# l-johnson-code/glTF-Renderer

Measured on AMD Instinct MI355X. Metric: Mrays/sec + ms/frame @1920x1080, 8-bounce, 1/2/4/8 MI355X, higher is better.
Workload: dtype f32

## Files before the change

gltf_renderer_amd/csrc/mipt_api.hip:

```cpp
#include <hip/hip_runtime.h>

#include <cmath>
#include <cstdio>
#include <cstdlib>
#include <cstring>
#include <string>
#include <vector>

#include "pt_types.h"

#include "pt_host.h"

using namespace pt;

struct StagingRing {
    static constexpr int kSlots = 8;
    void* host[kSlots] = {};
    size_t cap[kSlots] = {};
    hipEvent_t done[kSlots] = {};
    bool pending[kSlots] = {};
    int next = 0;
};

enum AccelState { ACCEL_CLEAN = 0, ACCEL_REFIT = 1, ACCEL_REBUILD = 2 };


struct pt_ctx {
    int device = 0;
    hipStream_t stream = nullptr;
    std::string error;
    StagingRing staging;

    std::vector<BufferRec> buffers;
    std::vector<TextureRec> textures;
    std::vector<SamplerRec> samplers;
    BufferRec* d_buffers = nullptr; size_t d_buffers_cap = 0; bool buffers_dirty = true;
    uint32_t* d_white = nullptr;
    struct TrioRec { const uint32_t *a, *n, *m, *e; uint4* ptr; };
    std::vector<TrioRec> trios;

    RMat* d_rmats = nullptr; int n_materials = 0; size_t rmats_cap = 0;
    std::vector<RMat> rmats_host;
    pt_light* d_lights = nullptr; int n_lights = 0; size_t lights_cap = 0;

    std::vector<InstanceRec> instances;
    InstanceRec* d_instances = nullptr; size_t instances_cap = 0;
    uint32_t n_tris = 0;
    Bvh4Node* d_nodes = nullptr; TriPacket* d_tris = nullptr; ShadePacket* d_shade = nullptr; size_t accel_cap = 0;
    uint32_t wide_nodes = 0, stack_need = 0;
    int32_t root = 0;
    AccelScratch scratch;
    int accel_state = ACCEL_REBUILD;
    bool accel_built = false;
    bool instances_dirty = true;
    std::vector<uint8_t> touched;
    uint8_t* d_touched = nullptr; size_t touched_cap = 0;
    uint32_t accel_refits = 0, accel_builds = 0;
    std::vector<int> free_buffers, free_textures, free_envs;

    std::vector<EnvDevice*> envs;
    float* d_sheen = nullptr;
    float* d_srgb = nullptr;
    float2* d_tangent_lut = nullptr;
    Counters* d_counters = nullptr;
    void* d_bones = nullptr; size_t bones_cap = 0, bones_used = 0;
    hipEvent_t bones_fence = nullptr; bool bones_fence_pending = false;
    void* d_workspace = nullptr; size_t workspace_cap = 0;
    void* d_tonemap = nullptr; size_t tonemap_cap = 0;
    pt::ExchangeState* exchange = nullptr;
    int32_t* d_deep = nullptr; size_t deep_cap = 0;
    uint32_t* d_occ = nullptr; size_t occ_pixels = 0; uint32_t occ_w = 0, occ_h = 0; bool occ_stale = true;
    bool occ_enabled = false;
    bool stage_timing = false;
    StageTimers timers;
    int kernel_mode = PT_MODE_WAVEFRONT;
    int stage_blocks = 0;
    hipEvent_t ev_trace[2] = {nullptr, nullptr}, ev_accel[2] = {nullptr, nullptr}, ev_skin[2] = {nullptr, nullptr};
    bool have_trace = false, have_accel = false, have_skin = false;
    int bounce_limit = PT_REFERENCE_MAX_BOUNCES;
    int samples_per_trace = 1;
    bool cull_null_shadow = false;
    bool counters_enabled = false;

    float previous_world_to_clip[16] = {0};
    int accumulated_frames = 0;

    int fail(int code, const std::string& msg) { error = msg; return code; }
};

#define HIPOK(call)                                                                                          \
    do {                                                                                                     \
        hipError_t _e = (call);                                                                              \
        if (_e != hipSuccess) return ctx->fail(PT_ERR_DEVICE, std::string(#call) + ": " + hipGetErrorString(_e)); \
    } while (0)
#define ENTER(ctx)                                                                                           \
    do {                                                                                                     \
        hipError_t _e = hipSetDevice((ctx)->device);                                                         \
        if (_e != hipSuccess) return (ctx)->fail(PT_ERR_DEVICE, std::string("hipSetDevice: ") + hipGetErrorString(_e)); \
    } while (0)

namespace {

hipError_t staged_upload(pt_ctx* ctx, void* dst, const void* src, size_t bytes) {
    if (bytes == 0) return hipSuccess;
    StagingRing& r = ctx->staging;
    const int k = r.next;
    r.next = (r.next + 1) % StagingRing::kSlots;
    hipError_t e;
    if (r.pending[k]) { if ((e = hipEventSynchronize(r.done[k]))) return e; r.pending[k] = false; }
    if (bytes > r.cap[k]) {
        if (r.host[k]) hipHostFree(r.host[k]);
        r.host[k] = nullptr; r.cap[k] = 0;
        const size_t nc = bytes + bytes / 2 + 4096;
        if ((e = hipHostMalloc(&r.host[k], nc, hipHostMallocDefault))) return e;
        r.cap[k] = nc;
    }
    if (!r.done[k] && (e = hipEventCreateWithFlags(&r.done[k], hipEventDisableTiming))) return e;
    memcpy(r.host[k], src, bytes);
    if ((e = hipMemcpyAsync(dst, r.host[k], bytes, hipMemcpyHostToDevice, ctx->stream))) return e;
    if ((e = hipEventRecord(r.done[k], ctx->stream))) return e;
    r.pending[k] = true;
    return hipSuccess;
}

template <typename T>
hipError_t upload_table(pt_ctx* ctx, T*& d, size_t& cap, const std::vector<T>& h) {
    size_t n = h.size() ? h.size() : 1;
    if (n > cap) {
        hipError_t e = hipStreamSynchronize(ctx->stream);
        if (e) return e;
        hipFree(d);
        d = nullptr; cap = 0;
        size_t nc = n + n / 2 + 8;
        e = hipMalloc((void**)&d, nc * sizeof(T));
        if (e) return e;
        cap = nc;
    }
    if (h.empty()) return hipSuccess;
    return staged_upload(ctx, d, h.data(), h.size() * sizeof(T));
}

void mat4_mul(const float* a, const float* b, float* out) {
    for (int c = 0; c < 4; c++)
        for (int r = 0; r < 4; r++) {
            float s = 0;
            for (int k = 0; k < 4; k++) s += a[k * 4 + r] * b[c * 4 + k];
            out[c * 4 + r] = s;
        }
}
bool mat4_inverse(const float* mf, float* out) {
    double m[16], inv[16];
    for (int i = 0; i < 16; i++) m[i] = mf[i];
    double s0 = m[0] * m[5] - m[4] * m[1], s1 = m[0] * m[9] - m[8] * m[1], s2 = m[0] * m[13] - m[12] * m[1];
    double s3 = m[4] * m[9] - m[8] * m[5], s4 = m[4] * m[13] - m[12] * m[5], s5 = m[8] * m[13] - m[12] * m[9];
    double c5 = m[10] * m[15] - m[14] * m[11], c4 = m[6] * m[15] - m[14] * m[7], c3 = m[6] * m[11] - m[10] * m[7];
    double c2 = m[2] * m[15] - m[14] * m[3], c1 = m[2] * m[11] - m[10] * m[3], c0 = m[2] * m[7] - m[6] * m[3];
    double det = s0 * c5 - s1 * c4 + s2 * c3 + s3 * c2 - s4 * c1 + s5 * c0;
    if (det == 0) return false;
    double id = 1.0 / det;
    inv[0] = (m[5] * c5 - m[9] * c4 + m[13] * c3) * id;
    inv[4] = (-m[4] * c5 + m[8] * c4 - m[12] * c3) * id;
    inv[8] = (m[7] * s5 - m[11] * s4 + m[15] * s3) * id;
    inv[12] = (-m[6] * s5 + m[10] * s4 - m[14] * s3) * id;
    inv[1] = (-m[1] * c5 + m[9] * c2 - m[13] * c1) * id;
    inv[5] = (m[0] * c5 - m[8] * c2 + m[12] * c1) * id;
    inv[9] = (-m[3] * s5 + m[11] * s2 - m[15] * s1) * id;
    inv[13] = (m[2] * s5 - m[10] * s2 + m[14] * s1) * id;
    inv[2] = (m[1] * c4 - m[5] * c2 + m[13] * c0) * id;
    inv[6] = (-m[0] * c4 + m[4] * c2 - m[12] * c0) * id;
    inv[10] = (m[3] * s4 - m[7] * s2 + m[15] * s0) * id;
    inv[14] = (-m[2] * s4 + m[6] * s2 - m[14] * s0) * id;
    inv[3] = (-m[1] * c3 + m[5] * c1 - m[9] * c0) * id;
    inv[7] = (m[0] * c3 - m[4] * c1 + m[8] * c0) * id;
    inv[11] = (-m[3] * s3 + m[7] * s1 - m[11] * s0) * id;
    inv[15] = (m[2] * s3 - m[6] * s1 + m[10] * s0) * id;
    for (int i = 0; i < 16; i++) out[i] = (float)inv[i];
    return true;
}

size_t format_stride(int f) {
    switch (f) {
        case PT_FORMAT_R16_UINT: return 2;
        case PT_FORMAT_R32_UINT: return 4;
        case PT_FORMAT_R32G32B32_FLOAT: return 12;
        case PT_FORMAT_R10G10B10A2_UNORM: return 4;
        case PT_FORMAT_R32G32_FLOAT: return 8;
        case PT_FORMAT_R16G16B16A16_UNORM: return 8;
        case PT_FORMAT_JOINT_WEIGHT: return 16;
        default: return 0;
    }
}

int stage_blocks_for(size_t slots) { return slots >= 1200000 ? 1536 : (slots >= 400000 ? 768 : 512); }

void mark_buffer_users(pt_ctx* ctx, int handle) {
    if (handle < 0) return;
    if (ctx->touched.size() != ctx->instances.size()) ctx->touched.assign(ctx->instances.size(), 0);
    const void* ptr = ctx->buffers[handle].ptr;
    bool any = false;
    for (size_t i = 0; i < ctx->instances.size(); i++) {
        const InstanceRec& r = ctx->instances[i];
        if (r.p_index == ptr || r.p_position == ptr || r.p_tangent_space == ptr || r.p_texcoord[0] == ptr || r.p_texcoord[1] == ptr || r.p_color == ptr) {
            ctx->touched[i] = 1;
            any = true;
        }
    }
    if (any && ctx->accel_state == ACCEL_CLEAN) ctx->accel_state = ACCEL_REFIT;
}

}

namespace pt {
class Pathtracer {
public:
    static int BuildAccel(pt_ctx* ctx) {
        if (ctx->buffers_dirty) { HIPOK(upload_table(ctx, ctx->d_buffers, ctx->d_buffers_cap, ctx->buffers)); ctx->buffers_dirty = false; }
        if (ctx->instances_dirty) { HIPOK(upload_table(ctx, ctx->d_instances, ctx->instances_cap, ctx->instances)); ctx->instances_dirty = false; }
        if (ctx->accel_state == ACCEL_CLEAN && ctx->accel_built) return PT_OK;
        const bool refit = ctx->accel_built && ctx->accel_state == ACCEL_REFIT;
        if (!refit) {
            size_t need = ctx->n_tris ? ctx->n_tris : 1;
            if (need > ctx->accel_cap) {
                HIPOK(hipStreamSynchronize(ctx->stream));
                hipFree(ctx->d_nodes); hipFree(ctx->d_tris); hipFree(ctx->d_shade);
                ctx->d_nodes = nullptr; ctx->d_tris = nullptr; ctx->d_shade = nullptr; ctx->accel_cap = 0;
                size_t cap = need + need / 8 + 64;
                HIPOK(hipMalloc((void**)&ctx->d_nodes, cap * sizeof(Bvh4Node)));
                HIPOK(hipMalloc((void**)&ctx->d_tris, cap * sizeof(TriPacket)));
                HIPOK(hipMalloc((void**)&ctx->d_shade, cap * sizeof(ShadePacket)));
                ctx->accel_cap = cap;
            }
        }
        HIPOK(hipEventRecord(ctx->ev_accel[0], ctx->stream));
        if (refit) {
            const size_t n = ctx->instances.size();
            if (n > ctx->touched_cap) {
                HIPOK(hipStreamSynchronize(ctx->stream));
                hipFree(ctx->d_touched); ctx->d_touched = nullptr; ctx->touched_cap = 0;
                HIPOK(hipMalloc((void**)&ctx->d_touched, n + 64));
                ctx->touched_cap = n + 64;
            }
            HIPOK(staged_upload(ctx, ctx->d_touched, ctx->touched.data(), n));
            HIPOK(accel_refit(ctx->scratch, ctx->d_instances, ctx->d_touched, ctx->n_tris, ctx->wide_nodes, ctx->d_nodes, ctx->d_tris, ctx->d_shade, ctx->stream));
            ctx->accel_refits++;
        } else {
            ctx->scratch.why.clear();
            const hipError_t be = accel_build(ctx->scratch, ctx->d_buffers, ctx->d_instances, (int)ctx->instances.size(), ctx->n_tris, ctx->d_nodes, ctx->d_tris,
                                              ctx->d_shade, &ctx->root, &ctx->wide_nodes, &ctx->stack_need, ctx->stream);
            if (be != hipSuccess) {
                ctx->accel_built = false; ctx->accel_state = ACCEL_REBUILD;
                return ctx->fail(PT_ERR_DEVICE, std::string("acceleration-structure build: ") + (ctx->scratch.why.empty() ? hipGetErrorString(be) : ctx->scratch.why.c_str()));
            }
            ctx->accel_builds++;
            ctx->occ_stale = true;
        }
        HIPOK(hipEventRecord(ctx->ev_accel[1], ctx->stream));
        ctx->have_accel = true;
        ctx->accel_state = ACCEL_CLEAN;
        ctx->accel_built = true;
        std::fill(ctx->touched.begin(), ctx->touched.end(), (uint8_t)0);
        if (!refit && ctx->stack_need > kDeepStackMax && ctx->scratch.builder != 0) {
            const int chosen = ctx->scratch.builder;
            ctx->scratch.builder = 0;
            ctx->scratch.fallbacks++;
            ctx->scratch.fallback_why = "clustered tree needs a traversal stack of " + std::to_string(ctx->stack_need) + " entries";
            const hipError_t be = accel_build(ctx->scratch, ctx->d_buffers, ctx->d_instances, (int)ctx->instances.size(), ctx->n_tris, ctx->d_nodes, ctx->d_tris,
                                              ctx->d_shade, &ctx->root, &ctx->wide_nodes, &ctx->stack_need, ctx->stream);
            ctx->scratch.builder = chosen;
            if (be != hipSuccess) {
                ctx->accel_built = false; ctx->accel_state = ACCEL_REBUILD;
                return ctx->fail(PT_ERR_DEVICE, std::string("acceleration-structure build (radix fallback): ") + (ctx->scratch.why.empty() ? hipGetErrorString(be) : ctx->scratch.why.c_str()));
            }
            HIPOK(hipEventRecord(ctx->ev_accel[1], ctx->stream));
        }
        if (!refit && ctx->stack_need > kDeepStackMax) {
            ctx->accel_built = false; ctx->accel_state = ACCEL_REBUILD;
            return ctx->fail(PT_ERR_CAPACITY, "acceleration structure needs a traversal stack of " + std::to_string(ctx->stack_need) + " entries (limit " +
                                              std::to_string(kDeepStackMax) + ")");
        }
        return PT_OK;
    }

    static int PathtraceScene(pt_ctx* ctx, const pt_settings* settings, const pt_execute_params* ep) {
        float world_to_clip[16], clip_to_world[16], view_to_world[16];
        mat4_mul(ep->view_to_clip, ep->world_to_view, world_to_clip);
        if (!mat4_inverse(ep->world_to_view, view_to_world) || !mat4_inverse(world_to_clip, clip_to_world))
            return ctx->fail(PT_ERR_INVALID_ARGUMENT, "singular camera matrix");
        bool reset = memcmp(world_to_clip, ctx->previous_world_to_clip, 64) != 0 || settings->reset;
        if (reset) ctx->accumulated_frames = 0;
        if (ctx->accumulated_frames < settings->max_accumulated_frames) {
            if (ep->light_count > ctx->n_lights) return ctx->fail(PT_ERR_INVALID_ARGUMENT, "light_count exceeds uploaded lights");
            if (ep->environment_map >= 0 && (ep->environment_map >= (int)ctx->envs.size() || !ctx->envs[ep->environment_map]))
                return ctx->fail(PT_ERR_BAD_HANDLE, "bad environment map handle");
            if (!ep->output) return ctx->fail(PT_ERR_INVALID_ARGUMENT, "output is null");
            if (ctx->accel_state != ACCEL_CLEAN || !ctx->accel_built || ctx->instances_dirty) { int r = BuildAccel(ctx); if (r) return r; }

            SceneRec sc;
            memset(&sc, 0, sizeof(sc));
            sc.rmats = ctx->d_rmats; sc.lights = ctx->d_lights; sc.instances = ctx->d_instances;
            sc.n_materials = (uint32_t)ctx->n_materials; sc.n_instances = (uint32_t)ctx->instances.size();
            sc.nodes = ctx->d_nodes; sc.tris = ctx->d_tris; sc.shade = ctx->d_shade; sc.root = ctx->root; sc.num_tris = ctx->n_tris;
            sc.sheen_e = ctx->d_sheen; sc.srgb_lut = ctx->d_srgb; sc.tangent_lut = ctx->d_tangent_lut;
            sc.has_env = 0;
            if (ep->environment_map >= 0) {
                const EnvDevice& ed = *ctx->envs[ep->environment_map];
                sc.env.cube = ed.cube; sc.env.cube_n = ed.mip_n[0]; sc.env.importance = ed.importance;
                for (int i = 0; i < 12; i++) sc.env.level_offset[i] = ed.level_offset[i];
                sc.env.imp_res = ed.imp_res; sc.env.imp_levels = ed.levels; sc.env.imp_total = ed.total;
                sc.env.blocked = ed.blocked;
                for (int i = 0; i < 5; i++) sc.env.blocked_offset[i] = ed.blocked_offset[i];
                sc.has_env = 1;
            }

            FrameConstants fc;
            memset(&fc, 0, sizeof(fc));
            memcpy(fc.clip_to_world, clip_to_world, 64);
            fc.camera_pos[0] = view_to_world[12]; fc.camera_pos[1] = view_to_world[13]; fc.camera_pos[2] = view_to_world[14];
            fc.num_of_lights = ep->light_count;
            fc.res_x = ep->width; fc.res_y = ep->height;
            fc.seed = settings->use_frame_as_seed ? (uint32_t)ep->frame : settings->seed;
            fc.accumulated_frames = ctx->accumulated_frames;
            memcpy(fc.environment_color, settings->environment_color, 12);
            fc.environment_intensity = settings->environment_intensity;
            fc.debug_output = settings->debug_output;
            fc.flags = settings->flags;
            fc.max_ray_length = 1000;
            auto clampi = [](int v, int lo, int hi) { return v < lo ? lo : (v > hi ? hi : v); };
            fc.min_bounces = clampi(settings->min_bounces, 0, ctx->bounce_limit);
            fc.max_bounces = clampi(settings->max_bounces, 0, ctx->bounce_limit);
            fc.luminance_clamp = settings->luminance_clamp;
            fc.min_rr = settings->min_russian_roulette_continue_prob;
            fc.max_rr = settings->max_russian_roulette_continue_prob;
            fc.tiles_x = (ep->width + PT_TILE - 1) / PT_TILE;
            fc.tiles_y = (ep->height + PT_TILE - 1) / PT_TILE;
            fc.tile_rank_count = ep->tile_rank_count ? ep->tile_rank_count : 1;
            fc.tile_rank = ep->tile_rank;
            if (fc.tile_rank >= fc.tile_rank_count) return ctx->fail(PT_ERR_INVALID_ARGUMENT, "tile_rank >= tile_rank_count");
            uint32_t ntiles = fc.tiles_x * fc.tiles_y;
            fc.my_tiles = ntiles > fc.tile_rank ? (ntiles - fc.tile_rank + fc.tile_rank_count - 1) / fc.tile_rank_count : 0;

            int batch = 1;
            if ((settings->flags & PT_FLAG_ACCUMULATE) && settings->debug_output == PT_DEBUG_OUTPUT_NONE) {
                batch = ctx->samples_per_trace;
                const long long room = (long long)settings->max_accumulated_frames - ctx->accumulated_frames;
                if ((long long)batch > room) batch = (int)room;
            }
            fc.cull_null_shadow = ctx->cull_null_shadow ? 1u : 0u;
            {
                size_t rare = 0;
                for (const RMat& m : ctx->rmats_host) rare += (m.sheen_color_factor[0] != 0.0f || m.sheen_color_factor[1] != 0.0f || m.sheen_color_factor[2] != 0.0f) ? 1 : 0;
                fc.defer_rare = (rare != 0 && rare * 10 <= ctx->rmats_host.size()) ? 1u : 0u;
                static const int forced = [] { const char* e = getenv("MIPT_DEFER_RARE"); return e ? (atoi(e) != 0 ? 1 : 0) : -1; }();
                if (forced >= 0) fc.defer_rare = (uint32_t)forced;
            }
            fc.spp = 1; fc.pixel_slots = fc.my_tiles * 256u;
            fc.div_pixel_slots = FastDiv::make(fc.pixel_slots); fc.div_tiles_x = FastDiv::make(fc.tiles_x);
            fc.seed_step = settings->use_frame_as_seed ? 1u : 0u;

            if ((int)ctx->stack_need > traversal_stack_capacity()) {
                const uint32_t entries = (ctx->stack_need - (uint32_t)traversal_stack_capacity() + 7u) & ~7u;
                size_t lanes;
                if (ctx->kernel_mode == PT_MODE_MEGAKERNEL) lanes = (size_t)fc.my_tiles * 256;
                else lanes = (size_t)traversal_grid_lanes(ctx->stage_blocks > 0 ? ctx->stage_blocks : stage_blocks_for((size_t)fc.pixel_slots * (size_t)batch));
                const size_t need = (size_t)entries * lanes * 4;
                if (need > ctx->deep_cap) {
                    HIPOK(hipStreamSynchronize(ctx->stream));
                    hipFree(ctx->d_deep); ctx->d_deep = nullptr; ctx->deep_cap = 0;
                    if (hipMalloc((void**)&ctx->d_deep, need) != hipSuccess) { (void)hipGetLastError(); return ctx->fail(PT_ERR_OUT_OF_MEMORY, "deep traversal stack: " + std::to_string(need) + " bytes"); }
                    ctx->deep_cap = need;
                }
                sc.deep_stack = ctx->d_deep; sc.deep_entries = entries; sc.deep_lanes = (uint32_t)lanes;
            }
            HIPOK(hipEventRecord(ctx->ev_trace[0], ctx->stream));
            if (ctx->kernel_mode == PT_MODE_MEGAKERNEL) {
                for (int k = 0; k < batch; k++) {
                    FrameConstants fk = fc;
                    fk.seed = fc.seed + (uint32_t)k * fc.seed_step;
                    fk.accumulated_frames = fc.accumulated_frames + k;
                    launch_megakernel(sc, fk, (float4*)ep->output, ctx->d_counters, ctx->counters_enabled, ctx->stream);
                }
            } else {
                fc.spp = (uint32_t)batch;
                if ((unsigned long long)fc.pixel_slots * fc.spp > 0x7fffffffull) return ctx->fail(PT_ERR_CAPACITY, "sample batch too large for this resolution");
                const int stage_blocks = ctx->stage_blocks > 0 ? ctx->stage_blocks : stage_blocks_for((size_t)fc.pixel_slots * fc.spp);
                size_t need = wavefront_workspace_bytes(fc, stage_blocks);
                if (need > ctx->workspace_cap) {
                    HIPOK(hipStreamSynchronize(ctx->stream));
                    hipFree(ctx->d_workspace); ctx->d_workspace = nullptr; ctx->workspace_cap = 0;
                    HIPOK(hipMalloc(&ctx->d_workspace, need));
                    ctx->workspace_cap = need;
                }
                uint32_t* occ = nullptr;
                if (ctx->occ_enabled && settings->debug_output == PT_DEBUG_OUTPUT_NONE) {
                    const size_t px = (size_t)ep->width * ep->height;
                    if (px != ctx->occ_pixels || ep->width != ctx->occ_w) {
                        HIPOK(hipStreamSynchronize(ctx->stream));
                        hipFree(ctx->d_occ); ctx->d_occ = nullptr; ctx->occ_pixels = 0;
                        if (hipMalloc((void**)&ctx->d_occ, px * 8 * 4) == hipSuccess) { ctx->occ_pixels = px; ctx->occ_w = ep->width; ctx->occ_h = ep->height; ctx->occ_stale = true; }
                        else (void)hipGetLastError();
                    }
                    if (ctx->d_occ && ctx->occ_stale) { HIPOK(hipMemsetAsync(ctx->d_occ, 0xff, ctx->occ_pixels * 8 * 4, ctx->stream)); ctx->occ_stale = false; }
                    occ = ctx->d_occ;
                }
                HIPOK(launch_wavefront(sc, fc, (float4*)ep->output, ctx->d_counters, ctx->counters_enabled, ctx->d_workspace, stage_blocks,
                                       ctx->stage_timing ? &ctx->timers : nullptr, ctx->stream, occ));
            }
            HIPOK(hipGetLastError());
            HIPOK(hipEventRecord(ctx->ev_trace[1], ctx->stream));
            ctx->have_trace = true;
            if (settings->flags & PT_FLAG_ACCUMULATE) ctx->accumulated_frames += batch;
            else ctx->accumulated_frames = 0;
        }
        memcpy(ctx->previous_world_to_clip, world_to_clip, 64);
        return PT_OK;
    }
};

class GpuSkin {
public:
    static int Run(pt_ctx* ctx, const pt_skin_params* p, const pt_bone* bones, int bone_count) {
        auto buf = [&](int h, int fmt, size_t count, const void** out) -> bool {
            if (h < 0 || h >= (int)ctx->buffers.size()) return false;
            const BufferRec& b = ctx->buffers[h];
            if ((int)b.format != fmt || b.bytes < count * format_stride(fmt)) return false;
            *out = b.ptr;
            return true;
        };
        SkinArgs a;
        memset(&a, 0, sizeof(a));
        a.num_of_vertices = p->num_of_vertices;
        a.input_mesh_flags = p->input_mesh_flags;
        a.output_mesh_flags = p->output_mesh_flags;
        a.num_of_morph_targets = p->num_of_morph_targets < PT_MAX_SIMULTANEOUS_MORPH_TARGETS ? p->num_of_morph_targets : PT_MAX_SIMULTANEOUS_MORPH_TARGETS;
        if (a.num_of_morph_targets < 0) a.num_of_morph_targets = 0;
        if (!bones || bone_count <= 0) a.input_mesh_flags &= (uint32_t)!PT_MESH_FLAG_JOINT_WEIGHT;
        const void* ptr = nullptr;
        if (!buf(p->input_position, PT_FORMAT_R32G32B32_FLOAT, p->num_of_vertices, &ptr)) return ctx->fail(PT_ERR_BAD_HANDLE, "skin: input_position");
        a.in_position = (const float*)ptr;
        if (a.input_mesh_flags & PT_MESH_FLAG_TANGENT_SPACE) {
            if (!buf(p->input_tangent_space, PT_FORMAT_R10G10B10A2_UNORM, p->num_of_vertices, &ptr)) return ctx->fail(PT_ERR_BAD_HANDLE, "skin: input_tangent_space");
            a.in_tangent_space = (const uint32_t*)ptr;
        }
        if (a.input_mesh_flags & PT_MESH_FLAG_JOINT_WEIGHT) {
            if (!buf(p->input_joint_weight, PT_FORMAT_JOINT_WEIGHT, p->num_of_vertices, &ptr)) return ctx->fail(PT_ERR_BAD_HANDLE, "skin: input_joint_weight");
            a.in_joint_weight = (const uint4*)ptr;
        }
        if (a.output_mesh_flags & PT_DYNAMIC_MESH_FLAG_POSITION) {
            if (!buf(p->output_position, PT_FORMAT_R32G32B32_FLOAT, p->num_of_vertices, &ptr)) return ctx->fail(PT_ERR_BAD_HANDLE, "skin: output_position");
            a.out_position = (float*)ptr;
        }
        if (a.output_mesh_flags & PT_DYNAMIC_MESH_FLAG_TANGENT_SPACE) {
            if (!buf(p->output_tangent_space, PT_FORMAT_R10G10B10A2_UNORM, p->num_of_vertices, &ptr)) return ctx->fail(PT_ERR_BAD_HANDLE, "skin: output_tangent_space");
            a.out_tangent_space = (uint32_t*)ptr;
        }
        for (int i = 0; i < a.num_of_morph_targets; i++) {
            a.morph_weight[i] = p->morph_weights[i];
            if (p->morph_position[i] != -1) {
                if (!buf(p->morph_position[i], PT_FORMAT_R32G32B32_FLOAT, p->num_of_vertices, &ptr)) return ctx->fail(PT_ERR_BAD_HANDLE, "skin: morph_position");
                a.morph_position[i] = (const float*)ptr;
            }
            if (p->morph_tangent_space[i] != -1) {
                if (!buf(p->morph_tangent_space[i], PT_FORMAT_R10G10B10A2_UNORM, p->num_of_vertices, &ptr)) return ctx->fail(PT_ERR_BAD_HANDLE, "skin: morph_tangent_space");
                a.morph_tangent_space[i] = (const uint32_t*)ptr;
            }
        }
        if (a.input_mesh_flags & PT_MESH_FLAG_JOINT_WEIGHT) {
            size_t bytes = (size_t)bone_count * sizeof(pt_bone);
            if (ctx->bones_used + bytes > ctx->bones_cap) {
                if (bytes > ctx->bones_cap) {
                    HIPOK(hipStreamSynchronize(ctx->stream));
                    hipFree(ctx->d_bones); ctx->d_bones = nullptr; ctx->bones_cap = 0;
                    const size_t nc = bytes * 8 + 4096;
                    HIPOK(hipMalloc(&ctx->d_bones, nc));
                    ctx->bones_cap = nc;
                } else if (ctx->bones_fence_pending) HIPOK(hipEventSynchronize(ctx->bones_fence));
                ctx->bones_used = 0;
            }
            void* dst = (char*)ctx->d_bones + ctx->bones_used;
            ctx->bones_used += (bytes + 255) & ~(size_t)255;
            HIPOK(staged_upload(ctx, dst, bones, bytes));
            a.bones = (const pt_bone*)dst;
            a.bone_count = bone_count;
        }
        HIPOK(hipEventRecord(ctx->ev_skin[0], ctx->stream));
        launch_skin(a, p->use_mfma != 0, ctx->stream);
        HIPOK(hipGetLastError());
        HIPOK(hipEventRecord(ctx->ev_skin[1], ctx->stream));
        if (a.bones) { HIPOK(hipEventRecord(ctx->bones_fence, ctx->stream)); ctx->bones_fence_pending = true; }
        ctx->have_skin = true;
        if (a.out_position) mark_buffer_users(ctx, p->output_position);
        if (a.out_tangent_space) mark_buffer_users(ctx, p->output_tangent_space);
        return PT_OK;
    }
};
}

static int exchange_frame_checked(pt_ctx* ctx, const void* local, void* frame, uint32_t w, uint32_t h, int mode, int dst, std::string& err) {
    return exchange_frame(ctx->exchange, local, frame ? frame : const_cast<void*>(local), w, h, mode, dst, ctx->stream, err);
}

extern "C" {

int pt_abi_version(void) { return MIPT_ABI_VERSION; }

int pt_create(int device, void* hip_stream, const float* sheen_e_16x16, pt_ctx** out) {
    if (!out || !sheen_e_16x16) return PT_ERR_INVALID_ARGUMENT;
    *out = nullptr;
    int count = 0;
    if (hipGetDeviceCount(&count) != hipSuccess || device < 0 || device >= count) return PT_ERR_DEVICE;
    if (hipSetDevice(device) != hipSuccess) return PT_ERR_DEVICE;
    pt_ctx* ctx = new pt_ctx();
    ctx->device = device;
    ctx->stream = (hipStream_t)hip_stream;
    float srgb[256];
    for (int i = 0; i < 256; i++) {
        double c = i / 255.0;
        srgb[i] = (float)(c <= 0.04045 ? c / 12.92 : pow((c + 0.055) / 1.055, 2.4));
    }
    bool ok = hipMalloc((void**)&ctx->d_sheen, 256 * 4) == hipSuccess && hipMalloc((void**)&ctx->d_srgb, 256 * 4) == hipSuccess &&
              hipMalloc((void**)&ctx->d_counters, sizeof(Counters)) == hipSuccess && hipMalloc((void**)&ctx->d_white, 16) == hipSuccess &&
              hipMemset(ctx->d_white, 0xff, 16) == hipSuccess &&
              hipMemcpy(ctx->d_sheen, sheen_e_16x16, 256 * 4, hipMemcpyHostToDevice) == hipSuccess &&
              hipMemcpy(ctx->d_srgb, srgb, 256 * 4, hipMemcpyHostToDevice) == hipSuccess &&
              hipMemset(ctx->d_counters, 0, sizeof(Counters)) == hipSuccess &&
              hipMalloc((void**)&ctx->d_tangent_lut, 1024 * sizeof(float2)) == hipSuccess &&
              build_tangent_lut(ctx->d_tangent_lut, ctx->stream) == hipSuccess;
    for (int i = 0; i < 2 && ok; i++)
        ok = hipEventCreate(&ctx->ev_trace[i]) == hipSuccess && hipEventCreate(&ctx->ev_accel[i]) == hipSuccess && hipEventCreate(&ctx->ev_skin[i]) == hipSuccess;
    ok = ok && hipEventCreateWithFlags(&ctx->bones_fence, hipEventDisableTiming) == hipSuccess;
    if (!ok) { pt_destroy(ctx); return PT_ERR_DEVICE; }
    ctx->samplers.push_back({PT_ADDRESS_WRAP, PT_ADDRESS_WRAP, PT_FILTER_LINEAR, PT_FILTER_LINEAR});
    if (const char* b = getenv("MIPT_ACCEL_BUILDER")) {
        if (!strcmp(b, "ploc")) ctx->scratch.builder = PT_BUILDER_PLOC;
        else if (!strcmp(b, "lbvh")) ctx->scratch.builder = PT_BUILDER_LBVH;
        else if (!strcmp(b, "reinsert")) ctx->scratch.builder = PT_BUILDER_PLOC_REINSERT;
    }
    if (const char* b = getenv("MIPT_OCC_CACHE")) ctx->occ_enabled = atoi(b) != 0;
    if (const char* b = getenv("MIPT_REINSERT_PASSES")) {
        const int v = atoi(b);
        if (v >= 0 && v <= 64) ctx->scratch.reinsert_passes = v;
    }
    if (const char* b = getenv("MIPT_REINSERT_MIN_GAIN")) {
        const float v = (float)atof(b);
        if (v >= 0.0f && v < 1.0f) ctx->scratch.reinsert_min_gain = v;
    }
    *out = ctx;
    return PT_OK;
}

void pt_destroy(pt_ctx* ctx) {
    if (!ctx) return;
    hipSetDevice(ctx->device);
    hipStreamSynchronize(ctx->stream);
    for (auto& b : ctx->buffers) hipFree((void*)b.ptr);
    for (auto& t : ctx->textures) hipFree((void*)t.texels);
    for (auto& t : ctx->trios) hipFree((void*)t.ptr);
    for (auto* e : ctx->envs) if (e) { env_free(*e); delete e; }
    hipFree(ctx->d_buffers); hipFree(ctx->d_white); hipFree(ctx->d_rmats); hipFree(ctx->d_lights);
// ... 73 lines not shown
    return PT_OK;
}

int pt_texture_create(pt_ctx* ctx, const uint8_t* rgba8, int width, int height, int srgb, int* handle_out) {
    if (!ctx || !rgba8 || !handle_out || width <= 0 || height <= 0) return PT_ERR_INVALID_ARGUMENT;
    ENTER(ctx);
    void* d = nullptr;
    size_t bytes = (size_t)width * height * 4;
    HIPOK(hipMalloc(&d, bytes + 4));
    hipError_t e = hipMemcpy(d, rgba8, bytes, hipMemcpyHostToDevice);
    if (e) { hipFree(d); return ctx->fail(PT_ERR_DEVICE, std::string("pt_texture_create: ") + hipGetErrorString(e)); }
    const TextureRec rec = {(const uint32_t*)d, width, height, srgb ? 1u : 0u, 0u};
    if (!ctx->free_textures.empty()) { *handle_out = ctx->free_textures.back(); ctx->free_textures.pop_back(); ctx->textures[*handle_out] = rec; }
    else { ctx->textures.push_back(rec); *handle_out = (int)ctx->textures.size() - 1; }
    return PT_OK;
}

int pt_texture_destroy(pt_ctx* ctx, int handle) {
    if (!ctx) return PT_ERR_INVALID_ARGUMENT;
    if (handle < 0 || handle >= (int)ctx->textures.size() || !ctx->textures[handle].texels) return ctx->fail(PT_ERR_BAD_HANDLE, "pt_texture_destroy");
    for (const RMat& m : ctx->rmats_host)
        for (int k = 0; k < SLOT_COUNT; k++)
            if (m.tex[k].texels == ctx->textures[handle].texels)
                return ctx->fail(PT_ERR_NOT_READY, "pt_texture_destroy: the texture is used by the current material table (replace it with pt_scene_set_materials first)");
    ENTER(ctx);
    HIPOK(hipStreamSynchronize(ctx->stream));
    hipFree((void*)ctx->textures[handle].texels);
    ctx->textures[handle] = TextureRec{nullptr, 0, 0, 0u, 0u};
    ctx->free_textures.push_back(handle);
    return PT_OK;
}

int pt_sampler_create(pt_ctx* ctx, const pt_sampler_desc* d, int* handle_out) {
    if (!ctx || !d || !handle_out) return PT_ERR_INVALID_ARGUMENT;
    if (d->address_u < 0 || d->address_u > 2 || d->address_v < 0 || d->address_v > 2) return ctx->fail(PT_ERR_INVALID_ARGUMENT, "pt_sampler_create: address mode");
    ctx->samplers.push_back({d->address_u, d->address_v, d->min_filter, d->mag_filter});
    *handle_out = (int)ctx->samplers.size() - 1;
    return PT_OK;
}

__global__ void k_trio_interleave(uint4* __restrict__ dst, const uint32_t* __restrict__ a, const uint32_t* __restrict__ n, const uint32_t* __restrict__ m,
                                  const uint32_t* __restrict__ e, size_t count) {
    const size_t i = (size_t)blockIdx.x * blockDim.x + threadIdx.x;
    if (i < count) dst[i] = make_uint4(a[i], n ? n[i] : 0xffffffffu, m ? m[i] : 0xffffffffu, e ? e[i] : 0xffffffffu);
}

int pt_scene_set_materials(pt_ctx* ctx, const pt_material* m, int count) {
    if (!ctx || (count > 0 && !m) || count < 0) return PT_ERR_INVALID_ARGUMENT;
    for (const InstanceRec& r : ctx->instances)
        if (r.gpu.material_id >= count)
            return ctx->fail(PT_ERR_BAD_HANDLE, "pt_scene_set_materials: the current instance table uses material " + std::to_string(r.gpu.material_id) +
                                                ", the new table has " + std::to_string(count) + " (replace the instances first)");
    ENTER(ctx);
    for (int i = 0; i < count; i++) {
        const pt_texture_sample* slots[15] = {&m[i].normal, &m[i].albedo, &m[i].metallic_roughness, &m[i].occlusion, &m[i].emissive, &m[i].specular,
                                              &m[i].specular_color, &m[i].clearcoat, &m[i].clearcoat_roughness, &m[i].clearcoat_normal, &m[i].anisotropy,
                                              &m[i].sheen_color, &m[i].sheen_roughness, &m[i].transmission, &m[i].thickness};
        for (auto* s : slots) {
            if (s->descriptor < -1 || s->descriptor >= (int)ctx->textures.size() || (s->descriptor >= 0 && !ctx->textures[s->descriptor].texels))
                return ctx->fail(PT_ERR_BAD_HANDLE, "material texture descriptor out of range or destroyed");
            if (s->sampler < 0 || s->sampler >= (int)ctx->samplers.size()) return ctx->fail(PT_ERR_BAD_HANDLE, "material sampler out of range");
        }
    }
    std::vector<RMat> rm((size_t)count);
    for (int i = 0; i < count; i++) {
        const pt_material& s = m[i];
        RMat& r = rm[i];
        memset(&r, 0, sizeof(r));
        r.flags = s.flags; r.alpha_mode = s.alpha_mode; r.metalness_factor = s.metalness_factor; r.roughness_factor = s.roughness_factor;
        memcpy(r.base_color_factor, s.base_color_factor, 16);
        memcpy(r.emissive_factor, s.emissive_factor, 12); r.alpha_cutoff = s.alpha_cutoff;
        r.ior = s.ior; r.normal_scale = s.normal_scale; r.specular_factor = s.specular_factor; r.clearcoat_normal_scale = s.clearcoat_normal_scale;
        memcpy(r.specular_color_factor, s.specular_color_factor, 12); r.clearcoat_factor = s.clearcoat_factor;
        r.clearcoat_roughness_factor = s.clearcoat_roughness_factor; r.anisotropy_strength = s.anisotropy_strength;
        r.anisotropy_cos = (float)cos((double)s.anisotropy_rotation); r.anisotropy_sin = (float)sin((double)s.anisotropy_rotation);
        memcpy(r.sheen_color_factor, s.sheen_color_factor, 12); r.sheen_roughness_factor = s.sheen_roughness_factor;
        r.transmission_factor = s.transmission_factor;
        const pt_texture_sample* slots[SLOT_COUNT] = {&s.normal, &s.albedo, &s.metallic_roughness, &s.occlusion, &s.emissive, &s.specular,
                                                      &s.specular_color, &s.clearcoat, &s.clearcoat_roughness, &s.clearcoat_normal, &s.anisotropy,
                                                      &s.sheen_color, &s.sheen_roughness, &s.transmission, &s.thickness};
        for (int k = 0; k < SLOT_COUNT; k++) {
            const pt_texture_sample& a = *slots[k];
            RTex& t = r.tex[k];
            if (a.descriptor == -1) {
                t.texels = ctx->d_white; t.width = 1; t.height = 1; t.flags = RT_POINT;
                t.m00 = 0; t.m01 = 0; t.ox = 0; t.m10 = 0; t.m11 = 0; t.oy = 0;
                continue;
            }
            const TextureRec& tx = ctx->textures[a.descriptor];
            const SamplerRec& sm = ctx->samplers[a.sampler];
            float sn = 0.0f, cs = 1.0f;
            if (a.rotation != 0.0f) { sn = (float)sin((double)a.rotation); cs = (float)cos((double)a.rotation); }
            t.texels = tx.texels; t.width = tx.width; t.height = tx.height;
            t.flags = (tx.srgb ? RT_SRGB : 0u) | ((uint32_t)sm.address_u << 1) | ((uint32_t)sm.address_v << 3) |
                      (sm.mag_filter == PT_FILTER_POINT ? RT_POINT : 0u) | ((a.tex_coord & 1) ? RT_TEXCOORD1 : 0u);
            t.m00 = cs * a.scale[0]; t.m01 = sn * a.scale[1]; t.ox = a.offset[0];
            t.m10 = -sn * a.scale[0]; t.m11 = cs * a.scale[1]; t.oy = a.offset[1];
            r.bound_mask |= 1u << k;
        }
    }
    const char* env_trio = getenv("MIPT_TEXTURE_INTERLEAVE");
    const bool use_trio = !(env_trio && env_trio[0] == '0');
    std::vector<char> trio_live(ctx->trios.size(), 0);
    for (int i = 0; i < count && use_trio; i++) {
        RMat& r = rm[i];
        const RTex& A = r.tex[SLOT_ALBEDO];
        const RTex& N = r.tex[SLOT_NORMAL];
        const RTex& M = r.tex[SLOT_METALLIC_ROUGHNESS];
        const RTex& E = r.tex[SLOT_EMISSIVE];
        const bool ba = (r.bound_mask >> SLOT_ALBEDO) & 1u, bn = (r.bound_mask >> SLOT_NORMAL) & 1u, bm = (r.bound_mask >> SLOT_METALLIC_ROUGHNESS) & 1u;
        auto same_footprint = [&](const RTex& t) {
            return t.width == A.width && t.height == A.height && ((t.flags ^ A.flags) & ~(uint32_t)RT_SRGB) == 0 && memcmp(&t.m00, &A.m00, 6 * sizeof(float)) == 0;
        };
        const bool be = ((r.bound_mask >> SLOT_EMISSIVE) & 1u) && same_footprint(E);
        if (!ba || !(bn || bm) || (bn && !same_footprint(N)) || (bm && !same_footprint(M))) continue;
        const uint32_t* kn = bn ? N.texels : nullptr;
        const uint32_t* km = bm ? M.texels : nullptr;
        const uint32_t* ke = be ? E.texels : nullptr;
        size_t at = ctx->trios.size();
        for (size_t k = 0; k < ctx->trios.size(); k++)
            if (ctx->trios[k].a == A.texels && ctx->trios[k].n == kn && ctx->trios[k].m == km && ctx->trios[k].e == ke) { at = k; break; }
        if (at == ctx->trios.size()) {
            const size_t texels = (size_t)A.width * A.height;
            uint4* d = nullptr;
            if (hipMalloc((void**)&d, texels * 16 + 32) != hipSuccess) { (void)hipGetLastError(); continue; }
            hipLaunchKernelGGL(k_trio_interleave, dim3((unsigned)((texels + 255) / 256)), dim3(256), 0, ctx->stream, d, A.texels, kn, km, ke, texels);
            HIPOK(hipMemsetAsync((char*)d + texels * 16, 0xff, 32, ctx->stream));
            ctx->trios.push_back({A.texels, kn, km, ke, d});
            trio_live.push_back(0);
        }
        trio_live[at] = 1;
        r.trio = ctx->trios[at].ptr;
        r.bound_mask |= RM_TRIO | ((bn && (N.flags & RT_SRGB)) ? RM_TRIO_SRGB_N : 0u) | ((bm && (M.flags & RT_SRGB)) ? RM_TRIO_SRGB_M : 0u) |
                        (be ? (RM_TRIO_EMISSIVE | ((E.flags & RT_SRGB) ? RM_TRIO_SRGB_E : 0u)) : 0u);
    }
    HIPOK(upload_table(ctx, ctx->d_rmats, ctx->rmats_cap, rm));
    ctx->rmats_host.swap(rm);
    ctx->n_materials = count;
    bool any_dead = false;
    for (char l : trio_live) any_dead |= !l;
    if (any_dead) {
        HIPOK(hipStreamSynchronize(ctx->stream));
        std::vector<pt_ctx::TrioRec> keep;
        for (size_t k = 0; k < ctx->trios.size(); k++) { if (trio_live[k]) keep.push_back(ctx->trios[k]); else hipFree((void*)ctx->trios[k].ptr); }
        ctx->trios.swap(keep);
    }
    return PT_OK;
}

extern "C" int pt_debug_interleaved_materials(const pt_ctx* ctx) {
    int n = 0;
    if (ctx) for (const RMat& r : ctx->rmats_host) n += (r.bound_mask & RM_TRIO) ? 1 : 0;
    return n;
}

extern "C" int pt_debug_interleaved_emissive(const pt_ctx* ctx) {
    int n = 0;
    if (ctx) for (const RMat& r : ctx->rmats_host) n += (r.bound_mask & RM_TRIO_EMISSIVE) ? 1 : 0;
    return n;
}

extern "C" int pt_debug_intersect(pt_ctx* ctx, const float* rays, uint32_t n, uint32_t ray_flags, int mode, float* out) {
    if (!ctx || (n && (!rays || !out)) || mode < 0 || mode > 1) return PT_ERR_INVALID_ARGUMENT;
    ENTER(ctx);
    if (ctx->accel_state != ACCEL_CLEAN || !ctx->accel_built || ctx->instances_dirty) { int r = Pathtracer::BuildAccel(ctx); if (r) return r; }
    if (n == 0) return PT_OK;
    SceneRec sc;
    memset(&sc, 0, sizeof(sc));
    sc.rmats = ctx->d_rmats; sc.lights = ctx->d_lights; sc.instances = ctx->d_instances;
    sc.n_materials = (uint32_t)ctx->n_materials; sc.n_instances = (uint32_t)ctx->instances.size();
    sc.nodes = ctx->d_nodes; sc.tris = ctx->d_tris; sc.shade = ctx->d_shade; sc.root = ctx->root; sc.num_tris = ctx->n_tris;
    sc.sheen_e = ctx->d_sheen; sc.srgb_lut = ctx->d_srgb; sc.tangent_lut = ctx->d_tangent_lut;
    const uint32_t lanes = (n + 255u) & ~255u;
    float *d_rays = nullptr, *d_out = nullptr; int32_t* d_deep = nullptr;
    auto done = [&](int code, const std::string& why) { hipFree(d_rays); hipFree(d_out); hipFree(d_deep); return code == PT_OK ? PT_OK : ctx->fail(code, why); };
    if (hipMalloc((void**)&d_rays, (size_t)n * 32) != hipSuccess || hipMalloc((void**)&d_out, (size_t)n * 32) != hipSuccess) { (void)hipGetLastError(); return done(PT_ERR_OUT_OF_MEMORY, "pt_debug_intersect: ray buffers"); }
    if ((int)ctx->stack_need > traversal_stack_capacity()) {
        const uint32_t entries = (ctx->stack_need - (uint32_t)traversal_stack_capacity() + 7u) & ~7u;
        if (hipMalloc((void**)&d_deep, (size_t)entries * lanes * 4) != hipSuccess) { (void)hipGetLastError(); return done(PT_ERR_OUT_OF_MEMORY, "pt_debug_intersect: deep stack"); }
        sc.deep_stack = d_deep; sc.deep_entries = entries; sc.deep_lanes = lanes;
    }
    hipError_t e = hipMemcpyAsync(d_rays, rays, (size_t)n * 32, hipMemcpyHostToDevice, ctx->stream);
    if (e == hipSuccess) { launch_debug_intersect(sc, d_rays, n, ray_flags, mode, d_out, ctx->stream); e = hipGetLastError(); }
    if (e == hipSuccess && getenv("MIPT_DEBUG_INTERSECT_TIMING")) {
        hipEvent_t ev[2]; hipEventCreate(&ev[0]); hipEventCreate(&ev[1]);
        hipEventRecord(ev[0], ctx->stream);
        for (int k = 0; k < 5; k++) launch_debug_intersect(sc, d_rays, n, ray_flags, mode, d_out, ctx->stream);
        hipEventRecord(ev[1], ctx->stream); hipEventSynchronize(ev[1]);
        float ms = 0; hipEventElapsedTime(&ms, ev[0], ev[1]);
        fprintf(stderr, "pt_debug_intersect: %u rays, %.3f ms per launch, %.1f Mrays/s\n", n, ms / 5, n / (ms / 5) * 1e-3);
        hipEventDestroy(ev[0]); hipEventDestroy(ev[1]);
    }
    if (e == hipSuccess) e = hipMemcpyAsync(out, d_out, (size_t)n * 32, hipMemcpyDeviceToHost, ctx->stream);
    if (e == hipSuccess) e = hipStreamSynchronize(ctx->stream);
    return done(e == hipSuccess ? PT_OK : PT_ERR_DEVICE, std::string("pt_debug_intersect: ") + hipGetErrorString(e));
}

extern "C" int pt_debug_sample_texture(pt_ctx* ctx, int unit, const uint32_t* mat_slot, const float* tc, uint32_t n, float* out_rgba, int32_t* out_taps) {
    if (!ctx || unit < 0 || unit > 1 || (n && (!mat_slot || !tc || !out_rgba))) return PT_ERR_INVALID_ARGUMENT;
    for (uint32_t i = 0; i < n; i++) {
        const uint32_t mat = mat_slot[2 * i], slot = mat_slot[2 * i + 1];
        if (mat >= (uint32_t)ctx->n_materials || !(slot < (uint32_t)SLOT_COUNT || (slot >= 16u && slot <= 19u)))
            return ctx->fail(PT_ERR_INVALID_ARGUMENT, "pt_debug_sample_texture: query " + std::to_string(i) + " names material " + std::to_string(mat) +
                                                      " slot " + std::to_string(slot) + " (" + std::to_string(ctx->n_materials) + " materials)");
    }
    ENTER(ctx);
    if (n == 0) return PT_OK;
    SceneRec sc;
    memset(&sc, 0, sizeof(sc));
    sc.rmats = ctx->d_rmats; sc.n_materials = (uint32_t)ctx->n_materials;
    sc.sheen_e = ctx->d_sheen; sc.srgb_lut = ctx->d_srgb; sc.tangent_lut = ctx->d_tangent_lut;
    uint32_t* d_ms = nullptr; float *d_tc = nullptr, *d_out = nullptr; int32_t* d_taps = nullptr;
    auto done = [&](int code, const std::string& why) { hipFree(d_ms); hipFree(d_tc); hipFree(d_out); hipFree(d_taps); return code == PT_OK ? PT_OK : ctx->fail(code, why); };
    if (hipMalloc((void**)&d_ms, (size_t)n * 8) != hipSuccess || hipMalloc((void**)&d_tc, (size_t)n * 16) != hipSuccess ||
        hipMalloc((void**)&d_out, (size_t)n * 16) != hipSuccess || hipMalloc((void**)&d_taps, (size_t)n * 20) != hipSuccess) {
        (void)hipGetLastError(); return done(PT_ERR_OUT_OF_MEMORY, "pt_debug_sample_texture: query buffers");
    }
    hipError_t e = hipMemcpyAsync(d_ms, mat_slot, (size_t)n * 8, hipMemcpyHostToDevice, ctx->stream);
    if (e == hipSuccess) e = hipMemcpyAsync(d_tc, tc, (size_t)n * 16, hipMemcpyHostToDevice, ctx->stream);
    if (e == hipSuccess) {
        if (unit == 0) launch_debug_sample_texture_wf(sc, d_ms, d_tc, n, d_out, d_taps, ctx->stream);
        else launch_debug_sample_texture_mk(sc, d_ms, d_tc, n, d_out, d_taps, ctx->stream);
        e = hipGetLastError();
    }
    if (e == hipSuccess) e = hipMemcpyAsync(out_rgba, d_out, (size_t)n * 16, hipMemcpyDeviceToHost, ctx->stream);
    if (e == hipSuccess && out_taps) e = hipMemcpyAsync(out_taps, d_taps, (size_t)n * 20, hipMemcpyDeviceToHost, ctx->stream);
    if (e == hipSuccess) e = hipStreamSynchronize(ctx->stream);
    return done(e == hipSuccess ? PT_OK : PT_ERR_DEVICE, std::string("pt_debug_sample_texture: ") + hipGetErrorString(e));
}

extern "C" int pt_debug_env_query(pt_ctx* ctx, int env, int unit, int op, const float* in, uint32_t n, float* out) {
    if (!ctx || unit < 0 || unit > 1 || op < 0 || op > 3 || (n && (!in || !out))) return PT_ERR_INVALID_ARGUMENT;
    if (env < 0 || env >= (int)ctx->envs.size() || !ctx->envs[env]) return ctx->fail(PT_ERR_BAD_HANDLE, "pt_debug_env_query: environment " + std::to_string(env));
    ENTER(ctx);
    if (n == 0) return PT_OK;
    const EnvDevice& ed = *ctx->envs[env];
    SceneRec sc;
    memset(&sc, 0, sizeof(sc));
    sc.env.cube = ed.cube; sc.env.cube_n = ed.mip_n[0]; sc.env.importance = ed.importance;
    for (int i = 0; i < 12; i++) sc.env.level_offset[i] = ed.level_offset[i];
    sc.env.imp_res = ed.imp_res; sc.env.imp_levels = ed.levels; sc.env.imp_total = ed.total;
    sc.env.blocked = ed.blocked;
    for (int i = 0; i < 5; i++) sc.env.blocked_offset[i] = ed.blocked_offset[i];
    sc.has_env = 1;
    const size_t in_bytes = (size_t)n * 8 * 4, out_bytes = (size_t)n * 16 * 4;
    float *d_in = nullptr, *d_out = nullptr;
    auto done = [&](int code, const std::string& why) { hipFree(d_in); hipFree(d_out); return code == PT_OK ? PT_OK : ctx->fail(code, why); };
    if (hipMalloc((void**)&d_in, in_bytes) != hipSuccess || hipMalloc((void**)&d_out, out_bytes) != hipSuccess) {
        (void)hipGetLastError(); return done(PT_ERR_OUT_OF_MEMORY, "pt_debug_env_query: query buffers");
    }
    hipError_t e = hipMemcpyAsync(d_in, in, in_bytes, hipMemcpyHostToDevice, ctx->stream);
    if (e == hipSuccess) e = hipMemcpyAsync(d_out, out, out_bytes, hipMemcpyHostToDevice, ctx->stream);
    if (e == hipSuccess) {
        if (unit == 0) launch_debug_env_query_wf(sc, op, d_in, n, d_out, ctx->stream);
        else launch_debug_env_query_mk(sc, op, d_in, n, d_out, ctx->stream);
        e = hipGetLastError();
    }
    if (e == hipSuccess) e = hipMemcpyAsync(out, d_out, out_bytes, hipMemcpyDeviceToHost, ctx->stream);
    if (e == hipSuccess) e = hipStreamSynchronize(ctx->stream);
    return done(e == hipSuccess ? PT_OK : PT_ERR_DEVICE, std::string("pt_debug_env_query: ") + hipGetErrorString(e));
}

extern "C" int pt_debug_env_create_raw(pt_ctx* ctx, int cube_n, const uint16_t* cube_rgba16f, const float* pyramid, int* env_out) {
    if (!ctx || cube_n < 1 || cube_n > 16384 || !cube_rgba16f || !pyramid || !env_out) return PT_ERR_INVALID_ARGUMENT;
    ENTER(ctx);
    EnvDevice* env = new EnvDevice();
    hipError_t e = env_build_raw(*env, cube_n, cube_rgba16f, pyramid, ctx->stream);
    if (e) { env_free(*env); delete env; return ctx->fail(PT_ERR_DEVICE, std::string("pt_debug_env_create_raw: ") + hipGetErrorString(e)); }
    if (!ctx->free_envs.empty()) { *env_out = ctx->free_envs.back(); ctx->free_envs.pop_back(); ctx->envs[*env_out] = env; }
    else { ctx->envs.push_back(env); *env_out = (int)ctx->envs.size() - 1; }
    return PT_OK;
}

extern "C" int pt_debug_env_read_blocked(pt_ctx* ctx, int env, float* out) {
    if (!ctx || !out) return PT_ERR_INVALID_ARGUMENT;
    if (env < 0 || env >= (int)ctx->envs.size() || !ctx->envs[env]) return ctx->fail(PT_ERR_BAD_HANDLE, "pt_debug_env_read_blocked: environment " + std::to_string(env));
    ENTER(ctx);
    HIPOK(hipStreamSynchronize(ctx->stream));
    const EnvDevice& ed = *ctx->envs[env];
    HIPOK(hipMemcpy(out, ed.blocked, (size_t)(ed.blocked_offset[4] + 1024u * 1024u) * 4, hipMemcpyDeviceToHost));
    return PT_OK;
}

int pt_scene_set_lights(pt_ctx* ctx, const pt_light* l, int count) {
    if (!ctx || (count > 0 && !l) || count < 0) return PT_ERR_INVALID_ARGUMENT;
    ENTER(ctx);
    std::vector<pt_light> h(l, l + count);
    HIPOK(upload_table(ctx, ctx->d_lights, ctx->lights_cap, h));
    ctx->n_lights = count;
    return PT_OK;
}

int pt_scene_set_instances(pt_ctx* ctx, const pt_instance_desc* in, int count) {
    if (!ctx || (count > 0 && !in) || count < 0) return PT_ERR_INVALID_ARGUMENT;
    if (count > PT_MAX_TLAS_INSTANCES) return ctx->fail(PT_ERR_CAPACITY, "more than PT_MAX_TLAS_INSTANCES instances");
    std::vector<InstanceRec> recs;
    uint64_t tris = 0;
    auto check = [&](int h, int fmt_a, int fmt_b, size_t count_needed) -> bool {
        if (h == -1) return true;
        if (!live_buffer(ctx, h)) return false;
        const BufferRec& b = ctx->buffers[h];
        if ((int)b.format != fmt_a && (int)b.format != fmt_b) return false;
        return b.bytes >= count_needed * format_stride(b.format);
    };
    for (int i = 0; i < count; i++) {
        const pt_instance_desc& d = in[i];
// ... 310 lines not shown
```

gltf_renderer_amd/csrc/pt_host.h:

```cpp
#pragma once
#include <hip/hip_runtime.h>

#include <string>
#include <vector>

#include "pt_types.h"

namespace pt {

struct AccelScratch {
    TriPacket* tris_unsorted = nullptr;
    uint64_t *keys_a = nullptr, *keys_b = nullptr;
    uint32_t *vals_a = nullptr, *vals_b = nullptr;
    int32_t* leaf_parent = nullptr;
    int32_t* node_parent = nullptr;
    void* seg = nullptr;
    size_t seg_leaves = 0;
    float* block_bounds = nullptr;
    uint32_t* bounds = nullptr;
    void* sort_temp = nullptr;
    size_t sort_temp_bytes = 0;
    BvhNode* nodes2 = nullptr;
    uint32_t* kept = nullptr;
    uint32_t* widx = nullptr;
    uint32_t* collapse_counters = nullptr;
    WideRanges* wide_ranges = nullptr;
    int builder = 2;
    float reinsert_min_gain = 1e-3f;
    int reinsert_passes = 8;
    void* reins_box = nullptr; int32_t *reins_parent = nullptr, *reins_top = nullptr; float* reins_gain = nullptr; uint32_t* reins_out = nullptr;
    unsigned long long* reins_lock = nullptr; uint8_t* reins_state = nullptr;
    void* ploc_c[2] = {nullptr, nullptr};
    uint32_t *ploc_nn = nullptr, *ploc_valid = nullptr, *ploc_pos = nullptr, *ploc_count = nullptr, *ploc_perm = nullptr, *ploc_counters = nullptr;
    int32_t *ploc_left = nullptr, *ploc_right = nullptr;
    void* ploc_scan_temp = nullptr; size_t ploc_scan_bytes = 0;
    size_t capacity = 0;
    std::string why;
    uint32_t fallbacks = 0;
    std::string fallback_why;
};
void accel_scratch_free(AccelScratch& s);
hipError_t accel_build(AccelScratch& s, const BufferRec* d_buffers, const InstanceRec* d_instances, int n_inst, uint32_t n_tris, Bvh4Node* d_nodes,
                       TriPacket* d_tris, ShadePacket* d_shade, int32_t* root_out, uint32_t* wide_nodes_out, uint32_t* stack_need_out, hipStream_t stream);
hipError_t accel_refit(AccelScratch& s, const InstanceRec* d_instances, const uint8_t* d_touched, uint32_t n_tris, uint32_t wide_nodes,
                       Bvh4Node* d_nodes, TriPacket* d_tris, ShadePacket* d_shade, hipStream_t stream);

hipError_t build_tangent_lut(float2* d_lut, hipStream_t stream);

struct EnvDevice {
    uint16_t* cube = nullptr;
    size_t mip_offset[16] = {0};
    int mip_n[16] = {0};
    int mips = 0;
    float* importance = nullptr;
    uint32_t level_offset[12] = {0};
    int levels = 0;
    int imp_res = 1024;
    float* blocked = nullptr;
    uint32_t blocked_offset[5] = {0};
    float total = 0.f;
};
hipError_t env_build(EnvDevice& e, const float* d_equirect, int w, int h, hipStream_t stream);
hipError_t env_build_raw(EnvDevice& e, int n, const uint16_t* cube_rgba16f, const float* pyramid, hipStream_t stream);
void env_free(EnvDevice& e);

struct SkinArgs {
    uint32_t num_of_vertices, input_mesh_flags, output_mesh_flags;
    int32_t num_of_morph_targets;
    float morph_weight[4];
    const float* morph_position[4];
    const uint32_t* morph_tangent_space[4];
    const float* in_position;
    const uint32_t* in_tangent_space;
    const uint4* in_joint_weight;
    const pt_bone* bones;
    int32_t bone_count;
    float* out_position;
    uint32_t* out_tangent_space;
};
void launch_skin(const SkinArgs& a, bool use_mfma, hipStream_t stream);
void launch_tonemap(const float4* in, uint32_t w, uint32_t h, const pt_tonemap_config& cfg, float* out_rgb, uint32_t* out_rgba8, hipStream_t stream);

size_t traversal_grid_lanes(int stage_blocks);
constexpr uint32_t kDeepStackMax = 1024;
int traversal_stack_capacity();
enum { STAGE_GENERATE = 0, STAGE_TRACE = 1, STAGE_SHADE = 2, STAGE_SHADOW = 3, STAGE_RESOLVE = 4, STAGE_COUNT = 5 };
struct StageTimers {
    std::vector<hipEvent_t> ev;
    std::vector<uint8_t> kind;
    size_t used = 0;
};
void launch_debug_sample_texture_wf(const SceneRec& sc, const uint32_t* d_mat_slot, const float* d_tc, uint32_t n, float* d_out, int32_t* d_taps, hipStream_t stream);
void launch_debug_sample_texture_mk(const SceneRec& sc, const uint32_t* d_mat_slot, const float* d_tc, uint32_t n, float* d_out, int32_t* d_taps, hipStream_t stream);
void launch_debug_env_query_wf(const SceneRec& sc, int op, const float* d_in, uint32_t n, float* d_out, hipStream_t stream);
void launch_debug_env_query_mk(const SceneRec& sc, int op, const float* d_in, uint32_t n, float* d_out, hipStream_t stream);
void launch_debug_intersect(const SceneRec& sc, const float* d_rays, uint32_t n, uint32_t rf, int mode, float* d_out, hipStream_t stream);
void launch_megakernel(const SceneRec& sc, const FrameConstants& fc, float4* output, Counters* counters, bool count, hipStream_t stream);
size_t wavefront_workspace_bytes(const FrameConstants& fc, int stage_blocks);
hipError_t launch_wavefront(const SceneRec& sc, const FrameConstants& fc, float4* output, Counters* counters, bool count, void* workspace,
                            int stage_blocks, StageTimers* timers, hipStream_t stream, uint32_t* occ_cache);

size_t radix_sort_temp_bytes(size_t n);
hipError_t radix_sort_pairs_u64_u32(void* temp, uint64_t* keys_in, uint64_t* keys_out, uint32_t* vals_in, uint32_t* vals_out, size_t n, hipStream_t stream);
size_t exclusive_scan_temp_bytes(size_t n);
hipError_t exclusive_scan_u32(void* temp, const uint32_t* in, uint32_t* out, size_t n, hipStream_t stream);

struct ExchangeState;
uint32_t tiles_of_rank(uint32_t w, uint32_t h, uint32_t rank, uint32_t world);
hipError_t tiles_pack(const void* image, uint32_t w, uint32_t h, uint32_t rank, uint32_t world, void* packed, hipStream_t stream);
hipError_t tiles_unpack(const void* packed, uint32_t w, uint32_t h, uint32_t rank, uint32_t world, void* image, hipStream_t stream);
int exchange_unique_id(void* out128, std::string& err);
int exchange_probe(std::string& err);
int exchange_create(ExchangeState** out, int rank, int world, const void* id128, std::string& err);
int exchange_create_loopback(ExchangeState** out, int rank, int world, uint64_t group, int device, std::string& err);
const char* exchange_transport_name(const ExchangeState* x);
int exchange_frame(ExchangeState* x, const void* local, void* frame, uint32_t w, uint32_t h, int mode, int dst, hipStream_t stream, std::string& err);
void exchange_free(ExchangeState* x);

}
```

gltf_renderer_amd/csrc/pt_shading.h:

```cpp
#pragma once
#include "pt_math.h"
#include "pt_types.h"

namespace pt {

constexpr float kMinRoughness = 0.001f;

PT_DEV vec4 next_random(uint32_t px, uint32_t py, uint32_t seed, int& count) {
    uint32_t x = px * 1664525u + 1013904223u, y = py * 1664525u + 1013904223u;
    uint32_t z = seed * 1664525u + 1013904223u, w = (uint32_t)count * 1664525u + 1013904223u;
    count++;
    x += y * w; y += z * x; z += x * y; w += y * z;
    x ^= x >> 16; y ^= y >> 16; z ^= z >> 16; w ^= w >> 16;
    x += y * w; y += z * x; z += x * y; w += y * z;
    const float s = 2.3283064365386963e-10f;
    return {(float)x * s, (float)y * s, (float)z * s, (float)w * s};
}

PT_DEV vec3 decode_octahedral(float ex, float ey) {
    float z = 1.f - fabsf(ex) - fabsf(ey);
    float x = ex, y = ey;
    if (!(z >= 0.f)) {
        x = (ex >= 0 ? 1.f : -1.f) * (1.f - fabsf(ey));
        y = (ey >= 0 ? 1.f : -1.f) * (1.f - fabsf(ex));
// ... 281 lines not shown
    if (threadIdx.x < n) {
        float4 q[6];
        shade_inst_pack(sc.instances[threadIdx.x], q);
#pragma unroll
        for (int k = 0; k < 6; k++) pt_lds_inst[threadIdx.x * 6u + k] = q[k];
    }
    __syncthreads();
}
PT_DEV ShadeInst load_shade_inst(const SceneRec& sc, uint32_t id) {
    float4 q[6];
    if (sc.small_tables || id < kInstCacheMax) {
#pragma unroll
        for (int k = 0; k < 6; k++) q[k] = pt_lds_inst[id * 6u + k];
    } else shade_inst_pack(sc.instances[id], q);
    return shade_inst_unpack(q);
}
#else
PT_DEV void stage_instances(const SceneRec&) {}
PT_DEV ShadeInst load_shade_inst(const SceneRec& sc, uint32_t id) { float4 q[6]; shade_inst_pack(sc.instances[id], q); return shade_inst_unpack(q); }
#endif
PT_DEV HitGeom get_vertex_attributes(const SceneRec& sc, const ShadeInst& in, const PacketVerts& pv, vec3 w) {
    HitGeom a;
    const vec3 p0 = pv.p[0], p1 = pv.p[1], p2 = pv.p[2];
    const bool has_ts = (in.streams & SI_TANGENT_SPACE) != 0;
    const uint32_t ts0 = pv.ts[0], ts1 = pv.ts[1], ts2 = pv.ts[2];
    a.color = fetch_vertex_color((in.streams & SI_COLOR) != 0, pv, w);
    a.tc[0] = fetch_texcoord((in.streams & SI_TEXCOORD0) != 0, pv.uv0, w);
    a.tc[1] = fetch_texcoord((in.streams & SI_TEXCOORD1) != 0, pv.uv1, w);
    vec3 pos = w.x * p0 + w.y * p1 + w.z * p2;
    vec3 ng = cross(p1 - p0, p2 - p0);
    vec3 n, t;
    float tw;
    if (has_ts) {
        vec3 n0, n1, n2, t0, t1, t2;
        float w0, w1, w2;
        decode_tangent_space(ts0, tangent_sincos(sc, (ts0 >> 20) & 0x3ffu), n0, t0, w0);
        decode_tangent_space(ts1, tangent_sincos(sc, (ts1 >> 20) & 0x3ffu), n1, t1, w1);
        decode_tangent_space(ts2, tangent_sincos(sc, (ts2 >> 20) & 0x3ffu), n2, t2, w2);
        n = w.x * n0 + w.y * n1 + w.z * n2;
        t = w.x * t0 + w.y * t1 + w.z * t2;
        tw = w0;
    } else {
        n = ng;
        vec3 helper = v3(1, 0, 0);
        if (fabsf(ng.x) > fabsf(ng.y)) helper = v3(0, 1, 0);
        t = normalize(cross(helper, ng));
        tw = 1;
    }
    a.position = mul_point(in.T, pos);
    a.ng = normalize(mul_dir(in.N, ng));
    a.n = normalize(mul_dir(in.N, n));
    a.t = normalize(mul_dir(in.T, t));
    a.tw = tw;
    a.bt = tw * normalize(cross(a.n, a.t));
    return a;
}

struct Surface {
    vec3 albedo; float alpha, metalness, ax, ay;
    vec3 n, at, ab; float ior;
    vec3 spec_color; float spec_factor, clearcoat, cc_rough;
    vec3 cc_n, sheen_color; float sheen_a, transmissive;
    vec3 emissive_texel;
    float sheen_lh, sheen_sv;
};
struct MatHeader {
    uint32_t flags; int32_t alpha_mode; float metalness_factor, roughness_factor;
    vec4 base_color_factor;
    vec3 emissive_factor; float alpha_cutoff;
    float ior, normal_scale, specular_factor, clearcoat_normal_scale;
    vec3 specular_color_factor; float clearcoat_factor;
    float clearcoat_roughness_factor, anisotropy_strength, anisotropy_cos, anisotropy_sin;
    vec3 sheen_color_factor; float sheen_roughness_factor;
    float transmission_factor; uint32_t bound_mask;
    const uint4* trio;
};
PT_DEV MatHeader load_mat_header(const RMat* m) {
    const float4* q = (const float4*)m;
    const float4 a = q[0], b = q[1], c = q[2], d = q[3], e = q[4], f = q[5], g = q[6], h = q[7];
    MatHeader r;
    r.flags = __float_as_uint(a.x); r.alpha_mode = __float_as_int(a.y); r.metalness_factor = a.z; r.roughness_factor = a.w;
    r.base_color_factor = {b.x, b.y, b.z, b.w};
    r.emissive_factor = v3(c.x, c.y, c.z); r.alpha_cutoff = c.w;
    r.ior = d.x; r.normal_scale = d.y; r.specular_factor = d.z; r.clearcoat_normal_scale = d.w;
    r.specular_color_factor = v3(e.x, e.y, e.z); r.clearcoat_factor = e.w;
    r.clearcoat_roughness_factor = f.x; r.anisotropy_strength = f.y; r.anisotropy_cos = f.z; r.anisotropy_sin = f.w;
    r.sheen_color_factor = v3(g.x, g.y, g.z); r.sheen_roughness_factor = g.w;
    r.transmission_factor = h.x; r.bound_mask = __float_as_uint(h.y);
    r.trio = (const uint4*)(((uint64_t)__float_as_uint(h.w) << 32) | (uint64_t)__float_as_uint(h.z));
    return r;
}
PT_DEV bool slot_bound(uint32_t mask, int slot) { return (mask >> slot) & 1u; }
#ifdef PT_LUT_LDS
constexpr uint32_t kMatCacheMax = 96;
constexpr uint32_t kMatCacheRecs = 17;
static __shared__ float4 pt_lds_mat[kMatCacheMax * kMatCacheRecs];
PT_DEV bool materials_cached(const SceneRec& sc) { return sc.small_tables || sc.n_materials <= kMatCacheMax; }
PT_DEV void stage_materials(const SceneRec& sc) {
    if (materials_cached(sc)) {
        const uint32_t total = sc.n_materials * kMatCacheRecs;
        for (uint32_t i = threadIdx.x; i < total; i += blockDim.x) {
            const uint32_t m = i / kMatCacheRecs, k = i - m * kMatCacheRecs;
            pt_lds_mat[i] = ((const float4*)(sc.rmats + m))[k];
        }
    }
    __syncthreads();
}
PT_DEV MatHeader material_header(const SceneRec& sc, uint32_t mid) {
    if (materials_cached(sc)) return load_mat_header((const RMat*)(pt_lds_mat + mid * kMatCacheRecs));
    return load_mat_header(sc.rmats + mid);
}
PT_DEV RTex material_slot012(const SceneRec& sc, uint32_t mid, int slot) {
    if (materials_cached(sc)) return load_rtex((const RTex*)(pt_lds_mat + mid * kMatCacheRecs + 8 + 3 * slot));
    return load_rtex(&sc.rmats[mid].tex[slot]);
}
#else
PT_DEV MatHeader material_header(const SceneRec& sc, uint32_t mid) { return load_mat_header(sc.rmats + mid); }
PT_DEV RTex material_slot012(const SceneRec& sc, uint32_t mid, int slot) { return load_rtex(&sc.rmats[mid].tex[slot]); }
#endif
PT_DEV void base_color_alpha(const SceneRec& sc, const RMat* m, const vec2 tc[2], vec4 vc, unsigned& taps, float& base_alpha, float& alpha, float& cutoff) {
    const float4* q = (const float4*)m;
    const float4 a = q[0], b = q[1], c = q[2], h = q[7];
    vec4 col = vec4{b.x, b.y, b.z, b.w} * vc;
    if (slot_bound(__float_as_uint(h.y), SLOT_ALBEDO)) col = col * sample_slot(sc, m, SLOT_ALBEDO, tc, taps);
    const int alpha_mode = __float_as_int(a.y);
    cutoff = c.w;
    base_alpha = col.w;
    alpha = alpha_mode == PT_ALPHA_MODE_BLEND ? col.w : (alpha_mode == PT_ALPHA_MODE_MASK ? (col.w < cutoff ? 0.f : 1.f) : 1.f);
}
PT_DEV vec3 normal_from_sample(vec4 s, float scale, vec3 gn, vec3 t, vec3 b) {
    vec3 nm = v3(s.x * 2.f - 1.f, s.y * 2.f - 1.f, s.z * 2.f - 1.f);
    nm.x *= scale; nm.y *= scale;
    return normalize(to_world(t, b, gn, nm));
}
PT_DEV vec3 emissive_of(const SceneRec& sc, const RMat* m, const MatHeader& h, const vec2 tc[2], unsigned& taps, vec3 fetched) {
    vec3 e = h.emissive_factor;
#if PT_TEX_PAIRS && PT_TEX_TRIO
    if (h.bound_mask & RM_TRIO_EMISSIVE) { taps++; return e * fetched; }
#endif
    if (slot_bound(h.bound_mask, SLOT_EMISSIVE)) e = e * xyz(sample_slot(sc, m, SLOT_EMISSIVE, tc, taps));
    return e;
}
PT_DEV vec3 normal_adaptation(vec3 ng, vec3 ns, vec3 v) {
    vec3 r = reflect(-v, ns);
    float rdng = dot(r, ng);
    if (rdng < 0) return normalize(v + normalize(r - rdng * ng));
    return ns;
}
struct PbrTexels {
    TexTaps k_alb, k_nrm, k_mr;
    uint32_t a00, a10, a01, a11, n00, n10, n01, n11, m00, m10, m01, m11;
    vec4 emissive;
};
PT_DEV PbrTexels fetch_pbr_texels(const SceneRec& sc, uint32_t mid, const MatHeader& h, const vec2 tc[2]) {
    PbrTexels f;
    f.emissive = vec4{0, 0, 0, 0};
#if PT_TEX_PAIRS && PT_TEX_TRIO
    const bool trio = (h.bound_mask & RM_TRIO) != 0;
    const RTex t_alb = material_slot012(sc, mid, SLOT_ALBEDO);
    const TexTaps k_alb = texture_taps(t_alb, tc);
    TexTaps k_nrm = k_alb, k_mr = k_alb;
    k_nrm.srgb = (h.bound_mask & RM_TRIO_SRGB_N) ? (uint32_t)RT_SRGB : 0u; k_mr.srgb = (h.bound_mask & RM_TRIO_SRGB_M) ? (uint32_t)RT_SRGB : 0u;
    uint32_t a00 = 0, a10 = 0, a01 = 0, a11 = 0, n00 = 0, n10 = 0, n01 = 0, n11 = 0, m00 = 0, m10 = 0, m01 = 0, m11 = 0;
    if (__any(trio)) {
        if (trio) {
            const uint4* row0 = h.trio + (k_alb.p0 - t_alb.texels) + k_alb.ia;
            const uint4* row1 = h.trio + (k_alb.p1 - t_alb.texels) + k_alb.ia;
            const uint4 A0 = gload_u4(row0), B0 = gload_u4(row0 + 1), A1 = gload_u4(row1), B1 = gload_u4(row1 + 1);
            uint4 t00 = k_alb.i0 == k_alb.ia ? A0 : B0, t01 = k_alb.i0 == k_alb.ia ? A1 : B1;
            uint4 t10 = k_alb.i1 == k_alb.ia ? A0 : B0, t11 = k_alb.i1 == k_alb.ia ? A1 : B1;
            if (__any(k_alb.edge)) {
                if (k_alb.edge) { t10 = gload_u4(h.trio + (k_alb.p0 - t_alb.texels) + k_alb.i1); t11 = gload_u4(h.trio + (k_alb.p1 - t_alb.texels) + k_alb.i1); }
            }
            a00 = t00.x; a10 = t10.x; a01 = t01.x; a11 = t11.x;
            n00 = t00.y; n10 = t10.y; n01 = t01.y; n11 = t11.y;
            m00 = t00.z; m10 = t10.z; m01 = t01.z; m11 = t11.z;
            if (h.bound_mask & RM_TRIO_EMISSIVE) {
                TexTaps k_em = k_alb;
                k_em.srgb = (h.bound_mask & RM_TRIO_SRGB_E) ? (uint32_t)RT_SRGB : 0u;
                f.emissive = resolve_taps(k_em, t00.w, t10.w, t01.w, t11.w, sc.srgb_lut);
            }
        }
    }
    if (__any(!trio)) {
        if (!trio) {
            const RTex t_nrm = material_slot012(sc, mid, SLOT_NORMAL), t_mr = material_slot012(sc, mid, SLOT_METALLIC_ROUGHNESS);
            k_nrm = texture_taps(t_nrm, tc); k_mr = texture_taps(t_mr, tc);
            const uint2 ar0 = tap_row(k_alb, 0), ar1 = tap_row(k_alb, 1), nr0 = tap_row(k_nrm, 0), nr1 = tap_row(k_nrm, 1), mr0 = tap_row(k_mr, 0), mr1 = tap_row(k_mr, 1);
            const TexQuad qa = tap_quad(k_alb, ar0, ar1), qn = tap_quad(k_nrm, nr0, nr1), qm = tap_quad(k_mr, mr0, mr1);
            a00 = qa.t00; a10 = qa.t10; a01 = qa.t01; a11 = qa.t11;
            n00 = qn.t00; n10 = qn.t10; n01 = qn.t01; n11 = qn.t11;
            m00 = qm.t00; m10 = qm.t10; m01 = qm.t01; m11 = qm.t11;
        }
    }
#else
    const RTex t_alb = material_slot012(sc, mid, SLOT_ALBEDO), t_nrm = material_slot012(sc, mid, SLOT_NORMAL), t_mr = material_slot012(sc, mid, SLOT_METALLIC_ROUGHNESS);
    const TexTaps k_alb = texture_taps(t_alb, tc), k_nrm = texture_taps(t_nrm, tc), k_mr = texture_taps(t_mr, tc);
#if PT_TEX_PAIRS
    const uint2 ar0 = tap_row(k_alb, 0), ar1 = tap_row(k_alb, 1), nr0 = tap_row(k_nrm, 0), nr1 = tap_row(k_nrm, 1), mr0 = tap_row(k_mr, 0), mr1 = tap_row(k_mr, 1);
    const TexQuad qa = tap_quad(k_alb, ar0, ar1), qn = tap_quad(k_nrm, nr0, nr1), qm = tap_quad(k_mr, mr0, mr1);
    const uint32_t a00 = qa.t00, a10 = qa.t10, a01 = qa.t01, a11 = qa.t11;
    const uint32_t n00 = qn.t00, n10 = qn.t10, n01 = qn.t01, n11 = qn.t11;
    const uint32_t m00 = qm.t00, m10 = qm.t10, m01 = qm.t01, m11 = qm.t11;
#else
    const uint32_t a00 = gload(k_alb.p00), a10 = gload(k_alb.p10), a01 = gload(k_alb.p01), a11 = gload(k_alb.p11);
    const uint32_t n00 = gload(k_nrm.p00), n10 = gload(k_nrm.p10), n01 = gload(k_nrm.p01), n11 = gload(k_nrm.p11);
    const uint32_t m00 = gload(k_mr.p00), m10 = gload(k_mr.p10), m01 = gload(k_mr.p01), m11 = gload(k_mr.p11);
#endif
#endif
    f.k_alb = k_alb; f.k_nrm = k_nrm; f.k_mr = k_mr;
    f.a00 = a00; f.a10 = a10; f.a01 = a01; f.a11 = a11;
    f.n00 = n00; f.n10 = n10; f.n01 = n01; f.n11 = n11;
    f.m00 = m00; f.m10 = m10; f.m01 = m01; f.m11 = m11;
    return f;
}
PT_DEV Surface get_surface(const SceneRec& sc, uint32_t flags, const RMat* m, const MatHeader& h, const HitGeom& a, vec3 view, unsigned& taps) {
    Surface s;
    const PbrTexels f = fetch_pbr_texels(sc, (uint32_t)(m - sc.rmats), h, a.tc);
    s.emissive_texel = xyz(f.emissive);
    const TexTaps &k_alb = f.k_alb, &k_nrm = f.k_nrm, &k_mr = f.k_mr;
    const uint32_t a00 = f.a00, a10 = f.a10, a01 = f.a01, a11 = f.a11, n00 = f.n00, n10 = f.n10, n01 = f.n01, n11 = f.n11, m00 = f.m00, m10 = f.m10, m01 = f.m01, m11 = f.m11;
    const bool b_alb = slot_bound(h.bound_mask, SLOT_ALBEDO), b_nrm = slot_bound(h.bound_mask, SLOT_NORMAL), b_mr = slot_bound(h.bound_mask, SLOT_METALLIC_ROUGHNESS);
    taps += (b_alb ? 1u : 0u) + (b_nrm ? 1u : 0u) + (b_mr ? 1u : 0u);
    vec4 bc = h.base_color_factor * a.color;
    if (b_alb) bc = bc * resolve_taps(k_alb, a00, a10, a01, a11, sc.srgb_lut);
    s.albedo = xyz(bc);
    s.alpha = h.alpha_mode == PT_ALPHA_MODE_BLEND ? bc.w : (h.alpha_mode == PT_ALPHA_MODE_MASK ? (bc.w < h.alpha_cutoff ? 0.f : 1.f) : 1.f);
    s.n = b_nrm ? normal_from_sample(resolve_taps(k_nrm, n00, n10, n01, n11, sc.srgb_lut), h.normal_scale, a.n, a.t, a.bt) : a.n;
    if (flags & PT_FLAG_SHADING_NORMAL_ADAPTATION) s.n = normal_adaptation(a.ng, s.n, view);
    float metal = h.metalness_factor, rough = h.roughness_factor;
    if (b_mr) { vec4 t = resolve_taps(k_mr, m00, m10, m01, m11, sc.srgb_lut); metal *= t.z; rough *= t.y; }
    s.metalness = metal;
    s.ay = hmax(rough * rough, kMinRoughness);
    if (slot_bound(h.bound_mask, SLOT_OCCLUSION)) taps++;
    if (slot_bound(h.bound_mask, SLOT_EMISSIVE)) taps++;
    s.ior = h.ior;
    s.spec_factor = h.specular_factor;
    s.spec_color = h.specular_color_factor;
    s.clearcoat = h.clearcoat_factor;
    s.cc_rough = h.clearcoat_roughness_factor;
    s.cc_n = a.n;
    float strength = h.anisotropy_strength;
    vec3 av = v3(1, 0, 1);
    s.sheen_color = h.sheen_color_factor;
    float sheen_rough = h.sheen_roughness_factor;
    s.transmissive = h.transmission_factor;
#ifndef PT_PROBE_BASE_ONLY
    if ((h.bound_mask & ((1u << SLOT_COUNT) - 1u)) >> SLOT_SPECULAR) {
        if (slot_bound(h.bound_mask, SLOT_SPECULAR)) s.spec_factor *= sample_slot(sc, m, SLOT_SPECULAR, a.tc, taps).w;
        if (slot_bound(h.bound_mask, SLOT_SPECULAR_COLOR)) s.spec_color = s.spec_color * xyz(sample_slot(sc, m, SLOT_SPECULAR_COLOR, a.tc, taps));
        if (slot_bound(h.bound_mask, SLOT_CLEARCOAT)) s.clearcoat *= sample_slot(sc, m, SLOT_CLEARCOAT, a.tc, taps).x;
        if (slot_bound(h.bound_mask, SLOT_CLEARCOAT_ROUGHNESS)) s.cc_rough *= sample_slot(sc, m, SLOT_CLEARCOAT_ROUGHNESS, a.tc, taps).y;
        if (slot_bound(h.bound_mask, SLOT_CLEARCOAT_NORMAL))
            s.cc_n = normal_from_sample(sample_slot(sc, m, SLOT_CLEARCOAT_NORMAL, a.tc, taps), h.clearcoat_normal_scale, a.n, a.t, a.bt);
        if (slot_bound(h.bound_mask, SLOT_ANISOTROPY)) {
            vec4 t = sample_slot(sc, m, SLOT_ANISOTROPY, a.tc, taps);
            av = v3(t.x * 2 - 1, t.y * 2 - 1, t.z);
        }
        if (slot_bound(h.bound_mask, SLOT_SHEEN_COLOR)) s.sheen_color = s.sheen_color * xyz(sample_slot(sc, m, SLOT_SHEEN_COLOR, a.tc, taps));
        if (slot_bound(h.bound_mask, SLOT_SHEEN_ROUGHNESS)) sheen_rough *= sample_slot(sc, m, SLOT_SHEEN_ROUGHNESS, a.tc, taps).w;
        if (slot_bound(h.bound_mask, SLOT_TRANSMISSION)) s.transmissive *= sample_slot(sc, m, SLOT_TRANSMISSION, a.tc, taps).x;
        if (slot_bound(h.bound_mask, SLOT_THICKNESS)) taps++;
    }
#endif
    if (flags & PT_FLAG_SHADING_NORMAL_ADAPTATION) s.cc_n = normal_adaptation(a.ng, s.cc_n, view);
    const float cr = h.anisotropy_cos, sr = h.anisotropy_sin;
    vec2 adir = normalize(vec2{cr * av.x + -sr * av.y, sr * av.x + cr * av.y});
    strength *= av.z;
    vec3 sb = normalize(cross(s.n, a.t));
    vec3 st = normalize(cross(sb, s.n));
    sb = sb * a.tw;
    s.at = normalize(to_world(st, sb, s.n, v3(adir.x, adir.y, 0)));
    s.ab = normalize(cross(s.at, s.n));
    s.ax = hmax(lerpf(s.ay, 1, strength * strength), kMinRoughness);
    s.sheen_a = hmax(sheen_rough * sheen_rough, kMinRoughness);
    s.ax = hmax(s.ax, kMinRoughness); s.ay = hmax(s.ay, kMinRoughness);
    s.cc_rough = hmax(s.cc_rough, kMinRoughness);
    if (flags & PT_FLAG_MATERIAL_USE_GEOMETRIC_NORMALS) { s.n = a.ng; s.cc_n = a.ng; }
    return s;
}

PT_DEV vec4 debug_sample_query(const SceneRec& sc, uint32_t mid, int slot, const vec2 tc[2], int32_t taps5[5]) {
    const RMat* m = sc.rmats + mid;
    unsigned taps = 0;
    const uint32_t* base;
    TexTaps k;
    vec4 r;
    if (slot < SLOT_COUNT) {
        const RTex t = load_rtex(&m->tex[slot]);
        k = texture_taps(t, tc); base = t.texels;
        r = sample_slot(sc, m, slot, tc, taps);
    } else {
        const MatHeader h = material_header(sc, mid);
        const PbrTexels f = fetch_pbr_texels(sc, mid, h, tc);
        const int s = slot == 16 ? SLOT_ALBEDO : slot == 17 ? SLOT_NORMAL : slot == 18 ? SLOT_METALLIC_ROUGHNESS : SLOT_EMISSIVE;
#if PT_TEX_PAIRS && PT_TEX_TRIO
        const bool trio = (h.bound_mask & RM_TRIO) != 0;
#else
        const bool trio = false;
#endif
        const RTex t = load_rtex(&m->tex[trio ? SLOT_ALBEDO : s]);
        base = t.texels;
        if (slot == 16) { k = f.k_alb; r = resolve_taps(k, f.a00, f.a10, f.a01, f.a11, sc.srgb_lut); }
        else if (slot == 17) { k = f.k_nrm; r = resolve_taps(k, f.n00, f.n10, f.n01, f.n11, sc.srgb_lut); }
        else if (slot == 18) { k = f.k_mr; r = resolve_taps(k, f.m00, f.m10, f.m01, f.m11, sc.srgb_lut); }
        else if (trio && (h.bound_mask & RM_TRIO_EMISSIVE)) { k = f.k_alb; r = f.emissive; }
        else { const RTex te = load_rtex(&m->tex[SLOT_EMISSIVE]); k = texture_taps(te, tc); base = te.texels; r = sample_slot(sc, m, SLOT_EMISSIVE, tc, taps); }
    }
#if PT_TEX_PAIRS
    taps5[0] = k.i0; taps5[1] = k.i1;
    taps5[2] = (int32_t)((k.p0 - base) / k.width); taps5[3] = (int32_t)((k.p1 - base) / k.width);
    taps5[4] = k.ia;
#else
    (void)k; (void)base; taps5[0] = taps5[1] = taps5[2] = taps5[3] = taps5[4] = -1;
#endif
    return r;
}

PT_DEV float schlick(float f0, float c) { return f0 + (1 - f0) * hpow5(1 - fabsf(c)); }
PT_DEV vec3 schlick3(vec3 f0, float c) { return f0 + (1 - f0) * hpow5(1 - fabsf(c)); }
PT_DEV float ggx_d(float a, float ndh) {
    float a2 = a * a;
    float den = ndh * ndh * (a2 - 1) + 1;
    den *= kPi * den;
    return fdiv(a2 * heavyside(ndh), den);
}
PT_DEV float ggx_corr_v(float a, float ndl, float ndv, float hdl, float hdv) {
    float a2 = a * a;
    float num = 0.5f * heavyside(hdl) * heavyside(hdv);
    float den = fabsf(ndv) * sqrtf(a2 + (1 - a2) * ndl * ndl);
    den += fabsf(ndl) * sqrtf(a2 + (1 - a2) * ndv * ndv);
    return fdiv(num, den);
}
PT_DEV float specular_brdf(float a, float ndl, float ndv, float ndh, float hdl, float hdv) { return ggx_corr_v(a, ndl, ndv, hdl, hdv) * ggx_d(a, ndh); }
PT_DEV float ggx_aniso_d(float ax, float ay, vec3 h) {
    float a2 = ax * ay;
    vec3 f = v3(ay * h.x, ax * h.y, a2 * h.z);
    float w2 = fdiv(a2, dot(f, f));
    return fdiv(heavyside(h.z) * a2 * w2 * w2, kPi);
}
PT_DEV float aniso_specular_brdf(float ax, float ay, vec3 v, vec3 h, vec3 l) {
    float hdv = dot(h, v), hdl = dot(h, l);
    float num = 0.5f * heavyside(hdv) * heavyside(hdl);
    float vv = fabsf(l.z) * length(v3(ax * v.x, ay * v.y, v.z));
    float ll = fabsf(v.z) * length(v3(ax * l.x, ay * l.y, l.z));
    return fdiv(num, vv + ll) * ggx_aniso_d(ax, ay, h);
}
PT_DEV float fresnel_coat_w(float weight, float ndv) {
    float f0 = (1 - 1.5f) / (1 + 1.5f);
    f0 *= f0;
    return weight * schlick(f0, ndv);
}
PT_DEV float sheen_l(float alpha, float x) {
    float t = (1 - alpha) * (1 - alpha);
    float a = lerpf(21.5473f, 25.3245f, t), b = lerpf(3.82987f, 3.32435f, t), c = lerpf(0.19823f, 0.16801f, t);
    float d = lerpf(-1.97760f, -1.27393f, t), e = lerpf(-4.32054f, -4.85967f, t);
    return fdiv(a, 1 + b * hpow(x, c)) + d * x + e;
}
PT_DEV float sheen_shadowing(float alpha, float c, float l_half) {
    if (c < 0.5f) return pt_exp(sheen_l(alpha, c));
    return pt_exp(2 * l_half - sheen_l(alpha, 1 - c));
}
PT_DEV float sheen_alpha(const Surface& s) { return clampf(s.sheen_a, 0.000001f, 1); }
PT_DEV void prepare_sheen(Surface& s, vec3 v) {
    const float sa = sheen_alpha(s);
    s.sheen_lh = sheen_l(sa, 0.5f);
    s.sheen_sv = sheen_shadowing(sa, to_local(s.at, s.ab, s.n, v).z, s.sheen_lh);
}
PT_DEV float sheen_brdf(const Surface& s, float alpha, float ndl, float ndv, float ndh) {
    float inv_r = fdiv(1.0f, alpha);
    float sin2h = 1 - ndh * ndh;
    float d = fdiv((2 + inv_r) * hpow(sin2h, inv_r * 0.5f), 2 * kPi);
    float vis = clampf(fdiv(1.0f, (1 + s.sheen_sv + sheen_shadowing(alpha, ndl, s.sheen_lh)) * 4 * ndv * ndl), 0, 1);
    return d * vis;
}
PT_DEV float sheen_e(const float* lut, float alpha, float cos_theta) {
    float x = cos_theta * 16.f - 0.5f, y = alpha * 16.f - 0.5f;
    if (!(x == x)) x = 0;
    if (!(y == y)) y = 0;
    x = clampf(x, -1.f, 16.f); y = clampf(y, -1.f, 16.f);
    float fx0 = floorf(x), fy0 = floorf(y);
    int i0 = (int)fx0, j0 = (int)fy0;
    float fx = x - fx0, fy = y - fy0;
    int ia = max(i0, 0), ib = min(i0 + 1, 15), ja = max(j0, 0), jb = min(j0 + 1, 15);
    ia = min(ia, 15); ja = min(ja, 15); ib = max(ib, 0); jb = max(jb, 0);
    float w00 = (1 - fx) * (1 - fy), w10 = fx * (1 - fy), w01 = (1 - fx) * fy, w11 = fx * fy;
    return sheen_entry(lut, ja * 16 + ia) * w00 + sheen_entry(lut, ja * 16 + ib) * w10 + sheen_entry(lut, jb * 16 + ia) * w01 + sheen_entry(lut, jb * 16 + ib) * w11;
}
PT_DEV float modulate_roughness(float a, float ior) { return clampf(lerpf(0, a, saturate(2 * (ior - 1))), kMinRoughness, 1.0f); }

PT_DEV vec3 gltf_bsdf(const float* lut, const Surface& s, vec3 v, vec3 l, int mode) {
    vec3 n = s.n;
    vec3 h = normalize(v + l);
    vec3 vl = to_local(s.at, s.ab, n, v), hl = to_local(s.at, s.ab, n, h), ll = to_local(s.at, s.ab, n, l);
    float hdl = dot(h, l), hdv = dot(h, v);
    float h_dot_abs_l = dot(normalize(v3(ll.x, ll.y, fabsf(ll.z)) + vl), vl);
    bool refl = mode != 2, trans = mode != 1;
    float cndv = dot(n, v), cndh = dot(n, h), cndl = dot(n, l);
#ifndef PT_PROBE_BASE_ONLY
    const float cc = refl ? saturate(cndl) * specular_brdf(s.cc_rough, cndl, cndv, cndh, hdl, hdv) : 0.f;
#else
    const float cc = 0.f;
#endif
    const float coat_w = fresnel_coat_w(s.clearcoat, cndv);
    float spec = refl ? saturate(ll.z) * aniso_specular_brdf(s.ax, s.ay, vl, hl, ll) : 0.f;
    vec3 diffuse = refl ? saturate(ll.z) * (s.albedo / kPi) : v3(0);
    vec3 transmission = v3(0);
#ifndef PT_PROBE_BASE_ONLY
    if (trans) {
        float a = modulate_roughness(s.ay, s.ior);
        vec3 lr = l - 2 * dot(n, l) * n;
        vec3 hr = normalize(v + lr);
        transmission = saturate(-ll.z) * (s.albedo * specular_brdf(a, dot(n, lr), dot(n, v), dot(n, hr), dot(hr, lr), dot(hr, v)));
    }
#endif
    diffuse = lerp3(diffuse, transmission, s.transmissive);
    float f0s = fdiv(1 - s.ior, 1 + s.ior);
    vec3 f0 = v3(f0s);
    f0 *= f0 * s.spec_color;
    f0 = hmin(f0, v3(1));
    vec3 fr = schlick3(f0, h_dot_abs_l);
    vec3 dielectric = (1 - s.spec_factor * max3(fr)) * diffuse + s.spec_factor * fr * v3(spec);
    vec3 metal = refl ? v3(spec) * schlick3(s.albedo, hdv) : v3(0);
    vec3 material = lerp3(dielectric, metal, s.metalness);
    float sa = sheen_alpha(s);
    float ms = max3(s.sheen_color);
#ifndef PT_SHEEN_SKIP
#define PT_SHEEN_SKIP 1
#endif
    const bool no_sheen = s.sheen_color.x == 0.0f && s.sheen_color.y == 0.0f && s.sheen_color.z == 0.0f;
    if (PT_SHEEN_SKIP && !__any(!no_sheen)) {
        const float sin2h = 1 - hl.z * hl.z;
        const float layer = (refl && !(sin2h >= 0.0f)) ? __builtin_nanf("") : 0.0f;
        material = v3(layer) + material * 1.0f;
    } else {
#ifndef PT_PROBE_BASE_ONLY
        vec3 sheen = refl ? v3(saturate(ll.z) * sheen_brdf(s, sa, ll.z, vl.z, hl.z)) : v3(0);
#else
        vec3 sheen = v3(0);
#endif
        float scaling = 1.0f;
        if (ms != 0.0f) scaling = hmin(1.0f - ms * sheen_e(lut, sa, vl.z), 1.0f - ms * sheen_e(lut, sa, ll.z));
        material = s.sheen_color * sheen + material * scaling;
    }
    return lerp3(material, v3(cc), coat_w);
}

PT_DEV vec2 uv_to_square(vec2 uv) { return {uv.x * 2 + -1, uv.y * -2 + 1}; }
PT_DEV vec2 square_to_uv(vec2 s) { return {(s.x - -1) * 0.5f, (s.y - 1) * -0.5f}; }
PT_DEV float square_to_disk_angle(vec2 s, float& r) {
    r = hmax(fabsf(s.x), fabsf(s.y));
    return r == 0 ? 0 : fdiv(kPi * (r + (fabsf(s.y) - fabsf(s.x))), 4 * r);
}
PT_DEV vec2 square_to_disk_finish(vec2 s, float r, float cs, float sn) { return {signf(s.x) * r * cs, signf(s.y) * r * sn}; }
PT_DEV vec2 square_to_disk(vec2 s) {
    float r;
    const float phi = square_to_disk_angle(s, r);
    float sn_, cs_;
    pt_sincos(phi, sn_, cs_);
    return square_to_disk_finish(s, r, cs_, sn_);
}
PT_DEV vec3 square_to_sphere(vec2 s) {
    float d = 1 - (fabsf(s.x) + fabsf(s.y));
    float r = 1 - fabsf(d);
    float phi = (r == 0) ? 0 : (kPi / 4) * (fdiv(fabsf(s.y) - fabsf(s.x), r) + 1);
    float f = r * sqrtf(2 - r * r);
    float sn_, cs_;
    pt_sincos(phi, sn_, cs_);
    return {f * signf(s.x) * cs_, f * signf(s.y) * sn_, signf(d) * (1 - r * r)};
}
PT_DEV vec2 sphere_to_square(vec3 p) {
    float r = sqrtf(1 - fabsf(p.z));
    float phi = pt_atan2(fabsf(p.y), fabsf(p.x));
    float d = signf(p.z) * (1 - r);
    float diff = r * ((4 / kPi) * phi - 1);
    return {signf(p.x) * 0.5f * (1 - d - diff), signf(p.y) * 0.5f * (1 - d + diff)};
}
PT_DEV vec3 cubemap_to_direction(int face, float u, float v) {
    vec3 ud, vd, fd;
    switch (face) {
        case 0: fd = v3(1, 0, 0); ud = v3(0, 0, -1); vd = v3(0, -1, 0); break;
        case 1: fd = v3(-1, 0, 0); ud = v3(0, 0, 1); vd = v3(0, -1, 0); break;
        case 2: fd = v3(0, 1, 0); ud = v3(1, 0, 0); vd = v3(0, 0, 1); break;
        case 3: fd = v3(0, -1, 0); ud = v3(1, 0, 0); vd = v3(0, 0, -1); break;
        case 4: fd = v3(0, 0, 1); ud = v3(1, 0, 0); vd = v3(0, -1, 0); break;
        default: fd = v3(0, 0, -1); ud = v3(-1, 0, 0); vd = v3(0, -1, 0); break;
    }
    u = u * 2 - 1; v = v * 2 - 1;
    return normalize(fd + u * ud + v * vd);
}
PT_DEV vec3 sample_cosine_hemisphere_finish(vec3 n, float u1, float cs, float sn) {
    float y = 2 * u1 - 1;
    float s = sqrtf(1.0f - y * y);
    return normalize(n + v3(s * cs, s * sn, y));
}
PT_DEV vec3 sample_cosine_hemisphere(vec3 n, float u0, float u1) {
    float theta = kTau * u0;
    float sn_, cs_;
    pt_sincos(theta, sn_, cs_);
    return sample_cosine_hemisphere_finish(n, u1, cs_, sn_);
}
PT_DEV float cosine_hemisphere_pdf(vec3 n, vec3 v) { return saturate(fdiv(dot(v, n), kPi)); }
PT_DEV vec3 sample_ggx_normal_finish(float a, float u1, float cs, float sn) {
    float ct = sqrtf(fdiv(1 - u1, 1 + (a * a - 1) * u1));
    float st = sqrtf(1 - ct * ct);
    return {st * cs, st * sn, ct};
}
PT_DEV vec3 sample_ggx_normal(float a, float u0, float u1) {
    float phi = kTau * u0;
    float sn_, cs_;
    pt_sincos(phi, sn_, cs_);
    return sample_ggx_normal_finish(a, u1, cs_, sn_);
}
PT_DEV float ggx_normal_pdf(float a, vec3 n, vec3 h) { float ndh = dot(n, h); return ggx_d(a, ndh) * ndh; }

struct Lobes { float alpha, clearcoat, sheen, specular, diffuse, transmission; };
PT_DEV Lobes lobe_probabilities(const Surface& s, vec3 v) {
    Lobes p;
    float remaining = 1;
    p.alpha = 1.0f - s.alpha;
    remaining -= p.alpha;
    p.clearcoat = lerpf(0.f, 1.f, fresnel_coat_w(s.clearcoat, dot(s.cc_n, v)));
    p.clearcoat *= remaining;
    remaining -= p.clearcoat;
    p.sheen = any_gt0(s.sheen_color) ? 0.5f : 0.0f;
    p.sheen *= remaining;
    remaining -= p.sheen;
    p.specular = 0.5f;
    p.specular *= remaining;
    remaining -= p.specular;
    p.transmission = s.transmissive;
    p.transmission *= remaining;
    remaining -= p.transmission;
    p.diffuse = remaining;
    return p;
}
PT_DEV float transmission_pdf(const Surface& s, vec3 v, vec3 l) {
    float a = modulate_roughness(s.ay, s.ior);
    l = l - 2 * dot(s.n, l) * s.n;
    vec3 h = normalize(v + l);
    float pdf = ggx_normal_pdf(a, s.n, h);
    pdf = fdiv(pdf, 4 * dot(v, h));
    return pdf;
}
PT_DEV float bsdf_pdf(const Surface& s, vec3 v, vec3 l, bool is_transmission, const Lobes& p) {
    if (is_transmission) return p.transmission * transmission_pdf(s, v, l);
    vec3 h = normalize(v + l);
    float vdh4 = 4 * dot(v, h);
    float cc = ggx_normal_pdf(s.cc_rough, s.cc_n, h);
    cc = fdiv(cc, vdh4);
    float pdf = p.clearcoat * cc;
    float cosp = cosine_hemisphere_pdf(s.n, l);
    pdf += p.sheen * cosp;
    vec3 lh = to_local(s.at, s.ab, s.n, h);
    float sp = ggx_aniso_d(s.ax, s.ay, lh) * lh.z;
    sp = fdiv(sp, vdh4);
    pdf += p.specular * sp;
    pdf += p.diffuse * cosp;
    return pdf;
}
PT_DEV vec3 evaluate_bsdf(uint32_t flags, const float* lut, const Surface& s, const Lobes& p, vec3 ng, vec3 v, vec3 l, float& pdf) {
    if (flags & PT_FLAG_MATERIAL_DIFFUSE_WHITE) {
        float ndl = saturate(dot(s.n, l));
        pdf = fdiv(ndl, kPi);
        return v3(fdiv(ndl, kPi));
    }
    if (flags & PT_FLAG_MATERIAL_MIS) {
        bool is_transmission = (dot(ng, l) * dot(ng, v)) < 0;
        pdf = bsdf_pdf(s, v, l, is_transmission, p);
        return s.alpha * gltf_bsdf(lut, s, v, l, is_transmission ? 2 : 1);
    }
    float ndl = saturate(dot(s.n, l));
    pdf = fdiv(ndl, kPi);
    pdf *= s.alpha;
    return s.alpha * gltf_bsdf(lut, s, v, l, 0);
}
PT_DEV vec3 sample_bsdf(uint32_t flags, const float* lut, const Surface& s, const Lobes& p, vec3 u, vec3 v, vec3& l, float& pdf,
                        bool& is_transmission, bool& use_mis) {
    if (flags & PT_FLAG_MATERIAL_DIFFUSE_WHITE) {
        use_mis = true; is_transmission = false;
        l = sample_cosine_hemisphere(s.n, u.y, u.z);
        pdf = cosine_hemisphere_pdf(s.n, l);
        return v3(fdiv(dot(s.n, l), kPi));
    }
    if (flags & PT_FLAG_MATERIAL_MIS) {
        is_transmission = false; use_mis = true;
        float x = u.x;
        int layer;
        if (x <= p.alpha) layer = 4;
        else { x -= p.alpha;
            if (x <= p.clearcoat) layer = 3;
            else { x -= p.clearcoat;
                if (x <= p.sheen) layer = 2;
                else { x -= p.sheen;
                    if (x <= p.specular) layer = 1;
                    else { x -= p.specular; layer = (x <= p.transmission) ? 5 : 0; } } } }
        if (layer == 4) {
            l = -v; use_mis = false; pdf = p.alpha; is_transmission = true;
            return v3(1 - s.alpha);
        }
        const vec2 sq = uv_to_square({u.y, u.z});
        float disk_r = 0;
        const float disk_phi = square_to_disk_angle(sq, disk_r);
        const float angle = layer == 1 ? disk_phi : kTau * u.y;
        float cs, sn;
        pt_sincos(angle, sn, cs);
        if (layer == 0 || layer == 2) l = sample_cosine_hemisphere_finish(s.n, u.z, cs, sn);
        else if (layer == 1) {
            vec2 d = square_to_disk_finish(sq, disk_r, cs, sn);
            vec3 hl = v3(d.x, d.y, sqrtf(1 - d.x * d.x - d.y * d.y));
            hl.x *= s.ax; hl.y *= s.ay;
            hl = normalize(hl);
            l = reflect(-v, to_world(s.at, s.ab, s.n, hl));
        } else if (layer == 3) {
            vec3 t, b;
            basis_simple(s.cc_n, t, b);
            l = reflect(-v, to_world(t, b, s.cc_n, sample_ggx_normal_finish(s.cc_rough, u.z, cs, sn)));
        } else {
            float a = modulate_roughness(s.ay, s.ior);
            vec3 h = to_world(s.at, s.ab, s.n, sample_ggx_normal_finish(a, u.z, cs, sn));
            l = reflect(-v, h);
            l = l - 2 * dot(s.n, l) * s.n;
            is_transmission = true;
        }
        pdf = bsdf_pdf(s, v, l, is_transmission, p);
        return s.alpha * gltf_bsdf(lut, s, v, l, is_transmission ? 2 : 1);
    }
    if (u.x > s.alpha) {
        l = -v; use_mis = false; pdf = (1 - s.alpha); is_transmission = true;
        return v3(1 - s.alpha);
    }
    use_mis = true; is_transmission = false;
    l = sample_cosine_hemisphere(s.n, u.y, u.z);
    pdf = cosine_hemisphere_pdf(s.n, l);
    pdf *= s.alpha;
    return s.alpha * gltf_bsdf(lut, s, v, l, 0);
}

#ifdef PT_LUT_LDS
constexpr int kLightCacheMax = 32;
static __shared__ float4 pt_lds_light[kLightCacheMax * 4];
PT_DEV void spot_cone_terms(float inner_angle, float outer_angle, float& scale, float& offset) {
    scale = fdiv(1.0f, hmax(0.001f, pt_cos(inner_angle) - pt_cos(outer_angle)));
    offset = -pt_cos(outer_angle) * scale;
}
PT_DEV void stage_lights(const SceneRec& sc, int num_of_lights) {
    const uint32_t n = (uint32_t)(num_of_lights < kLightCacheMax ? num_of_lights : kLightCacheMax), n4 = n * 4u;
    if (threadIdx.x < n4) pt_lds_light[threadIdx.x] = gload_f4((const float4*)sc.lights + threadIdx.x);
    __syncthreads();
    if (threadIdx.x < n) {
        float4& last = pt_lds_light[threadIdx.x * 4u + 3u];
        float scale, offset;
        spot_cone_terms(last.x, last.y, scale, offset);
        last.z = scale; last.w = offset;
    }
    __syncthreads();
}
PT_DEV pt_light load_light(const SceneRec& sc, uint32_t li, bool& cone_terms_staged) {
    float4 q[4];
    cone_terms_staged = sc.small_tables || li < (uint32_t)kLightCacheMax;
    if (cone_terms_staged) { const float4* p = pt_lds_light + li * 4u; q[0] = p[0]; q[1] = p[1]; q[2] = p[2]; q[3] = p[3]; }
    else { const float4* p = (const float4*)sc.lights + (size_t)li * 4u; q[0] = gload_f4(p); q[1] = gload_f4(p + 1); q[2] = gload_f4(p + 2); q[3] = gload_f4(p + 3); }
    pt_light l;
    static_assert(sizeof(pt_light) == 64, "pt_light");
    memcpy(&l, q, 64);
    return l;
}
#else
PT_DEV void spot_cone_terms(float inner_angle, float outer_angle, float& scale, float& offset) {
    scale = fdiv(1.0f, hmax(0.001f, pt_cos(inner_angle) - pt_cos(outer_angle)));
    offset = -pt_cos(outer_angle) * scale;
}
PT_DEV void stage_lights(const SceneRec&, int) {}
PT_DEV pt_light load_light(const SceneRec& sc, uint32_t li, bool& cone_terms_staged) { cone_terms_staged = false; return sc.lights[li]; }
#endif
PT_DEV void light_ray(const pt_light& light, vec3 p, vec3& dir, vec3& color, bool cone_terms_staged = false) {
    bool local = light.type == PT_LIGHT_POINT || light.type == PT_LIGHT_SPOT;
    if (local) dir = v3p(light.position) - p;
    else dir = -v3p(light.direction);
    color = v3p(light.color) * light.intensity;
    if (local) {
        float distance = length(dir);
        float falloff = 1.0f;
        if (light.cutoff > 0.0f) falloff = hmax(hmin(1.0f - hpow4(fdiv(distance, light.cutoff)), 1.0f), 0.0f);
        falloff = fdiv(falloff, distance * distance);
        color *= falloff;
    }
    dir = normalize(dir);
    if (light.type == PT_LIGHT_SPOT) {
        float scale, offset;
        if (cone_terms_staged) { float staged[2]; memcpy(staged, light.pad, 8); scale = staged[0]; offset = staged[1]; }
        else spot_cone_terms(light.inner_angle, light.outer_angle, scale, offset);
        float cd = -dot(normalize(v3p(light.direction)), dir);
        float att = saturate(cd * scale + offset);
        att *= att;
        color *= att;
    }
}

PT_DEV void dir_to_face(vec3 d, int& face, float& u, float& v) {
    float ax = fabsf(d.x), ay = fabsf(d.y), az = fabsf(d.z), sc, tc, ma;
    if (ax >= ay && ax >= az) { ma = ax; if (d.x >= 0) { face = 0; sc = -d.z; tc = -d.y; } else { face = 1; sc = d.z; tc = -d.y; } }
    else if (ay >= az) { ma = ay; if (d.y >= 0) { face = 2; sc = d.x; tc = d.z; } else { face = 3; sc = d.x; tc = -d.z; } }
    else { ma = az; if (d.z >= 0) { face = 4; sc = d.x; tc = -d.y; } else { face = 5; sc = -d.x; tc = -d.y; } }
    const float rma_ = frcp_refined(ma);
    u = 0.5f * (fdiv_with(sc, ma, rma_) + 1.0f);
    v = 0.5f * (fdiv_with(tc, ma, rma_) + 1.0f);
}
PT_DEV vec3 cube_texel(const uint16_t* cube, int n, int face, int i, int j) {
    const uint2 q = *(const uint2*)(cube + (((size_t)face * n + j) * n + i) * 4);
    return {half_bits_to_float((uint16_t)(q.x & 0xffff)), half_bits_to_float((uint16_t)(q.x >> 16)), half_bits_to_float((uint16_t)(q.y & 0xffff))};
}
PT_DEV size_t cube_tap_index(int n, int face, int i, int j) {
    if (!(i >= 0 && i < n && j >= 0 && j < n)) {
        vec3 d = cubemap_to_direction(face, fdiv((float)i + 0.5f, (float)n), fdiv((float)j + 0.5f, (float)n));
        float u, v;
        dir_to_face(d, face, u, v);
        i = (int)floorf(u * (float)n); j = (int)floorf(v * (float)n);
        i = min(max(i, 0), n - 1); j = min(max(j, 0), n - 1);
    }
    return ((size_t)face * n + j) * n + i;
}
PT_DEV vec3 cube_unpack(uint2 q) {
    return {half_bits_to_float((uint16_t)(q.x & 0xffff)), half_bits_to_float((uint16_t)(q.x >> 16)), half_bits_to_float((uint16_t)(q.y & 0xffff))};
}
PT_DEV bool cube_footprint(int n, vec3 d, size_t a[4], float w[4]) {
    int face; float u, v;
    dir_to_face(d, face, u, v);
    if (!(u == u) || !(v == v)) return false;
    float x = u * (float)n - 0.5f, y = v * (float)n - 0.5f;
    float fx0 = floorf(x), fy0 = floorf(y);
    float fx = x - fx0, fy = y - fy0;
    int i0 = (int)fx0, j0 = (int)fy0;
    w[0] = (1 - fx) * (1 - fy); w[1] = fx * (1 - fy); w[2] = (1 - fx) * fy; w[3] = fx * fy;
    a[0] = cube_tap_index(n, face, i0, j0); a[1] = cube_tap_index(n, face, i0 + 1, j0);
    a[2] = cube_tap_index(n, face, i0, j0 + 1); a[3] = cube_tap_index(n, face, i0 + 1, j0 + 1);
    return true;
}
PT_DEV vec3 sample_cube(const uint16_t* cube, int n, vec3 d) {
    size_t a[4]; float w[4];
    if (!cube_footprint(n, d, a, w)) return v3(0);
    const size_t a00 = a[0], a10 = a[1], a01 = a[2], a11 = a[3];
    const float w00 = w[0], w10 = w[1], w01 = w[2], w11 = w[3];
    const uint2* texels = (const uint2*)cube;
    const uint2 q00 = gload_u2(texels + a00), q10 = gload_u2(texels + a10), q01 = gload_u2(texels + a01), q11 = gload_u2(texels + a11);
    return cube_unpack(q00) * w00 + cube_unpack(q10) * w10 + cube_unpack(q01) * w01 + cube_unpack(q11) * w11;
}
PT_DEV float imp_load(const EnvRec& e, int level, uint32_t x, uint32_t y) {
    uint32_t n = (uint32_t)e.imp_res >> level;
    if (x >= n || y >= n) return 0.f;
    return e.importance[e.level_offset[level] + (size_t)y * n + x];
}
PT_DEV void importance_step(float ul, float ur, float ll, float lr, float& ux, float& uy, uint32_t& sx, uint32_t& sy) {
    const float left = ul + ll, right = ur + lr, total = left + right;
    const float prob_left = fdiv(left, total);
    const bool go_left = ux < prob_left;
    ux = fdiv(go_left ? ux : ux - prob_left, go_left ? prob_left : 1 - prob_left);
    const float prob_upper = fdiv(go_left ? ul : ur, go_left ? left : right);
    const bool up = uy < prob_upper;
    uy = fdiv(up ? uy : uy - prob_upper, up ? prob_upper : 1 - prob_upper);
    sx = go_left ? 0u : 1u;
    sy = up ? 0u : 1u;
}
#ifdef PT_LUT_LDS
constexpr int kImpLdsLevels = 3;
constexpr uint32_t kImpLdsFloat4 = (16u + 256u + 4096u) / 4u;
static __shared__ float4 pt_lds_imp[kImpLdsFloat4];
PT_DEV void stage_importance_top(const SceneRec& sc) {
    if (sc.has_env) for (uint32_t i = threadIdx.x; i < kImpLdsFloat4; i += 256u) pt_lds_imp[i] = gload_f4((const float4*)sc.env.blocked + i);
    __syncthreads();
}
PT_DEV const float4* importance_lds_top() { return pt_lds_imp; }
PT_DEV void stage_importance_top_into(const SceneRec& sc, float4* dst) {
    if (sc.has_env) for (uint32_t i = threadIdx.x; i < kImpLdsFloat4; i += 256u) dst[i] = gload_f4((const float4*)sc.env.blocked + i);
    __syncthreads();
}
#else
constexpr int kImpLdsLevels = 0;
PT_DEV void stage_importance_top(const SceneRec&) {}
PT_DEV const float4* importance_lds_top() { return nullptr; }
#endif
PT_DEV vec2 sample_importance_map_texel(const EnvRec& e, float ux, float uy, float& pdf, const float4* lds_top, uint32_t& px_out, uint32_t& py_out) {
#ifdef PT_PROBE_NO_DESCENT
    pdf = 1.0f; px_out = py_out = 0;
    return {ux, uy};
#endif
    uint32_t px = 0, py = 0;
    float value = 0.f;
#pragma unroll 1
// ... 59 lines not shown
```

gltf_renderer_amd/csrc/pt_vertex.h:

```cpp
#pragma once
#include "pt_traverse.h"

namespace pt {

struct PathState {
    vec3 beta, thr;
    float prev_pdf;
    int rc, bounce;
    bool prev_mis;
};

struct Followups {
    vec3 add;
    bool overwrite;
    bool q_env, q_light, q_bounce;
    vec3 pend_env, env_dir, pend_light, light_dir, origin_above;
    vec3 b_o, b_d, b_beta, b_thr;
    float b_pdf;
    bool b_mis;
    unsigned counted_shadow;
    uint32_t light_index;
    uint32_t hint_env, hint_light;
};

PT_DEV vec3 miss_environment_color(const SceneRec& sc, float environment_intensity, vec3 dir) {
    return sc.has_env ? environment_intensity * sample_cube(sc.env.cube, sc.env.cube_n, dir) : v3(0);
}
PT_DEV float miss_environment_pdf(const SceneRec& sc, vec3 dir) {
    return sc.has_env ? fdiv(importance_map_pdf(sc.env, square_to_uv(sphere_to_square(normalize(dir)))), 4 * kPi) : 0.f;
}
PT_DEV float miss_mis_weight(float prev_pdf, float env_pdf) { return prev_pdf / (prev_pdf + env_pdf); }

PT_DEV vec3 shade_miss(const SceneRec& sc, const FrameConstants& fc, vec3 dir, const PathState& ps) {
    const uint32_t flags = fc.flags;
    vec3 c;
    if (flags & PT_FLAG_ENVIRONMENT_MAP) {
        c = miss_environment_color(sc, fc.environment_intensity, dir);
        if ((flags & PT_FLAG_ENVIRONMENT_MIS) && ps.prev_mis) c *= miss_mis_weight(ps.prev_pdf, miss_environment_pdf(sc, dir));
    } else c = fc.environment_intensity * v3p(fc.environment_color);
    return ps.beta * c;
}

constexpr int kEnvQueryIn = 8, kEnvQueryOut = 16;
PT_DEV void debug_env_query(const SceneRec& sc, int op, const float* __restrict__ in, float* __restrict__ out, const float4* lds_top) {
    if (op == 0) {
        float pdf;
        uint32_t px, py;
        const vec2 uv = sample_importance_map_texel(sc.env, in[0], in[1], pdf, lds_top, px, py);
        const EnvSample e = environment_light_sample(sc, in[2], in[0], in[1], lds_top);
        out[0] = uv.x; out[1] = uv.y; out[2] = pdf; out[3] = (float)px; out[4] = (float)py;
        out[5] = e.dir.x; out[6] = e.dir.y; out[7] = e.dir.z; out[8] = e.pdf; out[9] = e.color.x; out[10] = e.color.y; out[11] = e.color.z;
    } else if (op == 1) {
        out[0] = importance_map_pdf(sc.env, {in[0], in[1]});
    } else if (op == 2) {
        const vec3 d = {in[0], in[1], in[2]};
        const vec3 c = sample_cube(sc.env.cube, sc.env.cube_n, d);
        out[0] = c.x; out[1] = c.y; out[2] = c.z;
        size_t a[4]; float w[4];
        const bool ok = cube_footprint(sc.env.cube_n, d, a, w);
        const size_t n = (size_t)sc.env.cube_n;
        for (int t = 0; t < 4; t++) {
            out[3 + 3 * t] = ok ? (float)(a[t] / (n * n)) : -1.0f;
            out[4 + 3 * t] = ok ? (float)(a[t] % n) : -1.0f;
            out[5 + 3 * t] = ok ? (float)(a[t] / n % n) : -1.0f;
        }
    } else {
        const vec3 d = {in[0], in[1], in[2]};
        const vec3 c = miss_environment_color(sc, in[4], d);
        const float env_pdf = miss_environment_pdf(sc, d);
        const vec3 m = c * miss_mis_weight(in[3], env_pdf);
        out[0] = c.x; out[1] = c.y; out[2] = c.z; out[3] = env_pdf; out[4] = m.x; out[5] = m.y; out[6] = m.z;
    }
}

#ifdef PT_TIMING
extern __device__ unsigned long long pt_timing[12];
#define PT_TICK(K) { const unsigned long long _now = __builtin_readcyclecounter(); _sec[K] += _now - _t; _t = _now; }
#define PT_TICK_FLUSH() { if (__lane_id() == (unsigned)(__ffsll((long long)__ballot(1)) - 1)) { for (int _k = 0; _k < 11; _k++) atomicAdd(&pt_timing[_k], _sec[_k]); atomicAdd(&pt_timing[11], 1ull); } }
#else
#define PT_TICK(K)
#define PT_TICK_FLUSH()
#endif
template <bool PRE = false>
PT_DEV bool shade_closest_hit(const SceneRec& sc, const FrameConstants& fc, uint32_t seed, uint32_t px, uint32_t py, const Ray& ray, const HitRec& hit,
                              const RawPacket& packet_in, const ShadePacket* packet_at, PathState& ps, Followups& fu, unsigned& taps, const EnvSample* pre = nullptr,
                              const uint32_t* occ_row = nullptr) {
    const uint32_t flags = fc.flags;
    fu.add = v3(0); fu.overwrite = false; fu.counted_shadow = 0; fu.light_index = 0; fu.hint_env = fu.hint_light = 0xffffffffu;
    if (occ_row) fu.hint_env = occ_row[0];
    fu.q_env = fu.q_light = fu.q_bounce = false;
#ifdef PT_TIMING
    unsigned long long _sec[11] = {0, 0, 0, 0, 0, 0, 0, 0, 0, 0, 0}, _t = __builtin_readcyclecounter();
#endif
    const ShadeInst inst = load_shade_inst(sc, raw_packet_inst(packet_in));
    RawPacket packet = packet_in;
    if (__any((inst.streams & (SI_TEXCOORD1 | SI_COLOR)) != 0)) {
        if (inst.streams & (SI_TEXCOORD1 | SI_COLOR)) load_shade_packet_extra(packet, packet_at);
    }
    const PacketVerts pv = unpack_shade_packet(packet);
    const RMat* mat = sc.rmats + inst.material_id;
    const MatHeader mh = material_header(sc, inst.material_id);
    HitGeom va = get_vertex_attributes(sc, inst, pv, v3(1 - hit.u - hit.v, hit.u, hit.v));
    PT_TICK(0)
    const int dbg = fc.debug_output;
    if (dbg >= PT_DEBUG_OUTPUT_HIT_KIND && dbg <= PT_DEBUG_OUTPUT_TEXCOORD_1) {
        vec3 c;
        switch (dbg) {
            case PT_DEBUG_OUTPUT_HIT_KIND: c = hit.front ? v3(1, 0, 0) : v3(0, 1, 0); break;
            case PT_DEBUG_OUTPUT_VERTEX_COLOR: c = xyz(va.color); break;
            case PT_DEBUG_OUTPUT_VERTEX_ALPHA: c = v3(va.color.w); break;
            case PT_DEBUG_OUTPUT_VERTEX_NORMAL: c = (va.n + 1) / 2; break;
            case PT_DEBUG_OUTPUT_VERTEX_TANGENT: c = (va.t + 1) / 2; break;
            case PT_DEBUG_OUTPUT_VERTEX_BITANGENT: c = (va.bt + 1) / 2; break;
            case PT_DEBUG_OUTPUT_TEXCOORD_0: c = v3(va.tc[0].x, va.tc[0].y, 0); break;
            default: c = v3(va.tc[1].x, va.tc[1].y, 0); break;
        }
        fu.add = ps.beta * c;
        return true;
    }
    if (!hit.front) { va.ng = -va.ng; va.n = -va.n; va.t = -va.t; va.tw = -va.tw; }
    const vec3 intersection = ray.o + (ray.d * hit.t);
    const vec3 o_above = offset_ray(va.position, va.ng), o_below = offset_ray(va.position, -va.ng);
    const vec3 view = -normalize(ray.d);
    Surface sp = get_surface(sc, flags, mat, mh, va, view, taps);
    PT_TICK(1)
    if (dbg >= PT_DEBUG_OUTPUT_COLOR && dbg <= PT_DEBUG_OUTPUT_TRANSMISSIVE) {
        vec3 c;
        switch (dbg) {
            case PT_DEBUG_OUTPUT_COLOR: c = sp.albedo; break;
            case PT_DEBUG_OUTPUT_ALPHA: c = v3(sp.alpha); break;
            case PT_DEBUG_OUTPUT_SHADING_NORMAL: c = (sp.n + 1) / 2; break;
            case PT_DEBUG_OUTPUT_SHADING_TANGENT: c = (sp.at + 1) / 2; break;
            case PT_DEBUG_OUTPUT_SHADING_BITANGENT: c = (sp.ab + 1) / 2; break;
            case PT_DEBUG_OUTPUT_METALNESS: c = v3(sp.metalness); break;
            case PT_DEBUG_OUTPUT_ROUGHNESS: c = v3(sqrtf(sp.ay)); break;
            case PT_DEBUG_OUTPUT_SPECULAR: c = v3(sp.spec_factor); break;
            case PT_DEBUG_OUTPUT_SPECULAR_COLOR: c = sp.spec_color; break;
            case PT_DEBUG_OUTPUT_CLEARCOAT: c = v3(sp.clearcoat); break;
            case PT_DEBUG_OUTPUT_CLEARCOAT_ROUGHNESS: c = v3(sp.cc_rough); break;
            case PT_DEBUG_OUTPUT_CLEARCOAT_NORMAL: c = (sp.cc_n + 1) / 2; break;
            default: c = v3(sp.transmissive); break;
        }
        fu.add = ps.beta * c;
        return true;
    }
    if (dbg == PT_DEBUG_OUTPUT_HEMISPHERE_VIEW_SIDE) {
        fu.add = ps.beta * (dot(view, sp.n) > 0 ? v3(0, 1, 0) : v3(1, 0, 0));
        return true;
    }
    const Lobes lobes = lobe_probabilities(sp, view);
    sp.sheen_lh = sp.sheen_sv = 0.0f;
    if (!PT_SHEEN_SKIP || __any(sp.sheen_color.x != 0.0f || sp.sheen_color.y != 0.0f || sp.sheen_color.z != 0.0f)) prepare_sheen(sp, view);
    vec3 c = emissive_of(sc, mat, mh, va.tc, taps, sp.emissive_texel);
    fu.origin_above = o_above;
    PT_TICK(2)
    if (ps.bounce < fc.max_bounces && (flags & PT_FLAG_ENVIRONMENT_MAP) && (flags & PT_FLAG_ENVIRONMENT_MIS)) {
        EnvSample es;
        if (PRE) { es = *pre; ps.rc++; }
        else {
            vec4 r = next_random(px, py, seed, ps.rc);
            es = environment_light_sample(sc, fc.environment_intensity, r.x, r.y, importance_lds_top());
        }
        const float light_pdf = es.pdf;
        const vec3 ldir = es.dir, lcol = es.color;
        PT_TICK(6)
        vec3 contrib = v3(0);
        if (any_gt0(lcol)) {
            float bp = 0;
            vec3 f = evaluate_bsdf(flags, sc.sheen_e, sp, lobes, va.ng, view, ldir, bp);
            float mis = fdiv(light_pdf, light_pdf + bp);
            contrib = (mis * f * lcol) / light_pdf;
        }
        if (flags & PT_FLAG_INDIRECT_ENVIRONMENT_ONLY) c += contrib;
        else {
            fu.pend_env = ps.beta * contrib;
            if (!(fc.cull_null_shadow && fu.pend_env.x == 0.0f && fu.pend_env.y == 0.0f && fu.pend_env.z == 0.0f)) { fu.q_env = true; fu.env_dir = ldir; }
        }
    }
    PT_TICK(3)
    if ((flags & PT_FLAG_POINT_LIGHTS) && fc.num_of_lights > 0) {
        float u = next_random(px, py, seed, ps.rc).x;
        uint32_t li = f2u(u * (float)fc.num_of_lights);
        li = min(li, (uint32_t)(fc.num_of_lights - 1));
        fu.light_index = li;
        if (occ_row) fu.hint_light = occ_row[1u + li % 7u];
        float pdf = fdiv(1.0f, (float)fc.num_of_lights);
        vec3 ldir, lcol;
        bool cone_terms_staged;
        const pt_light light = load_light(sc, li, cone_terms_staged);
        light_ray(light, intersection, ldir, lcol, cone_terms_staged);
        vec3 contrib = v3(0);
        if (any_gt0(lcol)) {
            float bp = 0;
            vec3 f = evaluate_bsdf(flags, sc.sheen_e, sp, lobes, va.ng, view, ldir, bp);
            contrib = (lcol * f) / pdf;
        }
        if ((flags & PT_FLAG_SHADOW_RAYS) && !(flags & PT_FLAG_INDIRECT_ENVIRONMENT_ONLY)) {
            fu.pend_light = ps.beta * contrib;
            if (!(fc.cull_null_shadow && fu.pend_light.x == 0.0f && fu.pend_light.y == 0.0f && fu.pend_light.z == 0.0f)) { fu.q_light = true; fu.light_dir = ldir; }
        }
        else c += contrib;
    }
    PT_TICK(4)
    fu.add = ps.beta * c;
    if (ps.bounce < fc.max_bounces) {
        vec4 r = next_random(px, py, seed, ps.rc);
        bool is_tr = false, use_mis = false;
        float bp = 1;
        vec3 l = v3(0);
        vec3 f = sample_bsdf(flags, sc.sheen_e, sp, lobes, v3(r.x, r.y, r.z), view, l, bp, is_tr, use_mis);
        vec3 weight = bp != 0 ? f / bp : v3(0);
        vec3 throughput = ps.thr * weight;
        if (dbg >= PT_DEBUG_OUTPUT_BOUNCE_DIRECTION && dbg <= PT_DEBUG_BOUNCE_IS_TRANSMISSION) {
            vec3 dc;
            switch (dbg) {
                case PT_DEBUG_OUTPUT_BOUNCE_DIRECTION: dc = 0.5f * (l + 1); break;
                case PT_DEBUG_OUTPUT_BOUNCE_BSDF: dc = f; break;
                case PT_DEBUG_OUTPUT_BOUNCE_PDF: dc = v3(bp); break;
                case PT_DEBUG_OUTPUT_BOUNCE_WEIGHT: dc = weight; break;
                default: dc = is_tr ? v3(0, 1, 0) : v3(1, 0, 0); break;
            }
            fu.counted_shadow = (fu.q_env ? 1u : 0u) + (fu.q_light ? 1u : 0u);
            fu.q_env = fu.q_light = false;
            fu.add = ps.beta * dc;
            fu.overwrite = true;
            return true;
        }
        if (any_gt0(throughput)) {
            float ur = next_random(px, py, seed, ps.rc).x;
            bool cont = ps.bounce < fc.min_bounces;
            if (!cont) {
                float p = clampf(max3(throughput), fc.min_rr, fc.max_rr);
                if (ur < p) { weight = weight / p; cont = true; }
            }
            if (cont) {
                fu.q_bounce = true;
                fu.b_o = is_tr ? o_below : o_above;
                fu.b_d = l;
                fu.b_beta = ps.beta * weight;
                fu.b_thr = throughput * weight;
                fu.b_pdf = bp; fu.b_mis = use_mis;
            }
        }
    }
    PT_TICK(5)
    PT_TICK_FLUSH()
    return false;
}

PT_DEV Ray camera_ray(const FrameConstants& fc, uint32_t seed, uint32_t px, uint32_t py, int& rc) {
    vec4 r = next_random(px, py, seed, rc);
    float jx = r.x - 0.5f, jy = r.y - 0.5f;
    float cx = fdiv((float)px + 0.5f + jx, (float)fc.res_x) * 2 - 1;
    float cy = fdiv((float)py + 0.5f + jy, (float)fc.res_y) * 2 - 1;
    cy = -cy;
    vec4 s = mul4(fc.clip_to_world, vec4{cx, cy, 1, 1});
    vec4 e = mul4(fc.clip_to_world, vec4{cx, cy, 0, 1});
    vec3 o = xyz(s) / s.w;
    vec3 d = xyz(e) / e.w - o;
    Ray ray;
    ray.o = o; ray.tmin = 0; ray.d = normalize(d); ray.tmax = length(d);
    return ray;
}

PT_DEV vec3 sanitize_sample(const FrameConstants& fc, vec3 L) {
    const uint32_t flags = fc.flags;
    if (any_nan(L)) L = (flags & PT_FLAG_SHOW_NAN) ? v3(1, 0, 0) : v3(0);
    if (any_inf(L)) L = (flags & PT_FLAG_SHOW_INF) ? v3(1, 0, 0) : v3(0);
    if (flags & PT_FLAG_LUMINANCE_CLAMP) {
        float lum = luminance(L);
        if (lum > fc.luminance_clamp) L *= fdiv(fc.luminance_clamp, lum);
    }
    return L;
}
PT_DEV float4 blend_sample(float4 h, int accumulated, vec3 L) {
    float blend = fdiv(1.0f, (float)accumulated + 1.0f);
    return make_float4(h.x + blend * (L.x - h.x), h.y + blend * (L.y - h.y), h.z + blend * (L.z - h.z), h.w + blend * (1.0f - h.w));
}
PT_DEV void write_pixel(const FrameConstants& fc, int accumulated, float4* __restrict__ output, uint32_t px, uint32_t py, vec3 L) {
    L = sanitize_sample(fc, L);
    float4* outp = output + ((size_t)py * fc.res_x + px);
    if ((fc.flags & PT_FLAG_ACCUMULATE) && accumulated != 0) *outp = blend_sample(*outp, accumulated, L);
    else *outp = make_float4(L.x, L.y, L.z, 1.0f);
}

PT_DEV uint32_t fast_div(const FastDiv& f, uint32_t x) { return f.d == 1u ? x : (__umulhi(x, f.mul) >> f.shift); }
PT_DEV uint32_t slot_sample(const FrameConstants& fc, uint32_t slot) { return fc.spp > 1 ? fast_div(fc.div_pixel_slots, slot) : 0u; }
PT_DEV uint32_t sample_seed(const FrameConstants& fc, uint32_t sample) { return fc.seed + sample * fc.seed_step; }
PT_DEV bool slot_pixel(const FrameConstants& fc, uint32_t slot, uint32_t& px, uint32_t& py) {
    if (fc.spp > 1) slot -= fast_div(fc.div_pixel_slots, slot) * fc.pixel_slots;
    const uint32_t local_tile = slot >> 8, t = slot & 255;
    const uint32_t tile = fc.tile_rank + local_tile * fc.tile_rank_count;
    const uint32_t ty = fast_div(fc.div_tiles_x, tile), tx = tile - ty * fc.tiles_x;
    const uint32_t wave = t >> 6, lane = t & 63;
    px = tx * PT_TILE + (wave & 1) * 8 + (lane & 7);
    py = ty * PT_TILE + (wave >> 1) * 8 + (lane >> 3);
    return (px < fc.res_x) && (py < fc.res_y) && (tile < fc.tiles_x * fc.tiles_y);
}

PT_DEV void flush_rare(Counters* __restrict__ counters, const LaneStats& st) {
    if (st.overflow) atomicAdd(&counters->stack_overflow, (unsigned long long)st.overflow);
    if (st.deep) atomicAdd(&counters->deep_pushes, (unsigned long long)st.deep);
}
PT_DEV void flush_counters(Counters* __restrict__ counters, uint32_t lane, unsigned n_primary, unsigned n_bounce, unsigned n_shadow, unsigned n_hits,
                           const LaneStats& st, bool occlusion = false) {
    unsigned vals[8] = {n_primary, n_bounce, n_shadow, st.nodes, st.tris, n_hits, st.taps, st.overflow};
#pragma unroll
    for (int k = 0; k < 8; k++) {
        unsigned v = vals[k];
#pragma unroll
        for (int off = 32; off > 0; off >>= 1) v += __shfl_down(v, off, 64);
        const int slot = (occlusion && (k == 3 || k == 4)) ? k + 5 : k;
        if (lane == 0 && v) atomicAdd(((unsigned long long*)counters) + slot, (unsigned long long)v);
    }
}

}
```

gltf_renderer_amd/csrc/pt_wavefront.hip:

```cpp
#define PT_LUT_LDS 1
#include "pt_vertex.h"
#include "pt_host.h"

#ifdef PT_TIMING
namespace pt { __device__ unsigned long long pt_timing[12]; }
extern "C" int pt_debug_read_timing(unsigned long long* out12, int reset) {
    hipDeviceSynchronize();
    hipMemcpyFromSymbol(out12, HIP_SYMBOL(pt::pt_timing), 96);
    if (reset) { unsigned long long z[12] = {0}; hipMemcpyToSymbol(HIP_SYMBOL(pt::pt_timing), z, 96); }
    return 0;
}
#endif
#ifdef PT_UTIL_PROBE
namespace pt { __device__ unsigned long long pt_util[16]; }
extern "C" int pt_debug_read_util(unsigned long long* out16, int reset) {
    hipDeviceSynchronize();
    hipMemcpyFromSymbol(out16, HIP_SYMBOL(pt::pt_util), 128);
    if (reset) { unsigned long long z[16] = {0}; hipMemcpyToSymbol(HIP_SYMBOL(pt::pt_util), z, 128); }
    return 0;
}
#define PT_UTIL(i, v) u_acc[i] += (v)
#else
#define PT_UTIL(i, v)
#endif
namespace pt {

constexpr uint32_t kShards = 256;
constexpr uint32_t kMissTri = 0x7fffffffu;
constexpr uint32_t kNoHint = 0xffffffffu;
#ifndef PT_OCC_CACHE
#define PT_OCC_CACHE 0
#endif
constexpr uint32_t kCounterStride = 16;
constexpr int kCounterArrays = 7;

struct WfBuffers {
    float4* L;
    float4* beta_pdf;
    float4* thr_misc;
    float4* pend;
    float4* ray_o[2];
    float4* ray_d[2];
    float4* q_beta[2];
    float4* q_thr[2];
    float4* hit;
    float4* env_a;
    float4* env_b;
    float4* sh_o;
    float4* sh_d;
    uint32_t* sh_c;
    uint32_t* occ_cache;
    uint32_t* cnt[7];
    uint32_t capacity;
    uint32_t chunks_per_shard;
    uint32_t seg_cap;
    uint32_t blocks_per_shard;
    uint32_t gen_region_tiles, gen_rounds;
};


#ifndef PT_STREAM
#define PT_STREAM 1
#endif
typedef float nt_v4f __attribute__((ext_vector_type(4)));
PT_DEV float4 nt_load(const float4& p) { const nt_v4f v = __builtin_nontemporal_load((const nt_v4f*)&p); return make_float4(v.x, v.y, v.z, v.w); }
PT_DEV uint32_t nt_load(const uint32_t& p) { return __builtin_nontemporal_load(&p); }
PT_DEV void nt_store(float4& p, const float4 v) { nt_v4f q; q.x = v.x; q.y = v.y; q.z = v.z; q.w = v.w; __builtin_nontemporal_store(q, (nt_v4f*)&p); }
PT_DEV void nt_store(uint32_t& p, const uint32_t v) { __builtin_nontemporal_store(v, &p); }
#if PT_STREAM >= 1
#define QLD(p) nt_load(p)
#define QST(p, v) nt_store((p), (v))
#else
#define QLD(p) (p)
#define QST(p, v) ((p) = (v))
#endif
#if PT_STREAM >= 2
#define SLD(p) nt_load(p)
#define SST(p, v) nt_store((p), (v))
#else
#define SLD(p) (p)
#define SST(p, v) ((p) = (v))
#endif

#ifndef PT_STATE_BY_SHARD
#define PT_STATE_BY_SHARD 0
#endif
PT_DEV uint32_t state_index(const WfBuffers& wf, uint32_t slot) {
#if PT_STATE_BY_SHARD
    const uint32_t c = slot >> 8;
    return (((c & (kShards - 1u)) * wf.chunks_per_shard + (c >> 8)) << 8) | (slot & 255u);
#else
    return slot;
#endif
}
#define SIDX(s) state_index(wf, (s))
#define PEND_ENV(s) wf.pend[2u * SIDX(s)]
#define PEND_LIGHT(s) wf.pend[2u * SIDX(s) + 1u]
constexpr int kRcAfterCamera = 1;
#ifndef PT_BT_IN_QUEUE
#define PT_BT_IN_QUEUE 1
#endif
#ifndef PT_FIRST_VERTEX_STATELESS
#define PT_FIRST_VERTEX_STATELESS 1
#endif

PT_DEV uint32_t queue_push(uint32_t* counter, bool pred) {
    const unsigned long long m = __ballot(pred);
    if (m == 0) return 0;
    const uint32_t lane = threadIdx.x & 63;
    const uint32_t rank = __popcll(m & ((1ull << lane) - 1ull));
    uint32_t base = 0;
    const int leader = __ffsll((long long)m) - 1;
    if ((int)lane == leader) base = atomicAdd(counter, (uint32_t)__popcll(m));
    base = __shfl(base, leader, 64);
    return base + rank;
}

struct ShardView { uint32_t shard, member, stride; };
PT_DEV ShardView shard_view(const WfBuffers& wf) {
    ShardView v;
    v.shard = blockIdx.x % kShards;
    v.member = blockIdx.x / kShards;
    v.stride = wf.blocks_per_shard * kBlock;
    return v;
}

constexpr uint32_t kXcds = 8;
#ifndef PT_GEN_XCD_BANDS
#define PT_GEN_XCD_BANDS 0
#endif
__global__ __launch_bounds__(kBlock) void k_wf_generate(FrameConstants fc, WfBuffers wf, Counters* __restrict__ counters) {
    const ShardView sv = shard_view(wf);
    const uint32_t per_xcd = gridDim.x / kXcds;
    const uint32_t xcd = blockIdx.x % kXcds, member = blockIdx.x / kXcds;
    uint32_t first_tile = xcd * wf.gen_region_tiles;
    uint32_t n_tiles = first_tile < fc.my_tiles ? min(wf.gen_region_tiles, fc.my_tiles - first_tile) : 0u;
#if PT_GEN_XCD_BANDS == 2
    const bool columns = fc.tile_rank_count == 1;
    const uint32_t c0 = xcd * fc.tiles_x / kXcds, band_w = (xcd + 1u) * fc.tiles_x / kXcds - c0;
    if (columns) n_tiles = band_w * fc.tiles_y;
#endif
    unsigned n_primary = 0;
    for (uint32_t rnd = 0; rnd < wf.gen_rounds; rnd++) {
#if PT_GEN_XCD_BANDS
        const uint32_t q = rnd * per_xcd + member;
        const uint32_t tile_in_region = q / fc.spp, sample = q - tile_in_region * fc.spp;
        uint32_t tile = first_tile + tile_in_region;
#if PT_GEN_XCD_BANDS == 2
        if (columns) { const uint32_t brow = band_w ? tile_in_region / band_w : 0u; tile = brow * fc.tiles_x + c0 + (tile_in_region - brow * band_w); }
#endif
        const uint32_t slot = sample * fc.pixel_slots + tile * kBlock + threadIdx.x;
        uint32_t px = 0, py = 0;
        const bool valid = tile_in_region < n_tiles && slot_pixel(fc, slot, px, py);
#else
        const uint32_t slot = (rnd * gridDim.x + blockIdx.x) * kBlock + threadIdx.x;
        const uint32_t sample = slot_sample(fc, slot);
        uint32_t px = 0, py = 0;
        const bool valid = slot < wf.capacity && slot_pixel(fc, slot, px, py);
#endif
        int rc = 0;
        Ray ray;
        ray.o = v3(0); ray.d = v3(0, 0, 1); ray.tmin = 0; ray.tmax = 0;
        if (valid) ray = camera_ray(fc, sample_seed(fc, sample), px, py, rc);
        const uint32_t idx = queue_push(wf.cnt[0] + sv.shard * kCounterStride, valid);
        if (valid) {
            const size_t e = (size_t)sv.shard * wf.seg_cap + idx;
            QST(wf.ray_o[0][e], make_float4(ray.o.x, ray.o.y, ray.o.z, ray.tmax));
            QST(wf.ray_d[0][e], make_float4(ray.d.x, ray.d.y, ray.d.z, __uint_as_float(slot)));
#if !PT_FIRST_VERTEX_STATELESS
            SST(wf.L[SIDX(slot)], make_float4(0, 0, 0, 0));
#if PT_BT_IN_QUEUE
            QST(wf.q_beta[0][e], make_float4(1, 1, 1, 0));
            QST(wf.q_thr[0][e], make_float4(1, 1, 1, __uint_as_float((uint32_t)rc)));
#else
            SST(wf.beta_pdf[SIDX(slot)], make_float4(1, 1, 1, 0));
            SST(wf.thr_misc[SIDX(slot)], make_float4(1, 1, 1, __uint_as_float((uint32_t)rc)));
#endif
#endif
            n_primary++;
        }
    }
    LaneStats st = {0, 0, 0, 0};
    flush_counters(counters, threadIdx.x & 63, n_primary, 0, 0, 0, st);
}

#ifndef PT_REFILL
#define PT_REFILL 32
#endif
PT_DEV int shadow_counter(int bounce) { return (bounce & 1) ? 5 : 2; }
template <bool COUNT, int MODE>
PT_DEV void trace_persistent(const SceneRec& sc, const WfBuffers& wf, int* my_stack, const ShardView& sv, int cur, uint32_t rf_closest, uint32_t rmask,
                             uint32_t flags, LaneStats& st, float shadow_tmax = 0.0f, bool use_occ_cache = false) {
    const uint32_t n = wf.cnt[cur][sv.shard * kCounterStride];
    uint32_t* head = wf.cnt[MODE == 0 ? 3 : 4] + sv.shard * kCounterStride;
    const size_t base = MODE == 0 ? (size_t)sv.shard * wf.seg_cap : (size_t)sv.shard * wf.seg_cap * 2;
    const uint32_t lane = threadIdx.x & 63;
    int spill[kStackSpill];
    Trav t;
    t.cur = kTravDone; t.sp = 0;
    bool has = false, exhausted = (n == 0);
    uint32_t entry = 0, slot_bits = 0, occ_at = kNoHint;
#ifdef PT_UTIL_PROBE
    unsigned long long u_acc[8] = {0, 0, 0, 0, 0, 0, 0, 0};
#endif
    for (;;) {
        const unsigned long long idle = __ballot(!has);
        const uint32_t nidle = (uint32_t)__popcll(idle);
        if (!exhausted && nidle >= PT_REFILL) {
            const int leader = __ffsll((long long)idle) - 1;
            uint32_t first = 0;
            if ((int)lane == leader) first = atomicAdd(head, nidle);
// ... 44 lines not shown
#if PT_POSTPONE_LEAF
            if (has && t.cur < 0 && t.cur != kTravDone && t.post == kTravDone && t.sp > 0) { t.post = t.cur; trav_pop(t, sc, my_stack, spill); }
#endif
            const unsigned long long at_node = __ballot(has && t.cur >= 0);
            if (at_node == 0) break;
            if (PT_NODE_MIN > 1 && (int)__popcll(at_node) < PT_NODE_MIN && __ballot(has && t.cur < 0 && (t.cur != kTravDone || t.post != kTravDone)) != 0) break;
            PT_UTIL(0, 1); PT_UTIL(1, __popcll(at_node)); PT_UTIL(6, __popcll(__ballot(has)));
            if (has && t.cur >= 0) trav_node_step<COUNT, MODE == 0>(t, sc, my_stack, spill, st);
        }
#ifdef PT_UTIL_PROBE
        { const unsigned long long at_leaf = __ballot(has && ((t.cur != kTravDone && t.cur < 0) || t.post != kTravDone)); if (at_leaf) { PT_UTIL(2, 1); PT_UTIL(3, __popcll(at_leaf)); } }
#endif
#if PT_POSTPONE_LEAF
#pragma nounroll
        for (int pass = 0; pass < 2; pass++) {
            const bool first_pass = pass == 0;
            const bool mine = has && (first_pass ? t.post != kTravDone : (t.cur != kTravDone && t.cur < 0));
            if (!__any(mine)) continue;
            if (mine) {
                const int keep = t.cur;
                if (first_pass) { t.cur = t.post; t.post = kTravDone; }
                trav_leaf_step<COUNT>(t, sc, my_stack, spill, st, first_pass, keep);
            }
        }
#else
        if (has && t.cur != kTravDone && t.cur < 0) trav_leaf_step<COUNT>(t, sc, my_stack, spill, st);
#endif
        if (has && t.cur == kTravDone) {
            if (MODE == 0) {
                const uint32_t bits = t.committed ? ((uint32_t)t.best.tri | (t.best.front ? 0x80000000u : 0u)) : kMissTri;
                QST(wf.hit[base + entry], make_float4(t.best.t, t.best.u, t.best.v, __uint_as_float(bits)));
            } else {
                const float tr = t.committed ? t.transmission : 1.0f;
                const uint32_t slot = slot_bits & 0x7fffffffu;
#if PT_OCC_CACHE
                if (use_occ_cache && occ_at != kNoHint && t.committed) wf.occ_cache[occ_at] = (uint32_t)t.best.tri;
#endif
                float* w = (slot_bits >> 31) ? &PEND_LIGHT(slot).w : &PEND_ENV(slot).w;
                *w = tr;
            }
            has = false;
        }
    }
#ifdef PT_UTIL_PROBE
    if (lane == 0) for (int k = 0; k < 7; k++) atomicAdd(&pt_util[MODE * 8 + k], u_acc[k]);
#endif
}

#ifndef PT_ENV_PREPASS
#define PT_ENV_PREPASS 1
#endif

PT_DEV bool env_prepass_wanted(const SceneRec& sc, const FrameConstants& fc, int vertex_bounce) {
    return PT_ENV_PREPASS && sc.has_env && (fc.flags & PT_FLAG_ENVIRONMENT_MAP) && (fc.flags & PT_FLAG_ENVIRONMENT_MIS) && vertex_bounce < fc.max_bounces;
}
PT_DEV void env_prepass(const SceneRec& sc, const FrameConstants& fc, const WfBuffers& wf, int* stack_lds, const ShardView& sv, int cur, bool first_vertex) {
    static_assert((size_t)kStackLds * kBlock * sizeof(int) >= (size_t)kImpLdsFloat4 * sizeof(float4), "the traversal stack's LDS must hold the importance pyramid's coarse levels");
    float4* top = (float4*)stack_lds;
    stage_importance_top_into(sc, top);
    const uint32_t n = wf.cnt[cur][sv.shard * kCounterStride];
    const size_t base = (size_t)sv.shard * wf.seg_cap;
    for (uint32_t i = sv.member * kBlock + threadIdx.x; i < n; i += sv.stride) {
        const uint32_t slot = QLD(*((const uint32_t*)&wf.ray_d[cur][base + i] + 3));
        int rc = kRcAfterCamera;
#if PT_BT_IN_QUEUE
        if (!(PT_FIRST_VERTEX_STATELESS && first_vertex)) rc = (int)(QLD(*((const uint32_t*)&wf.q_thr[cur][base + i] + 3)) & 0xffffu);
#else
        if (!(PT_FIRST_VERTEX_STATELESS && first_vertex)) rc = (int)(SLD(*((const uint32_t*)&wf.thr_misc[SIDX(slot)] + 3)) & 0xffffu);
#endif
        uint32_t px, py;
        slot_pixel(fc, slot, px, py);
        const vec4 r = next_random(px, py, sample_seed(fc, slot_sample(fc, slot)), rc);
        const EnvSample e = environment_light_sample(sc, fc.environment_intensity, r.x, r.y, top);
        QST(wf.env_a[base + i], make_float4(e.dir.x, e.dir.y, e.dir.z, e.pdf));
        QST(wf.env_b[base + i], make_float4(e.color.x, e.color.y, e.color.z, 0.0f));
    }
    __syncthreads();
}

#ifndef PT_TRACE_WAVES
#define PT_TRACE_WAVES 1
#endif
#ifndef PT_LATE_GRID
#define PT_LATE_GRID 1
#endif
#ifndef PT_FUSE_TRAVERSAL
#define PT_FUSE_TRAVERSAL 1
#endif
constexpr uint32_t kTravFlagMask = PT_FLAG_CULL_BACKFACE | PT_FLAG_ALPHA_SHADOWS | PT_FLAG_INDIRECT_ENVIRONMENT_ONLY;
#ifndef PT_TRAV_SPECIALISE
#define PT_TRAV_SPECIALISE 1
#endif
template <bool COUNT, bool DEFAULTS>
__global__ __launch_bounds__(kBlock, PT_TRACE_WAVES) void k_wf_trace(SceneRec sc, FrameConstants fc, WfBuffers wf, int cur, int bounce, uint32_t rf, uint32_t rmask, Counters* __restrict__ counters) {
    if (DEFAULTS) { rf = 0; rmask = 0xff; }
    __shared__ int s_stack[kStackLds * kBlock];
    stage_luts(sc);
    const ShardView sv = shard_view(wf);
    if (env_prepass_wanted(sc, fc, bounce)) env_prepass(sc, fc, wf, s_stack, sv, cur, bounce == 0);
    if (sv.member == 0 && threadIdx.x == 0) { wf.cnt[cur ^ 1][sv.shard * kCounterStride] = 0; wf.cnt[shadow_counter(bounce)][sv.shard * kCounterStride] = 0; wf.cnt[6][sv.shard * kCounterStride] = 0; }
    LaneStats st = {0, 0, 0, 0};
    trace_persistent<COUNT, 0>(sc, wf, s_stack + threadIdx.x, sv, cur, rf, rmask, 0, st);
    if (COUNT) { flush_counters(counters, threadIdx.x & 63, 0, 0, 0, 0, st); if (st.deep) atomicAdd(&counters->deep_pushes, (unsigned long long)st.deep); }
    else if (st.overflow | st.deep) flush_rare(counters, st);
}

template <bool COUNT, bool DEFAULTS>
__global__ __launch_bounds__(kBlock, PT_TRACE_WAVES) void k_wf_traverse(SceneRec sc, FrameConstants fc, WfBuffers wf, int nxt, int bounce, uint32_t rf, uint32_t rmask, uint32_t flags,
                                                                        Counters* __restrict__ counters) {
    if (DEFAULTS) { rf = 0; rmask = 0xff; flags &= ~kTravFlagMask; }
    __shared__ int s_stack[kStackLds * kBlock];
    stage_luts(sc);
    const ShardView sv = shard_view(wf);
    if (env_prepass_wanted(sc, fc, bounce + 1)) env_prepass(sc, fc, wf, s_stack, sv, nxt, false);
    if (sv.member == 0 && threadIdx.x == 0) { wf.cnt[nxt ^ 1][sv.shard * kCounterStride] = 0; wf.cnt[shadow_counter(bounce + 1)][sv.shard * kCounterStride] = 0; wf.cnt[6][sv.shard * kCounterStride] = 0; }
    LaneStats st_shadow = {0, 0, 0, 0}, st = {0, 0, 0, 0};
    trace_persistent<COUNT, 1>(sc, wf, s_stack + threadIdx.x, sv, shadow_counter(bounce), 0, 0xff, flags, st_shadow, fc.max_ray_length, wf.occ_cache != nullptr && bounce == 0);
    trace_persistent<COUNT, 0>(sc, wf, s_stack + threadIdx.x, sv, nxt, rf, rmask, 0, st);
    if (COUNT) {
        flush_counters(counters, threadIdx.x & 63, 0, 0, 0, 0, st_shadow, true); flush_counters(counters, threadIdx.x & 63, 0, 0, 0, 0, st);
        if (st.deep | st_shadow.deep) atomicAdd(&counters->deep_pushes, (unsigned long long)st.deep + st_shadow.deep);
    } else if (st.overflow | st_shadow.overflow | st.deep | st_shadow.deep) { flush_rare(counters, st); flush_rare(counters, st_shadow); }
}

PT_DEV void apply_pending(const WfBuffers& wf, uint32_t slot, uint32_t pf, vec3& L) {
    const float4 pe = SLD(PEND_ENV(slot)), pl = SLD(PEND_LIGHT(slot));
    if ((pf & 1u) && pe.w > 0.0f) L += v3(pe.x, pe.y, pe.z) * pe.w;
    if ((pf & 2u) && pl.w > 0.0f) L += v3(pl.x, pl.y, pl.z) * pl.w;
}

#ifndef PT_DEFER_FEATURES
#define PT_DEFER_FEATURES 0
#endif
#ifndef PT_DEFER_FLUSH
#define PT_DEFER_FLUSH 60
#endif
#ifndef PT_DEFER_MAJORITY
#define PT_DEFER_MAJORITY 4
#endif
constexpr uint32_t kNoHeld = 0xffffffffu;
constexpr int kDeferFlush = PT_DEFER_FLUSH;
constexpr uint32_t kDeferMajority = PT_DEFER_MAJORITY;
PT_DEV bool material_is_rare(const SceneRec& sc, uint32_t inst_id) {
    const ShadeInst inst = load_shade_inst(sc, inst_id);
    const MatHeader mh = material_header(sc, inst.material_id);
    bool rare = false;
    if (PT_DEFER_FEATURES & 1) rare = rare || mh.sheen_color_factor.x != 0.0f || mh.sheen_color_factor.y != 0.0f || mh.sheen_color_factor.z != 0.0f;
    if (PT_DEFER_FEATURES & 2) rare = rare || mh.clearcoat_factor != 0.0f;
    if (PT_DEFER_FEATURES & 4) rare = rare || mh.transmission_factor != 0.0f;
    if (PT_DEFER_FEATURES & 8) rare = rare || mh.anisotropy_strength != 0.0f;
    return rare;
}

#ifndef PT_SHADE_DYNAMIC
#define PT_SHADE_DYNAMIC 1
#endif
#ifndef PT_SHADE_WAVES
#define PT_SHADE_WAVES 2
#endif
constexpr uint32_t kShadeFlagMask = PT_FLAG_MATERIAL_DIFFUSE_WHITE | PT_FLAG_MATERIAL_MIS | PT_FLAG_MATERIAL_USE_GEOMETRIC_NORMALS | PT_FLAG_SHADING_NORMAL_ADAPTATION |
                                    PT_FLAG_ENVIRONMENT_MAP | PT_FLAG_ENVIRONMENT_MIS | PT_FLAG_INDIRECT_ENVIRONMENT_ONLY | PT_FLAG_POINT_LIGHTS | PT_FLAG_SHADOW_RAYS;
constexpr uint32_t kShadeSpecialised = 0x80000000u;
constexpr uint32_t kShadeDefaultsNoLights = PT_FLAG_SHADOW_RAYS | PT_FLAG_ENVIRONMENT_MAP | PT_FLAG_ENVIRONMENT_MIS | PT_FLAG_MATERIAL_MIS | PT_FLAG_SHADING_NORMAL_ADAPTATION;
constexpr uint32_t kShadeDefaults = kShadeDefaultsNoLights | PT_FLAG_POINT_LIGHTS;
#ifndef PT_SHADE_SPECIALISE
#define PT_SHADE_SPECIALISE 1
#endif
template <uint32_t SPECIAL, bool SMALL>
__global__ __launch_bounds__(kBlock, PT_SHADE_WAVES) void k_wf_shade(SceneRec sc_in, FrameConstants fc_in, WfBuffers wf, int cur, int bounce, Counters* __restrict__ counters) {
    SceneRec sc = sc_in; sc.small_tables = SMALL ? 1u : 0u;
    FrameConstants fc = fc_in;
    if (SPECIAL) { fc.flags = (fc_in.flags & ~kShadeFlagMask) | (SPECIAL & kShadeFlagMask); fc.debug_output = PT_DEBUG_OUTPUT_NONE; }
    {
        const ShardView sv0 = shard_view(wf);
        if (sv0.member != 0 && sv0.member * kBlock >= wf.cnt[cur][sv0.shard * kCounterStride]) return;
    }
    stage_luts(sc);
    stage_tangent_lut(sc);
#if !PT_ENV_PREPASS
    stage_importance_top(sc);
#endif
    stage_lights(sc, fc.num_of_lights);
    stage_instances(sc);
    stage_materials(sc);
    const ShardView sv = shard_view(wf);
    const uint32_t n = wf.cnt[cur][sv.shard * kCounterStride];
    const int nxt = cur ^ 1;
    const size_t base = (size_t)sv.shard * wf.seg_cap, sbase = (size_t)sv.shard * wf.seg_cap * 2;
    uint32_t* cnt_next = wf.cnt[nxt] + sv.shard * kCounterStride;
    uint32_t* cnt_shadow = wf.cnt[shadow_counter(bounce)] + sv.shard * kCounterStride;
    if (sv.member == 0 && threadIdx.x == 0) { wf.cnt[3][sv.shard * kCounterStride] = 0; wf.cnt[4][sv.shard * kCounterStride] = 0; }
    unsigned n_bounce = 0, n_shadow = 0, n_hits = 0;
    LaneStats st = {0, 0, 0, 0};
#if PT_SHADE_DYNAMIC
    uint32_t* shade_head = wf.cnt[6] + sv.shard * kCounterStride;
    const uint32_t lane64 = threadIdx.x & 63u;
    uint32_t chunk = 0;
    if (lane64 == 0) chunk = atomicAdd(shade_head, 64u);
    chunk = (uint32_t)__builtin_amdgcn_readfirstlane((int)chunk);
    const bool defer_on = PT_DEFER_FEATURES != 0 && fc.defer_rare != 0;
    uint32_t held = kNoHeld;
    __shared__ uint32_t s_hand[kBlock];
    uint32_t* hand = s_hand + (threadIdx.x & ~63u);
    for (;;) {
        const bool more = chunk < n;
        const unsigned long long held_mask = __ballot(held != kNoHeld);
        if (!more && held_mask == 0) break;
        const bool flush = defer_on && (!more || __popcll(held_mask) >= kDeferFlush);
        uint32_t next_chunk = 0;
        if (!flush && lane64 == 0) next_chunk = atomicAdd(shade_head, 64u);
        const uint32_t i = flush ? held : chunk + lane64;
        const bool active = flush ? held != kNoHeld : i < n;
        if (flush) held = kNoHeld;
#else
    const bool flush = true;
    const unsigned long long held_mask = 0; uint32_t held = kNoHeld; uint32_t* hand = nullptr; const uint32_t lane64 = threadIdx.x & 63u;
    const uint32_t rounds = (n + sv.stride - 1) / sv.stride;
    for (uint32_t rnd = 0; rnd < rounds; rnd++) {
        const uint32_t i = rnd * sv.stride + sv.member * kBlock + threadIdx.x;
        const bool active = i < n;
#endif
        bool push_env = false, push_light = false, push_bounce = false;
        uint32_t occ_pixel = kNoHint;
        Followups fu;
        fu.q_env = fu.q_light = fu.q_bounce = false;
        uint32_t slot = 0;
        PathState ps;
        ps.beta = v3(0); ps.thr = v3(0); ps.prev_pdf = 0; ps.rc = 0; ps.bounce = 0; ps.prev_mis = false;
        float4 o = make_float4(0, 0, 0, 0), d = o, h = o, bp = o, tm = o, Lq = o, pe = o, pl = o;
        uint32_t hb = kMissTri;
        const ShadePacket* packet_at = sc.shade;
        RawPacket packet;
#if PT_ENV_PREPASS
        EnvSample es;
        es.dir = v3(0, 0, 1); es.pdf = 1; es.color = v3(0);
#endif
        const bool with_state = !(PT_FIRST_VERTEX_STATELESS && bounce == 0);
        if (active) {
            o = QLD(wf.ray_o[cur][base + i]); d = QLD(wf.ray_d[cur][base + i]); h = QLD(wf.hit[base + i]);
#if PT_ENV_PREPASS
            if (env_prepass_wanted(sc, fc, bounce)) {
                const float4 ea = QLD(wf.env_a[base + i]), eb = QLD(wf.env_b[base + i]);
                es.dir = v3(ea.x, ea.y, ea.z); es.pdf = ea.w; es.color = v3(eb.x, eb.y, eb.z);
            }
#endif
            slot = __float_as_uint(d.w);
            hb = __float_as_uint(h.w);
#ifdef PT_PROBE_NO_PACKET
            packet_at = sc.shade + (hb == kMissTri ? 0u : (hb & 63u));
#else
            packet_at = sc.shade + (hb == kMissTri ? 0u : (hb & 0x7fffffffu));
#endif
            packet = load_shade_packet_raw(packet_at);
            if (with_state) {
#if PT_BT_IN_QUEUE
                bp = QLD(wf.q_beta[cur][base + i]); tm = QLD(wf.q_thr[cur][base + i]);
#else
                bp = SLD(wf.beta_pdf[SIDX(slot)]); tm = SLD(wf.thr_misc[SIDX(slot)]);
#endif
#ifndef PT_PROBE_NO_LP
                Lq = SLD(wf.L[SIDX(slot)]); pe = SLD(PEND_ENV(slot)); pl = SLD(PEND_LIGHT(slot));
#endif
            }
        }
        bool set_aside = false;
#if PT_SHADE_DYNAMIC
        if (defer_on && !flush) {
            const bool rare = active && hb != kMissTri && material_is_rare(sc, raw_packet_inst(packet));
            const unsigned long long R = __ballot(rare), F = ~held_mask;
            const uint32_t nR = (uint32_t)__popcll(R), nF = (uint32_t)__popcll(F);
            if (nR != 0 && nR < kDeferMajority) {
                const unsigned long long below = (1ull << lane64) - 1ull;
                const uint32_t rr = (uint32_t)__popcll(R & below), rf = (uint32_t)__popcll(F & below);
                if (rare && rr < nF) { hand[rr] = i; set_aside = true; }
                __builtin_amdgcn_fence(__ATOMIC_RELEASE, "wavefront");
                __builtin_amdgcn_wave_barrier();
                __builtin_amdgcn_fence(__ATOMIC_ACQUIRE, "wavefront");
                if (held == kNoHeld && rf < min(nR, nF)) held = hand[rf];
            }
        }
#endif
        if (active && !set_aside) {
            Ray ray;
            ray.o = v3(o.x, o.y, o.z); ray.tmin = 0; ray.d = v3(d.x, d.y, d.z); ray.tmax = o.w;
            vec3 L = v3(0);
            ps.beta = v3(1); ps.prev_pdf = 0; ps.thr = v3(1); ps.rc = kRcAfterCamera; ps.bounce = 0; ps.prev_mis = false;
            if (with_state) {
                const uint32_t misc = __float_as_uint(tm.w);
                ps.beta = v3(bp.x, bp.y, bp.z); ps.prev_pdf = bp.w; ps.thr = v3(tm.x, tm.y, tm.z);
                ps.rc = (int)(misc & 0xffffu); ps.bounce = (int)((misc >> 16) & 0x7fffu); ps.prev_mis = (misc >> 31) != 0;
#ifndef PT_PROBE_NO_LP
                L = v3(Lq.x, Lq.y, Lq.z);
                const uint32_t pfb = __float_as_uint(Lq.w);
                if ((pfb & 1u) && pe.w > 0.0f) L += v3(pe.x, pe.y, pe.z) * pe.w;
                if ((pfb & 2u) && pl.w > 0.0f) L += v3(pl.x, pl.y, pl.z) * pl.w;
#endif
            }
            uint32_t pf = 0;
            if (hb == kMissTri) L += shade_miss(sc, fc, ray.d, ps);
            else {
                HitRec hit;
                hit.t = h.x; hit.u = h.y; hit.v = h.z; hit.tri = (int)(hb & 0x7fffffffu); hit.front = (hb >> 31) != 0;
                uint32_t px, py;
                slot_pixel(fc, slot, px, py);
                n_hits++;
#if PT_OCC_CACHE
                if (bounce == 0 && wf.occ_cache) occ_pixel = (py * fc.res_x + px) * 8u;
                const uint32_t* occ_row = occ_pixel != kNoHint ? wf.occ_cache + occ_pixel : nullptr;
#else
                const uint32_t* occ_row = nullptr;
#endif
#if PT_ENV_PREPASS
                const bool done = shade_closest_hit<true>(sc, fc, sample_seed(fc, slot_sample(fc, slot)), px, py, ray, hit, packet, packet_at, ps, fu, st.taps, &es, occ_row);
#else
                const bool done = shade_closest_hit(sc, fc, sample_seed(fc, slot_sample(fc, slot)), px, py, ray, hit, packet, packet_at, ps, fu, st.taps, nullptr, occ_row);
#endif
                if (fu.overwrite) L = v3(0);
                L += fu.add;
                n_shadow += fu.counted_shadow;
                if (!done) {
                    push_env = fu.q_env; push_light = fu.q_light; push_bounce = fu.q_bounce;
#ifndef PT_PROBE_NO_LP
                    if (push_env) { pf |= 1u; SST(PEND_ENV(slot), make_float4(fu.pend_env.x, fu.pend_env.y, fu.pend_env.z, 0.0f)); }
                    if (push_light) { pf |= 2u; SST(PEND_LIGHT(slot), make_float4(fu.pend_light.x, fu.pend_light.y, fu.pend_light.z, 0.0f)); }
#endif
                }
            }
#ifndef PT_PROBE_NO_LP
            SST(wf.L[SIDX(slot)], make_float4(L.x, L.y, L.z, __uint_as_float(pf)));
#endif
        }
        uint32_t at_env = kNoHint, at_light = kNoHint, hint_env = kNoHint, hint_light = kNoHint;
#if PT_OCC_CACHE
        if (bounce == 0 && occ_pixel != kNoHint) {
            at_env = occ_pixel; at_light = occ_pixel + 1u + fu.light_index % 7u;
            hint_env = fu.hint_env; hint_light = fu.hint_light;
        }
#endif
        const uint32_t ie = queue_push(cnt_shadow, push_env);
        if (push_env) {
            QST(wf.sh_o[sbase + ie], make_float4(fu.origin_above.x, fu.origin_above.y, fu.origin_above.z, __uint_as_float(slot)));
            QST(wf.sh_d[sbase + ie], make_float4(fu.env_dir.x, fu.env_dir.y, fu.env_dir.z, __uint_as_float(hint_env)));
#if PT_OCC_CACHE
            if (bounce == 0 && wf.occ_cache) QST(wf.sh_c[sbase + ie], at_env);
#endif
            n_shadow++;
        }
        const uint32_t il = queue_push(cnt_shadow, push_light);
        if (push_light) {
            QST(wf.sh_o[sbase + il], make_float4(fu.origin_above.x, fu.origin_above.y, fu.origin_above.z, __uint_as_float(slot | 0x80000000u)));
            QST(wf.sh_d[sbase + il], make_float4(fu.light_dir.x, fu.light_dir.y, fu.light_dir.z, __uint_as_float(hint_light)));
#if PT_OCC_CACHE
            if (bounce == 0 && wf.occ_cache) QST(wf.sh_c[sbase + il], at_light);
#endif
            n_shadow++;
        }
        const uint32_t ib = queue_push(cnt_next, push_bounce);
        if (push_bounce) {
            QST(wf.ray_o[nxt][base + ib], make_float4(fu.b_o.x, fu.b_o.y, fu.b_o.z, fc.max_ray_length));
            QST(wf.ray_d[nxt][base + ib], make_float4(fu.b_d.x, fu.b_d.y, fu.b_d.z, __uint_as_float(slot)));
            const uint32_t misc = ((uint32_t)ps.rc & 0xffffu) | ((uint32_t)(ps.bounce + 1) << 16) | (fu.b_mis ? 0x80000000u : 0u);
#if PT_BT_IN_QUEUE
            QST(wf.q_beta[nxt][base + ib], make_float4(fu.b_beta.x, fu.b_beta.y, fu.b_beta.z, fu.b_pdf));
            QST(wf.q_thr[nxt][base + ib], make_float4(fu.b_thr.x, fu.b_thr.y, fu.b_thr.z, __uint_as_float(misc)));
#else
            SST(wf.beta_pdf[SIDX(slot)], make_float4(fu.b_beta.x, fu.b_beta.y, fu.b_beta.z, fu.b_pdf));
            SST(wf.thr_misc[SIDX(slot)], make_float4(fu.b_thr.x, fu.b_thr.y, fu.b_thr.z, __uint_as_float(misc)));
#endif
            n_bounce++;
        }
#if PT_SHADE_DYNAMIC
        if (!flush) chunk = (uint32_t)__builtin_amdgcn_readfirstlane((int)next_chunk);
#endif
    }
    flush_counters(counters, threadIdx.x & 63, 0, n_bounce, n_shadow, n_hits, st);
}

template <bool COUNT>
__global__ __launch_bounds__(kBlock, PT_TRACE_WAVES) void k_wf_shadow(SceneRec sc, WfBuffers wf, int bounce, uint32_t flags, float tmax, Counters* __restrict__ counters) {
    __shared__ int s_stack[kStackLds * kBlock];
    stage_luts(sc);
    const ShardView sv = shard_view(wf);
    LaneStats st = {0, 0, 0, 0};
    trace_persistent<COUNT, 1>(sc, wf, s_stack + threadIdx.x, sv, shadow_counter(bounce), 0, 0xff, flags, st, tmax, wf.occ_cache != nullptr && bounce == 0);
    if (COUNT) { flush_counters(counters, threadIdx.x & 63, 0, 0, 0, 0, st, true); if (st.deep) atomicAdd(&counters->deep_pushes, (unsigned long long)st.deep); }
    else if (st.overflow | st.deep) flush_rare(counters, st);
}

__global__ __launch_bounds__(kBlock) void k_debug_sample_texture_wf(SceneRec sc, const uint32_t* __restrict__ mat_slot, const float* __restrict__ tc,
                                                                 uint32_t n, float* __restrict__ out, int32_t* __restrict__ taps) {
    stage_luts(sc);
    stage_materials(sc);
    const uint32_t i = blockIdx.x * kBlock + threadIdx.x;
    if (i >= n) return;
    const vec2 uv[2] = {{tc[4 * i], tc[4 * i + 1]}, {tc[4 * i + 2], tc[4 * i + 3]}};
    int32_t t5[5];
    const vec4 r = debug_sample_query(sc, mat_slot[2 * i], (int)mat_slot[2 * i + 1], uv, t5);
    out[4 * i] = r.x; out[4 * i + 1] = r.y; out[4 * i + 2] = r.z; out[4 * i + 3] = r.w;
    for (int c = 0; c < 5; c++) taps[5 * i + c] = t5[c];
}
void launch_debug_sample_texture_wf(const SceneRec& sc, const uint32_t* d_mat_slot, const float* d_tc, uint32_t n, float* d_out, int32_t* d_taps, hipStream_t stream) {
    if (n == 0) return;
    hipLaunchKernelGGL(k_debug_sample_texture_wf, dim3((n + kBlock - 1) / kBlock), dim3(kBlock), 0, stream, sc, d_mat_slot, d_tc, n, d_out, d_taps);
}
__global__ __launch_bounds__(kBlock) void k_debug_env_query_wf(SceneRec sc, int op, const float* __restrict__ in, uint32_t n, float* __restrict__ out) {
    __shared__ int s_stack[kStackLds * kBlock];
    static_assert((size_t)kStackLds * kBlock * sizeof(int) >= (size_t)kImpLdsFloat4 * sizeof(float4), "the traversal stack's LDS must hold the importance pyramid's coarse levels");
    float4* top = (float4*)s_stack;
    stage_importance_top_into(sc, top);
    const uint32_t i = blockIdx.x * kBlock + threadIdx.x;
    if (i >= n) return;
    debug_env_query(sc, op, in + (size_t)kEnvQueryIn * i, out + (size_t)kEnvQueryOut * i, top);
}
void launch_debug_env_query_wf(const SceneRec& sc, int op, const float* d_in, uint32_t n, float* d_out, hipStream_t stream) {
    if (n == 0) return;
    hipLaunchKernelGGL(k_debug_env_query_wf, dim3((n + kBlock - 1) / kBlock), dim3(kBlock), 0, stream, sc, op, d_in, n, d_out);
}
__global__ __launch_bounds__(kBlock) void k_wf_resolve(FrameConstants fc, WfBuffers wf, float4* __restrict__ output) {
    const uint32_t pslot = blockIdx.x * kBlock + threadIdx.x;
    uint32_t px, py;
    if (pslot >= fc.pixel_slots || !slot_pixel(fc, pslot, px, py)) return;
    float4* outp = output + ((size_t)py * fc.res_x + px);
    const bool accumulate = (fc.flags & PT_FLAG_ACCUMULATE) != 0;
    float4 pixel = make_float4(0, 0, 0, 0);
    if (accumulate && fc.accumulated_frames != 0) pixel = *outp;
    for (uint32_t k = 0; k < fc.spp; k++) {
        const uint32_t slot = k * fc.pixel_slots + pslot;
        float4 Lq = SLD(wf.L[SIDX(slot)]);
        vec3 L = v3(Lq.x, Lq.y, Lq.z);
        apply_pending(wf, slot, __float_as_uint(Lq.w), L);
        L = sanitize_sample(fc, L);
        const int accumulated = fc.accumulated_frames + (int)k;
        pixel = (accumulate && accumulated != 0) ? blend_sample(pixel, accumulated, L) : make_float4(L.x, L.y, L.z, 1.0f);
    }
    *outp = pixel;
}

static uint32_t blocks_per_shard_for(int stage_blocks) {
    uint32_t b = (uint32_t)(stage_blocks > 0 ? stage_blocks : 1536) / kShards;
    return b < 1 ? 1 : b;
}
static uint32_t gen_region_tiles_for(const FrameConstants& fc) {
#if PT_GEN_XCD_BANDS == 2
    if (fc.tile_rank_count == 1) return ((fc.tiles_x + kXcds - 1) / kXcds) * fc.tiles_y;
#endif
    return (fc.my_tiles + kXcds - 1) / kXcds;
}
static uint32_t gen_rounds_for(const FrameConstants& fc, uint32_t blocks_per_shard) {
    const uint32_t per_xcd = kShards * blocks_per_shard / kXcds;
    const uint32_t pairs = gen_region_tiles_for(fc) * fc.spp;
    return (pairs + per_xcd - 1) / per_xcd;
}
static uint32_t seg_cap_for(const FrameConstants& fc, uint32_t blocks_per_shard) {
    return gen_rounds_for(fc, blocks_per_shard) * blocks_per_shard * kBlock;
}

static uint32_t chunks_per_shard_for(size_t slots) { return (uint32_t)(((slots + kBlock - 1) / kBlock + kShards - 1) / kShards); }
static size_t state_slots_for(size_t slots) { return (size_t)chunks_per_shard_for(slots) * kShards * kBlock; }

size_t wavefront_workspace_bytes(const FrameConstants& fc, int stage_blocks) {
    const uint32_t bps = blocks_per_shard_for(stage_blocks);
    const size_t slots = state_slots_for((size_t)fc.my_tiles * kBlock * fc.spp);
    const size_t q = (size_t)kShards * seg_cap_for(fc, bps);
    return slots * (5 * 16) + q * (4 * 16 + 4 * 16 + 16 + 2 * 16 + 2 * 2 * 16 + (PT_OCC_CACHE ? 2 * 4 : 0)) + kCounterArrays * kShards * kCounterStride * 4 + 52 * 256;
}

static WfBuffers carve(void* base, const FrameConstants& fc, int stage_blocks) {
    const uint32_t slots = fc.my_tiles * kBlock * fc.spp;
    const size_t state_slots = state_slots_for(slots);
    WfBuffers wf;
    wf.chunks_per_shard = chunks_per_shard_for(slots);
    char* p = (char*)base;
    auto take = [&](size_t bytes) { char* r = p; p += (bytes + 255) & ~(size_t)255; return r; };
    wf.blocks_per_shard = blocks_per_shard_for(stage_blocks);
    wf.seg_cap = seg_cap_for(fc, wf.blocks_per_shard);
    wf.gen_region_tiles = gen_region_tiles_for(fc);
    wf.gen_rounds = gen_rounds_for(fc, wf.blocks_per_shard);
    const size_t q = (size_t)kShards * wf.seg_cap;
    for (int k = 0; k < kCounterArrays; k++) wf.cnt[k] = (uint32_t*)take((size_t)kShards * kCounterStride * 4);
    wf.L = (float4*)take(state_slots * 16);
    wf.beta_pdf = (float4*)take(state_slots * 16);
    wf.thr_misc = (float4*)take(state_slots * 16);
    wf.pend = (float4*)take(state_slots * 32);
    for (int k = 0; k < 2; k++) { wf.ray_o[k] = (float4*)take(q * 16); wf.ray_d[k] = (float4*)take(q * 16); }
    for (int k = 0; k < 2; k++) { wf.q_beta[k] = (float4*)take(q * 16); wf.q_thr[k] = (float4*)take(q * 16); }
    wf.hit = (float4*)take(q * 16);
    wf.env_a = (float4*)take(q * 16);
    wf.env_b = (float4*)take(q * 16);
    wf.sh_o = (float4*)take(q * 2 * 16);
    wf.sh_d = (float4*)take(q * 2 * 16);
    wf.sh_c = PT_OCC_CACHE ? (uint32_t*)take(q * 2 * 4) : nullptr;
    wf.occ_cache = nullptr;
    wf.capacity = slots;
    return wf;
}

int traversal_stack_capacity() { return kStackLds + kStackSpill; }
size_t traversal_grid_lanes(int stage_blocks) { return (size_t)kShards * blocks_per_shard_for(stage_blocks) * kBlock; }

hipError_t launch_wavefront(const SceneRec& sc, const FrameConstants& fc, float4* output, Counters* counters, bool count, void* workspace,
                            int stage_blocks, StageTimers* timers, hipStream_t stream, uint32_t* occ_cache) {
    if (timers) timers->used = 0;
    if (fc.my_tiles == 0) return hipSuccess;
    auto event_at = [&](size_t i) -> hipEvent_t {
        while (timers->ev.size() <= i) { hipEvent_t e = nullptr; if (hipEventCreate(&e) != hipSuccess) return nullptr; timers->ev.push_back(e); }
        return timers->ev[i];
    };
    auto mark = [&](int kind) {
        if (!timers) return;
        const size_t k = timers->used;
        hipEvent_t ev = event_at(k + 1);
        if (!ev) return;
        if (timers->kind.size() < k + 1) timers->kind.resize(k + 1);
        timers->kind[k] = (uint8_t)kind;
        hipEventRecord(ev, stream);
        timers->used = k + 1;
    };
    const uint32_t slots = fc.my_tiles * kBlock * fc.spp;
    WfBuffers wf = carve(workspace, fc, stage_blocks);
    wf.occ_cache = PT_OCC_CACHE ? occ_cache : nullptr;
    hipError_t e = hipMemsetAsync(wf.cnt[0], 0, (size_t)kCounterArrays * kShards * kCounterStride * 4, stream);
    if (e) return e;
    const dim3 block(kBlock), full(fc.my_tiles), stage(kShards * wf.blocks_per_shard);
    if (timers) { hipEvent_t ev = event_at(0); if (ev) hipEventRecord(ev, stream); else timers = nullptr; }
    hipLaunchKernelGGL(k_wf_generate, stage, block, 0, stream, fc, wf, counters);
    mark(STAGE_GENERATE);
    const uint32_t flags = fc.flags;
    const int iterations = fc.debug_output != PT_DEBUG_OUTPUT_NONE ? 1 : fc.max_bounces + 1;
    auto ray_flags = [&](int b, uint32_t& rf, uint32_t& rmask) {
        rmask = 0xff;
        if (b == 0) rf = (flags & PT_FLAG_CULL_BACKFACE) ? RF_CULL_BACK : 0;
        else {
            rf = (flags & PT_FLAG_CULL_BACKFACE) ? RF_CULL_FRONT : 0;
            rmask = (flags & PT_FLAG_INDIRECT_ENVIRONMENT_ONLY) ? 0 : 0xff;
        }
    };
    const bool trav_defaults = PT_TRAV_SPECIALISE && (flags & kTravFlagMask) == 0;
    auto launch_trace = [&](dim3 grid, const WfBuffers& w, int cur, int b, uint32_t rf, uint32_t rmask) {
        if (trav_defaults) { if (count) hipLaunchKernelGGL((k_wf_trace<true, true>), grid, block, 0, stream, sc, fc, w, cur, b, rf, rmask, counters);
                             else hipLaunchKernelGGL((k_wf_trace<false, true>), grid, block, 0, stream, sc, fc, w, cur, b, rf, rmask, counters); }
        else { if (count) hipLaunchKernelGGL((k_wf_trace<true, false>), grid, block, 0, stream, sc, fc, w, cur, b, rf, rmask, counters);
               else hipLaunchKernelGGL((k_wf_trace<false, false>), grid, block, 0, stream, sc, fc, w, cur, b, rf, rmask, counters); }
    };
    auto launch_traverse = [&](dim3 grid, const WfBuffers& w, int nxt, int b, uint32_t rf, uint32_t rmask) {
        if (trav_defaults) { if (count) hipLaunchKernelGGL((k_wf_traverse<true, true>), grid, block, 0, stream, sc, fc, w, nxt, b, rf, rmask, flags, counters);
                             else hipLaunchKernelGGL((k_wf_traverse<false, true>), grid, block, 0, stream, sc, fc, w, nxt, b, rf, rmask, flags, counters); }
        else { if (count) hipLaunchKernelGGL((k_wf_traverse<true, false>), grid, block, 0, stream, sc, fc, w, nxt, b, rf, rmask, flags, counters);
               else hipLaunchKernelGGL((k_wf_traverse<false, false>), grid, block, 0, stream, sc, fc, w, nxt, b, rf, rmask, flags, counters); }
    };
    const uint32_t shade_bits = flags & kShadeFlagMask;
    const int shade_variant = (!PT_SHADE_SPECIALISE || fc.debug_output != PT_DEBUG_OUTPUT_NONE) ? 0 : (shade_bits == kShadeDefaults ? 1 : (shade_bits == kShadeDefaultsNoLights ? 2 : 0));
    const bool small_tables = PT_SHADE_SPECIALISE && sc.n_instances <= kInstCacheMax && sc.n_materials <= kMatCacheMax && fc.num_of_lights <= kLightCacheMax;
    auto launch_shade = [&](dim3 grid, const WfBuffers& w, int cur, int b) {
        if (small_tables && shade_variant == 1) hipLaunchKernelGGL((k_wf_shade<kShadeSpecialised | kShadeDefaults, true>), grid, block, 0, stream, sc, fc, w, cur, b, counters);
        else if (small_tables && shade_variant == 2) hipLaunchKernelGGL((k_wf_shade<kShadeSpecialised | kShadeDefaultsNoLights, true>), grid, block, 0, stream, sc, fc, w, cur, b, counters);
        else if (small_tables) hipLaunchKernelGGL((k_wf_shade<0u, true>), grid, block, 0, stream, sc, fc, w, cur, b, counters);
        else hipLaunchKernelGGL((k_wf_shade<0u, false>), grid, block, 0, stream, sc, fc, w, cur, b, counters);
    };
#if PT_LATE_GRID
    static const int env_shade_bps = getenv("MIPT_SHADE_BPS") ? atoi(getenv("MIPT_SHADE_BPS")) : 0;
    static const int env_trace_bps = getenv("MIPT_TRACE_BPS") ? atoi(getenv("MIPT_TRACE_BPS")) : 0;
    auto grid_of = [&](int b) -> dim3 {
        uint32_t bps = wf.blocks_per_shard;
        if (b > fc.min_bounces + 1) {
            double expected = (double)slots;
            for (int k = fc.min_bounces + 1; k < b; k++) expected *= 0.25;
            const uint32_t want = expected >= 1200000.0 ? 6u : (expected >= 400000.0 ? 3u : 2u);
            bps = want < bps ? want : bps;
        }
        return dim3(kShards * bps);
    };
#define PT_GRID(b) grid_of(b)
#define PT_WF(b) wf_for(b)
    auto wf_for = [&](int b) { WfBuffers w = wf; w.blocks_per_shard = grid_of(b).x / kShards; return w; };
    auto cap = [&](dim3 g, int env) { if (env > 0 && (uint32_t)env * kShards < g.x) g.x = (uint32_t)env * kShards; return g; };
    auto wf_of = [&](dim3 g) { WfBuffers w = wf; w.blocks_per_shard = g.x / kShards; return w; };
#else
#define PT_GRID(b) stage
#define PT_WF(b) wf
#endif
#if PT_FUSE_TRAVERSAL
    {
        uint32_t rf, rmask;
        ray_flags(0, rf, rmask);
#if PT_LATE_GRID
        const dim3 g0 = cap(stage, env_trace_bps);
        launch_trace(g0, wf_of(g0), 0, 0, rf, rmask);
#else
        launch_trace(stage, wf, 0, 0, rf, rmask);
#endif
        mark(STAGE_TRACE);
    }
    for (int b = 0; b < iterations; b++) {
        const int cur = b & 1;
#if PT_LATE_GRID
        const dim3 gs = cap(grid_of(b), env_shade_bps), gt = cap(grid_of(b), env_trace_bps);
        const WfBuffers ws = wf_of(gs), wt = wf_of(gt);
#else
        const dim3 gs = stage, gt = stage;
        const WfBuffers& ws = wf; const WfBuffers& wt = wf;
#endif
        launch_shade(gs, ws, cur, b);
        mark(STAGE_SHADE);
        uint32_t rf, rmask;
        ray_flags(b + 1, rf, rmask);
        if (b + 1 < iterations) {
            launch_traverse(gt, wt, cur ^ 1, b, rf, rmask);
        } else {
            if (count) hipLaunchKernelGGL(k_wf_shadow<true>, gt, block, 0, stream, sc, wt, b, flags, fc.max_ray_length, counters);
            else hipLaunchKernelGGL(k_wf_shadow<false>, gt, block, 0, stream, sc, wt, b, flags, fc.max_ray_length, counters);
        }
        mark(STAGE_SHADOW);
    }
#else
    for (int b = 0; b < iterations; b++) {
        const int cur = b & 1;
        uint32_t rf, rmask;
        ray_flags(b, rf, rmask);
        launch_trace(stage, wf, cur, b, rf, rmask);
        mark(STAGE_TRACE);
        launch_shade(stage, wf, cur, b);
        mark(STAGE_SHADE);
        if (count) hipLaunchKernelGGL(k_wf_shadow<true>, stage, block, 0, stream, sc, wf, b, flags, fc.max_ray_length, counters);
        else hipLaunchKernelGGL(k_wf_shadow<false>, stage, block, 0, stream, sc, wf, b, flags, fc.max_ray_length, counters);
        mark(STAGE_SHADOW);
    }
#endif
    hipLaunchKernelGGL(k_wf_resolve, full, block, 0, stream, fc, wf, output);
    mark(STAGE_RESOLVE);
    return hipGetLastError();
}

}
```

Before: 6107.

## Add lean shade kernel variants that compile out specular and sheen material paths

The host now inspects every instance's material and, when no material uses the specular, clearcoat or other extension slots (and optionally has no sheen), launches a k_wf_shade instantiation templated on LEAN that compiles out those texture fetches and BSDF branches. When the lean path is forced but some materials do not qualify, non-lean hits are pushed into an aside queue. A second, general shade pass with a reduced grid then processes that queue. The goal is lower register pressure and fewer instructions in the shade kernel for simple glTF scenes. The cost is a per-frame host scan over instances, extra workspace, and more kernel instantiations.

```diff
diff --git a/gltf_renderer_amd/csrc/mipt_api.hip b/gltf_renderer_amd/csrc/mipt_api.hip
--- a/gltf_renderer_amd/csrc/mipt_api.hip
+++ b/gltf_renderer_amd/csrc/mipt_api.hip
@@ -81,6 +81,8 @@
     int samples_per_trace = 1;
     bool cull_null_shadow = false;
     bool counters_enabled = false;
+    int shade_path_forced = -1;
+    int shade_path_last = SHADE_PATH_GENERAL, shade_second_passes = 0;
 
     float previous_world_to_clip[16] = {0};
     int accumulated_frames = 0;
@@ -100,6 +102,30 @@
     } while (0)
 
 namespace {
+
+bool material_is_lean(const RMat& m, bool sheen) {
+    const uint32_t bm = m.bound_mask;
+    if (((bm & ((1u << SLOT_COUNT) - 1u)) >> SLOT_SPECULAR) != 0u) return false;
+    return sheen || (m.sheen_color_factor[0] == 0.0f && m.sheen_color_factor[1] == 0.0f && m.sheen_color_factor[2] == 0.0f &&
+                     ((bm & RM_TRIO) != 0u || (bm & ((1u << SLOT_OCCLUSION) - 1u)) == 0u));
+}
+
+int choose_shade_path(const pt_ctx* ctx, const SceneRec& sc, const FrameConstants& fc) {
+    if (!wavefront_lean_available(sc, fc)) return SHADE_PATH_GENERAL;
+    bool lean = true, lean_sheen = true;
+    for (const InstanceRec& r : ctx->instances) {
+        const int mid = r.gpu.material_id;
+        const bool valid = mid >= 0 && mid < (int)ctx->rmats_host.size();
+        lean = lean && valid && material_is_lean(ctx->rmats_host[mid], false);
+        lean_sheen = lean_sheen && valid && material_is_lean(ctx->rmats_host[mid], true);
+    }
+    static const int env = [] { const char* e = getenv("MIPT_SHADE_PATH"); return e ? atoi(e) : -1; }();
+    const int path = ctx->shade_path_forced >= 0 ? ctx->shade_path_forced : env;
+    if (path < 0 || path >= SHADE_PATH_COUNT) return lean ? SHADE_PATH_LEAN : (lean_sheen ? SHADE_PATH_LEAN_SHEEN : SHADE_PATH_GENERAL);
+    if (path == SHADE_PATH_LEAN && !lean) return SHADE_PATH_LEAN_ASIDE;
+    if (path == SHADE_PATH_LEAN_SHEEN && !lean_sheen) return SHADE_PATH_LEAN_SHEEN_ASIDE;
+    return path;
+}
 
 hipError_t staged_upload(pt_ctx* ctx, void* dst, const void* src, size_t bytes) {
     if (bytes == 0) return hipSuccess;
@@ -373,6 +399,7 @@
             }
             HIPOK(hipEventRecord(ctx->ev_trace[0], ctx->stream));
             if (ctx->kernel_mode == PT_MODE_MEGAKERNEL) {
+                ctx->shade_path_last = SHADE_PATH_GENERAL; ctx->shade_second_passes = 0;
                 for (int k = 0; k < batch; k++) {
                     FrameConstants fk = fc;
                     fk.seed = fc.seed + (uint32_t)k * fc.seed_step;
@@ -383,7 +410,8 @@
                 fc.spp = (uint32_t)batch;
                 if ((unsigned long long)fc.pixel_slots * fc.spp > 0x7fffffffull) return ctx->fail(PT_ERR_CAPACITY, "sample batch too large for this resolution");
                 const int stage_blocks = ctx->stage_blocks > 0 ? ctx->stage_blocks : stage_blocks_for((size_t)fc.pixel_slots * fc.spp);
-                size_t need = wavefront_workspace_bytes(fc, stage_blocks);
+                const int shade_path = choose_shade_path(ctx, sc, fc);
+                size_t need = wavefront_workspace_bytes(fc, stage_blocks, shade_path != SHADE_PATH_GENERAL);
                 if (need > ctx->workspace_cap) {
                     HIPOK(hipStreamSynchronize(ctx->stream));
                     hipFree(ctx->d_workspace); ctx->d_workspace = nullptr; ctx->workspace_cap = 0;
@@ -403,7 +431,9 @@
                     occ = ctx->d_occ;
                 }
                 HIPOK(launch_wavefront(sc, fc, (float4*)ep->output, ctx->d_counters, ctx->counters_enabled, ctx->d_workspace, stage_blocks,
-                                       ctx->stage_timing ? &ctx->timers : nullptr, ctx->stream, occ));
+                                       ctx->stage_timing ? &ctx->timers : nullptr, ctx->stream, occ, shade_path));
+                ctx->shade_path_last = shade_path;
+                ctx->shade_second_passes = (shade_path == SHADE_PATH_LEAN_ASIDE || shade_path == SHADE_PATH_LEAN_SHEEN_ASIDE) ? (fc.debug_output != PT_DEBUG_OUTPUT_NONE ? 1 : fc.max_bounces + 1) : 0;
             }
             HIPOK(hipGetLastError());
             HIPOK(hipEventRecord(ctx->ev_trace[1], ctx->stream));
@@ -783,6 +813,20 @@
     int n = 0;
     if (ctx) for (const RMat& r : ctx->rmats_host) n += (r.bound_mask & RM_TRIO) ? 1 : 0;
     return n;
+}
+
+extern "C" int pt_debug_shade_path(pt_ctx* ctx, int path) {
+    if (!ctx) return PT_ERR_INVALID_ARGUMENT;
+    if (path < -1 || path >= SHADE_PATH_COUNT) return ctx->fail(PT_ERR_INVALID_ARGUMENT, "pt_debug_shade_path: path " + std::to_string(path));
+    ctx->shade_path_forced = path;
+    return PT_OK;
+}
+extern "C" int pt_debug_shade_path_stats(pt_ctx* ctx, long long* out3) {
+    if (!ctx || !out3) return PT_ERR_INVALID_ARGUMENT;
+    ENTER(ctx);
+    out3[0] = ctx->shade_path_last; out3[1] = ctx->shade_second_passes;
+    out3[2] = (ctx->have_trace && ctx->shade_path_last != SHADE_PATH_GENERAL && ctx->d_workspace) ? (long long)wavefront_aside_total(ctx->d_workspace, ctx->stream) : 0;
+    return PT_OK;
 }
 
 extern "C" int pt_debug_interleaved_emissive(const pt_ctx* ctx) {
diff --git a/gltf_renderer_amd/csrc/pt_host.h b/gltf_renderer_amd/csrc/pt_host.h
--- a/gltf_renderer_amd/csrc/pt_host.h
+++ b/gltf_renderer_amd/csrc/pt_host.h
@@ -96,9 +96,12 @@
 void launch_debug_env_query_mk(const SceneRec& sc, int op, const float* d_in, uint32_t n, float* d_out, hipStream_t stream);
 void launch_debug_intersect(const SceneRec& sc, const float* d_rays, uint32_t n, uint32_t rf, int mode, float* d_out, hipStream_t stream);
 void launch_megakernel(const SceneRec& sc, const FrameConstants& fc, float4* output, Counters* counters, bool count, hipStream_t stream);
-size_t wavefront_workspace_bytes(const FrameConstants& fc, int stage_blocks);
+enum { SHADE_PATH_GENERAL = 0, SHADE_PATH_LEAN = 1, SHADE_PATH_LEAN_ASIDE = 2, SHADE_PATH_LEAN_SHEEN = 3, SHADE_PATH_LEAN_SHEEN_ASIDE = 4, SHADE_PATH_COUNT };
+bool wavefront_lean_available(const SceneRec& sc, const FrameConstants& fc);
+size_t wavefront_workspace_bytes(const FrameConstants& fc, int stage_blocks, bool aside);
+uint64_t wavefront_aside_total(const void* workspace, hipStream_t stream);
 hipError_t launch_wavefront(const SceneRec& sc, const FrameConstants& fc, float4* output, Counters* counters, bool count, void* workspace,
-                            int stage_blocks, StageTimers* timers, hipStream_t stream, uint32_t* occ_cache);
+                            int stage_blocks, StageTimers* timers, hipStream_t stream, uint32_t* occ_cache, int shade_path);
 
 size_t radix_sort_temp_bytes(size_t n);
 hipError_t radix_sort_pairs_u64_u32(void* temp, uint64_t* keys_in, uint64_t* keys_out, uint32_t* vals_in, uint32_t* vals_out, size_t n, hipStream_t stream);
diff --git a/gltf_renderer_amd/csrc/pt_shading.h b/gltf_renderer_amd/csrc/pt_shading.h
--- a/gltf_renderer_amd/csrc/pt_shading.h
+++ b/gltf_renderer_amd/csrc/pt_shading.h
@@ -457,6 +457,8 @@
     uint32_t a00, a10, a01, a11, n00, n10, n01, n11, m00, m10, m01, m11;
     vec4 emissive;
 };
+constexpr int kLeanNoSheen = 1, kLeanSheen = 2;
+template <int LEAN = 0>
 PT_DEV PbrTexels fetch_pbr_texels(const SceneRec& sc, uint32_t mid, const MatHeader& h, const vec2 tc[2]) {
     PbrTexels f;
     f.emissive = vec4{0, 0, 0, 0};
@@ -487,7 +489,7 @@
             }
         }
     }
-    if (__any(!trio)) {
+    if (LEAN != kLeanNoSheen && __any(!trio)) {
         if (!trio) {
             const RTex t_nrm = material_slot012(sc, mid, SLOT_NORMAL), t_mr = material_slot012(sc, mid, SLOT_METALLIC_ROUGHNESS);
             k_nrm = texture_taps(t_nrm, tc); k_mr = texture_taps(t_mr, tc);
@@ -519,9 +521,10 @@
     f.m00 = m00; f.m10 = m10; f.m01 = m01; f.m11 = m11;
     return f;
 }
+template <int LEAN = 0>
 PT_DEV Surface get_surface(const SceneRec& sc, uint32_t flags, const RMat* m, const MatHeader& h, const HitGeom& a, vec3 view, unsigned& taps) {
     Surface s;
-    const PbrTexels f = fetch_pbr_texels(sc, (uint32_t)(m - sc.rmats), h, a.tc);
+    const PbrTexels f = fetch_pbr_texels<LEAN>(sc, (uint32_t)(m - sc.rmats), h, a.tc);
     s.emissive_texel = xyz(f.emissive);
     const TexTaps &k_alb = f.k_alb, &k_nrm = f.k_nrm, &k_mr = f.k_mr;
     const uint32_t a00 = f.a00, a10 = f.a10, a01 = f.a01, a11 = f.a11, n00 = f.n00, n10 = f.n10, n01 = f.n01, n11 = f.n11, m00 = f.m00, m10 = f.m10, m01 = f.m01, m11 = f.m11;
@@ -551,7 +554,7 @@
     float sheen_rough = h.sheen_roughness_factor;
     s.transmissive = h.transmission_factor;
 #ifndef PT_PROBE_BASE_ONLY
-    if ((h.bound_mask & ((1u << SLOT_COUNT) - 1u)) >> SLOT_SPECULAR) {
+    if (LEAN == 0 && ((h.bound_mask & ((1u << SLOT_COUNT) - 1u)) >> SLOT_SPECULAR)) {
         if (slot_bound(h.bound_mask, SLOT_SPECULAR)) s.spec_factor *= sample_slot(sc, m, SLOT_SPECULAR, a.tc, taps).w;
         if (slot_bound(h.bound_mask, SLOT_SPECULAR_COLOR)) s.spec_color = s.spec_color * xyz(sample_slot(sc, m, SLOT_SPECULAR_COLOR, a.tc, taps));
         if (slot_bound(h.bound_mask, SLOT_CLEARCOAT)) s.clearcoat *= sample_slot(sc, m, SLOT_CLEARCOAT, a.tc, taps).x;
@@ -694,6 +697,7 @@
 }
 PT_DEV float modulate_roughness(float a, float ior) { return clampf(lerpf(0, a, saturate(2 * (ior - 1))), kMinRoughness, 1.0f); }
 
+template <int LEAN = 0>
 PT_DEV vec3 gltf_bsdf(const float* lut, const Surface& s, vec3 v, vec3 l, int mode) {
     vec3 n = s.n;
     vec3 h = normalize(v + l);
@@ -734,7 +738,7 @@
 #define PT_SHEEN_SKIP 1
 #endif
     const bool no_sheen = s.sheen_color.x == 0.0f && s.sheen_color.y == 0.0f && s.sheen_color.z == 0.0f;
-    if (PT_SHEEN_SKIP && !__any(!no_sheen)) {
+    if (LEAN == kLeanNoSheen || (PT_SHEEN_SKIP && !__any(!no_sheen))) {
         const float sin2h = 1 - hl.z * hl.z;
         const float layer = (refl && !(sin2h >= 0.0f)) ? __builtin_nanf("") : 0.0f;
         material = v3(layer) + material * 1.0f;
@@ -864,6 +868,7 @@
     pdf += p.diffuse * cosp;
     return pdf;
 }
+template <int LEAN = 0>
 PT_DEV vec3 evaluate_bsdf(uint32_t flags, const float* lut, const Surface& s, const Lobes& p, vec3 ng, vec3 v, vec3 l, float& pdf) {
     if (flags & PT_FLAG_MATERIAL_DIFFUSE_WHITE) {
         float ndl = saturate(dot(s.n, l));
@@ -873,13 +878,14 @@
     if (flags & PT_FLAG_MATERIAL_MIS) {
         bool is_transmission = (dot(ng, l) * dot(ng, v)) < 0;
         pdf = bsdf_pdf(s, v, l, is_transmission, p);
-        return s.alpha * gltf_bsdf(lut, s, v, l, is_transmission ? 2 : 1);
+        return s.alpha * gltf_bsdf<LEAN>(lut, s, v, l, is_transmission ? 2 : 1);
     }
     float ndl = saturate(dot(s.n, l));
     pdf = fdiv(ndl, kPi);
     pdf *= s.alpha;
-    return s.alpha * gltf_bsdf(lut, s, v, l, 0);
-}
+    return s.alpha * gltf_bsdf<LEAN>(lut, s, v, l, 0);
+}
+template <int LEAN = 0>
 PT_DEV vec3 sample_bsdf(uint32_t flags, const float* lut, const Surface& s, const Lobes& p, vec3 u, vec3 v, vec3& l, float& pdf,
                         bool& is_transmission, bool& use_mis) {
     if (flags & PT_FLAG_MATERIAL_DIFFUSE_WHITE) {
@@ -929,7 +935,7 @@
             is_transmission = true;
         }
         pdf = bsdf_pdf(s, v, l, is_transmission, p);
-        return s.alpha * gltf_bsdf(lut, s, v, l, is_transmission ? 2 : 1);
+        return s.alpha * gltf_bsdf<LEAN>(lut, s, v, l, is_transmission ? 2 : 1);
     }
     if (u.x > s.alpha) {
         l = -v; use_mis = false; pdf = (1 - s.alpha); is_transmission = true;
@@ -939,7 +945,7 @@
     l = sample_cosine_hemisphere(s.n, u.y, u.z);
     pdf = cosine_hemisphere_pdf(s.n, l);
     pdf *= s.alpha;
-    return s.alpha * gltf_bsdf(lut, s, v, l, 0);
+    return s.alpha * gltf_bsdf<LEAN>(lut, s, v, l, 0);
 }
 
 #ifdef PT_LUT_LDS
diff --git a/gltf_renderer_amd/csrc/pt_vertex.h b/gltf_renderer_amd/csrc/pt_vertex.h
--- a/gltf_renderer_amd/csrc/pt_vertex.h
+++ b/gltf_renderer_amd/csrc/pt_vertex.h
@@ -81,7 +81,7 @@
 #define PT_TICK(K)
 #define PT_TICK_FLUSH()
 #endif
-template <bool PRE = false>
+template <bool PRE = false, int LEAN = 0>
 PT_DEV bool shade_closest_hit(const SceneRec& sc, const FrameConstants& fc, uint32_t seed, uint32_t px, uint32_t py, const Ray& ray, const HitRec& hit,
                               const RawPacket& packet_in, const ShadePacket* packet_at, PathState& ps, Followups& fu, unsigned& taps, const EnvSample* pre = nullptr,
                               const uint32_t* occ_row = nullptr) {
@@ -122,7 +122,7 @@
     const vec3 intersection = ray.o + (ray.d * hit.t);
     const vec3 o_above = offset_ray(va.position, va.ng), o_below = offset_ray(va.position, -va.ng);
     const vec3 view = -normalize(ray.d);
-    Surface sp = get_surface(sc, flags, mat, mh, va, view, taps);
+    Surface sp = get_surface<LEAN>(sc, flags, mat, mh, va, view, taps);
     PT_TICK(1)
     if (dbg >= PT_DEBUG_OUTPUT_COLOR && dbg <= PT_DEBUG_OUTPUT_TRANSMISSIVE) {
         vec3 c;
@@ -150,7 +150,7 @@
     }
     const Lobes lobes = lobe_probabilities(sp, view);
     sp.sheen_lh = sp.sheen_sv = 0.0f;
-    if (!PT_SHEEN_SKIP || __any(sp.sheen_color.x != 0.0f || sp.sheen_color.y != 0.0f || sp.sheen_color.z != 0.0f)) prepare_sheen(sp, view);
+    if (LEAN != kLeanNoSheen && (!PT_SHEEN_SKIP || __any(sp.sheen_color.x != 0.0f || sp.sheen_color.y != 0.0f || sp.sheen_color.z != 0.0f))) prepare_sheen(sp, view);
     vec3 c = emissive_of(sc, mat, mh, va.tc, taps, sp.emissive_texel);
     fu.origin_above = o_above;
     PT_TICK(2)
@@ -167,7 +167,7 @@
         vec3 contrib = v3(0);
         if (any_gt0(lcol)) {
             float bp = 0;
-            vec3 f = evaluate_bsdf(flags, sc.sheen_e, sp, lobes, va.ng, view, ldir, bp);
+            vec3 f = evaluate_bsdf<LEAN>(flags, sc.sheen_e, sp, lobes, va.ng, view, ldir, bp);
             float mis = fdiv(light_pdf, light_pdf + bp);
             contrib = (mis * f * lcol) / light_pdf;
         }
@@ -192,7 +192,7 @@
         vec3 contrib = v3(0);
         if (any_gt0(lcol)) {
             float bp = 0;
-            vec3 f = evaluate_bsdf(flags, sc.sheen_e, sp, lobes, va.ng, view, ldir, bp);
+            vec3 f = evaluate_bsdf<LEAN>(flags, sc.sheen_e, sp, lobes, va.ng, view, ldir, bp);
             contrib = (lcol * f) / pdf;
         }
         if ((flags & PT_FLAG_SHADOW_RAYS) && !(flags & PT_FLAG_INDIRECT_ENVIRONMENT_ONLY)) {
@@ -208,7 +208,7 @@
         bool is_tr = false, use_mis = false;
         float bp = 1;
         vec3 l = v3(0);
-        vec3 f = sample_bsdf(flags, sc.sheen_e, sp, lobes, v3(r.x, r.y, r.z), view, l, bp, is_tr, use_mis);
+        vec3 f = sample_bsdf<LEAN>(flags, sc.sheen_e, sp, lobes, v3(r.x, r.y, r.z), view, l, bp, is_tr, use_mis);
         vec3 weight = bp != 0 ? f / bp : v3(0);
         vec3 throughput = ps.thr * weight;
         if (dbg >= PT_DEBUG_OUTPUT_BOUNCE_DIRECTION && dbg <= PT_DEBUG_BOUNCE_IS_TRANSMISSION) {
diff --git a/gltf_renderer_amd/csrc/pt_wavefront.hip b/gltf_renderer_amd/csrc/pt_wavefront.hip
--- a/gltf_renderer_amd/csrc/pt_wavefront.hip
+++ b/gltf_renderer_amd/csrc/pt_wavefront.hip
@@ -33,6 +33,7 @@
 #endif
 constexpr uint32_t kCounterStride = 16;
 constexpr int kCounterArrays = 7;
+constexpr uint32_t kAsideCount = 1, kAsideHead = 3, kAsideTotal = 4;
 
 struct WfBuffers {
     float4* L;
@@ -57,6 +58,13 @@
     uint32_t blocks_per_shard;
     uint32_t gen_region_tiles, gen_rounds;
 };
+
+enum { ASIDE_O = 0, ASIDE_D, ASIDE_HIT, ASIDE_ENV_A, ASIDE_ENV_B, ASIDE_BETA, ASIDE_THR, kAsideArrays };
+__host__ __device__ inline float4* aside_array(const WfBuffers& wf, int k) {
+    const size_t q = (size_t)kShards * wf.seg_cap;
+    char* end = PT_OCC_CACHE ? (char*)(wf.sh_c + q * 2) : (char*)(wf.sh_d + q * 2);
+    return (float4*)end + (size_t)k * q;
+}
 
 
 #ifndef PT_STREAM
@@ -407,6 +415,13 @@
     return rare;
 }
 
+PT_DEV bool material_is_lean(const MatHeader& mh, bool sheen) {
+    const uint32_t bm = mh.bound_mask;
+    if (((bm & ((1u << SLOT_COUNT) - 1u)) >> SLOT_SPECULAR) != 0u) return false;
+    return sheen || (mh.sheen_color_factor.x == 0.0f && mh.sheen_color_factor.y == 0.0f && mh.sheen_color_factor.z == 0.0f &&
+                     ((bm & RM_TRIO) != 0u || (bm & ((1u << SLOT_OCCLUSION) - 1u)) == 0u));
+}
+
 #ifndef PT_SHADE_DYNAMIC
 #define PT_SHADE_DYNAMIC 1
 #endif
@@ -421,7 +436,7 @@
 #ifndef PT_SHADE_SPECIALISE
 #define PT_SHADE_SPECIALISE 1
 #endif
-template <uint32_t SPECIAL, bool SMALL>
+template <uint32_t SPECIAL, bool SMALL, int LEAN = 0>
 __global__ __launch_bounds__(kBlock, PT_SHADE_WAVES) void k_wf_shade(SceneRec sc_in, FrameConstants fc_in, WfBuffers wf, int cur, int bounce, Counters* __restrict__ counters) {
     SceneRec sc = sc_in; sc.small_tables = SMALL ? 1u : 0u;
     FrameConstants fc = fc_in;
@@ -445,6 +460,9 @@
     uint32_t* cnt_next = wf.cnt[nxt] + sv.shard * kCounterStride;
     uint32_t* cnt_shadow = wf.cnt[shadow_counter(bounce)] + sv.shard * kCounterStride;
     if (sv.member == 0 && threadIdx.x == 0) { wf.cnt[3][sv.shard * kCounterStride] = 0; wf.cnt[4][sv.shard * kCounterStride] = 0; }
+    uint32_t* cnt_aside = wf.cnt[6] + sv.shard * kCounterStride + kAsideCount + ((uint32_t)bounce & 1u);
+    if (LEAN != 0 && sv.member == 0 && threadIdx.x == 0) { cnt_aside[((uint32_t)bounce & 1u) ? -1 : 1] = 0; wf.cnt[6][sv.shard * kCounterStride + kAsideHead] = 0; }
+    uint32_t n_aside = 0;
     unsigned n_bounce = 0, n_shadow = 0, n_hits = 0;
     LaneStats st = {0, 0, 0, 0};
 #if PT_SHADE_DYNAMIC
@@ -453,7 +471,7 @@
     uint32_t chunk = 0;
     if (lane64 == 0) chunk = atomicAdd(shade_head, 64u);
     chunk = (uint32_t)__builtin_amdgcn_readfirstlane((int)chunk);
-    const bool defer_on = PT_DEFER_FEATURES != 0 && fc.defer_rare != 0;
+    const bool defer_on = PT_DEFER_FEATURES != 0 && LEAN == 0 && fc.defer_rare != 0;
     uint32_t held = kNoHeld;
     __shared__ uint32_t s_hand[kBlock];
     uint32_t* hand = s_hand + (threadIdx.x & ~63u);
@@ -535,6 +553,23 @@
             }
         }
 #endif
+        if (LEAN != 0) {
+            const bool aside = active && hb != kMissTri && !material_is_lean(material_header(sc, load_shade_inst(sc, raw_packet_inst(packet)).material_id), LEAN == kLeanSheen);
+            const uint32_t ia = queue_push(cnt_aside, aside);
+            n_aside += (uint32_t)__popcll(__ballot(aside));
+            if (aside) {
+                const size_t e = base + ia;
+                QST(aside_array(wf, ASIDE_O)[e], o); QST(aside_array(wf, ASIDE_D)[e], d); QST(aside_array(wf, ASIDE_HIT)[e], h);
+#if PT_ENV_PREPASS
+                if (env_prepass_wanted(sc, fc, bounce)) {
+                    QST(aside_array(wf, ASIDE_ENV_A)[e], make_float4(es.dir.x, es.dir.y, es.dir.z, es.pdf));
+                    QST(aside_array(wf, ASIDE_ENV_B)[e], make_float4(es.color.x, es.color.y, es.color.z, 0.0f));
+                }
+#endif
+                if (with_state) { QST(aside_array(wf, ASIDE_BETA)[e], bp); QST(aside_array(wf, ASIDE_THR)[e], tm); }
+                set_aside = true;
+            }
+        }
         if (active && !set_aside) {
             Ray ray;
             ray.o = v3(o.x, o.y, o.z); ray.tmin = 0; ray.d = v3(d.x, d.y, d.z); ray.tmax = o.w;
@@ -566,7 +601,7 @@
                 const uint32_t* occ_row = nullptr;
 #endif
 #if PT_ENV_PREPASS
-                const bool done = shade_closest_hit<true>(sc, fc, sample_seed(fc, slot_sample(fc, slot)), px, py, ray, hit, packet, packet_at, ps, fu, st.taps, &es, occ_row);
+                const bool done = shade_closest_hit<true, LEAN>(sc, fc, sample_seed(fc, slot_sample(fc, slot)), px, py, ray, hit, packet, packet_at, ps, fu, st.taps, &es, occ_row);
 #else
                 const bool done = shade_closest_hit(sc, fc, sample_seed(fc, slot_sample(fc, slot)), px, py, ray, hit, packet, packet_at, ps, fu, st.taps, nullptr, occ_row);
 #endif
@@ -627,6 +662,9 @@
 #if PT_SHADE_DYNAMIC
         if (!flush) chunk = (uint32_t)__builtin_amdgcn_readfirstlane((int)next_chunk);
 #endif
+    }
+    if (LEAN != 0) {
+        if (lane64 == 0 && n_aside != 0) atomicAdd(wf.cnt[6] + sv.shard * kCounterStride + kAsideTotal, n_aside);
     }
     flush_counters(counters, threadIdx.x & 63, 0, n_bounce, n_shadow, n_hits, st);
 }
@@ -713,14 +751,15 @@
 static uint32_t chunks_per_shard_for(size_t slots) { return (uint32_t)(((slots + kBlock - 1) / kBlock + kShards - 1) / kShards); }
 static size_t state_slots_for(size_t slots) { return (size_t)chunks_per_shard_for(slots) * kShards * kBlock; }
 
-size_t wavefront_workspace_bytes(const FrameConstants& fc, int stage_blocks) {
+size_t wavefront_workspace_bytes(const FrameConstants& fc, int stage_blocks, bool aside) {
     const uint32_t bps = blocks_per_shard_for(stage_blocks);
     const size_t slots = state_slots_for((size_t)fc.my_tiles * kBlock * fc.spp);
     const size_t q = (size_t)kShards * seg_cap_for(fc, bps);
-    return slots * (5 * 16) + q * (4 * 16 + 4 * 16 + 16 + 2 * 16 + 2 * 2 * 16 + (PT_OCC_CACHE ? 2 * 4 : 0)) + kCounterArrays * kShards * kCounterStride * 4 + 52 * 256;
-}
-
-static WfBuffers carve(void* base, const FrameConstants& fc, int stage_blocks) {
+    return slots * (5 * 16) + q * (4 * 16 + 4 * 16 + 16 + 2 * 16 + 2 * 2 * 16 + (PT_OCC_CACHE ? 2 * 4 : 0)) + kCounterArrays * kShards * kCounterStride * 4 + 52 * 256 +
+           (aside ? q * kAsideArrays * 16 + kAsideArrays * 256 : 0);
+}
+
+static WfBuffers carve(void* base, const FrameConstants& fc, int stage_blocks, bool aside) {
     const uint32_t slots = fc.my_tiles * kBlock * fc.spp;
     const size_t state_slots = state_slots_for(slots);
     WfBuffers wf;
@@ -745,16 +784,36 @@
     wf.sh_o = (float4*)take(q * 2 * 16);
     wf.sh_d = (float4*)take(q * 2 * 16);
     wf.sh_c = PT_OCC_CACHE ? (uint32_t*)take(q * 2 * 4) : nullptr;
+    if (aside) (void)take(q * 16 * kAsideArrays);
     wf.occ_cache = nullptr;
     wf.capacity = slots;
     return wf;
 }
 
 int traversal_stack_capacity() { return kStackLds + kStackSpill; }
+
+static int shade_variant_of(const FrameConstants& fc) {
+    const uint32_t shade_bits = fc.flags & kShadeFlagMask;
+    return (!PT_SHADE_SPECIALISE || fc.debug_output != PT_DEBUG_OUTPUT_NONE) ? 0 : (shade_bits == kShadeDefaults ? 1 : (shade_bits == kShadeDefaultsNoLights ? 2 : 0));
+}
+static bool shade_small_tables(const SceneRec& sc, const FrameConstants& fc) {
+    return PT_SHADE_SPECIALISE && sc.n_instances <= kInstCacheMax && sc.n_materials <= kMatCacheMax && fc.num_of_lights <= kLightCacheMax;
+}
+bool wavefront_lean_available(const SceneRec& sc, const FrameConstants& fc) { return shade_small_tables(sc, fc) && shade_variant_of(fc) != 0; }
+
+uint64_t wavefront_aside_total(const void* workspace, hipStream_t stream) {
+    std::vector<uint32_t> line((size_t)kShards * kCounterStride);
+    const char* cnt6 = (const char*)workspace + 6 * (((size_t)kShards * kCounterStride * 4 + 255) & ~(size_t)255);
+    if (hipMemcpyAsync(line.data(), cnt6, line.size() * 4, hipMemcpyDeviceToHost, stream) != hipSuccess || hipStreamSynchronize(stream) != hipSuccess) return 0;
+    uint64_t n = 0;
+    for (uint32_t s = 0; s < kShards; s++) n += line[s * kCounterStride + kAsideTotal];
+    return n;
+}
 size_t traversal_grid_lanes(int stage_blocks) { return (size_t)kShards * blocks_per_shard_for(stage_blocks) * kBlock; }
 
 hipError_t launch_wavefront(const SceneRec& sc, const FrameConstants& fc, float4* output, Counters* counters, bool count, void* workspace,
-                            int stage_blocks, StageTimers* timers, hipStream_t stream, uint32_t* occ_cache) {
+                            int stage_blocks, StageTimers* timers, hipStream_t stream, uint32_t* occ_cache, int shade_path) {
+    if (shade_path != SHADE_PATH_GENERAL && !wavefront_lean_available(sc, fc)) return hipErrorInvalidValue;
     if (timers) timers->used = 0;
     if (fc.my_tiles == 0) return hipSuccess;
     auto event_at = [&](size_t i) -> hipEvent_t {
@@ -772,7 +831,7 @@
         timers->used = k + 1;
     };
     const uint32_t slots = fc.my_tiles * kBlock * fc.spp;
-    WfBuffers wf = carve(workspace, fc, stage_blocks);
+    WfBuffers wf = carve(workspace, fc, stage_blocks, shade_path != SHADE_PATH_GENERAL);
     wf.occ_cache = PT_OCC_CACHE ? occ_cache : nullptr;
     hipError_t e = hipMemsetAsync(wf.cnt[0], 0, (size_t)kCounterArrays * kShards * kCounterStride * 4, stream);
     if (e) return e;
@@ -803,10 +862,31 @@
         else { if (count) hipLaunchKernelGGL((k_wf_traverse<true, false>), grid, block, 0, stream, sc, fc, w, nxt, b, rf, rmask, flags, counters);
                else hipLaunchKernelGGL((k_wf_traverse<false, false>), grid, block, 0, stream, sc, fc, w, nxt, b, rf, rmask, flags, counters); }
     };
-    const uint32_t shade_bits = flags & kShadeFlagMask;
-    const int shade_variant = (!PT_SHADE_SPECIALISE || fc.debug_output != PT_DEBUG_OUTPUT_NONE) ? 0 : (shade_bits == kShadeDefaults ? 1 : (shade_bits == kShadeDefaultsNoLights ? 2 : 0));
-    const bool small_tables = PT_SHADE_SPECIALISE && sc.n_instances <= kInstCacheMax && sc.n_materials <= kMatCacheMax && fc.num_of_lights <= kLightCacheMax;
+    const int shade_variant = shade_variant_of(fc);
+    const bool small_tables = shade_small_tables(sc, fc);
+    const bool lean = shade_path != SHADE_PATH_GENERAL, lean_sheen = shade_path == SHADE_PATH_LEAN_SHEEN || shade_path == SHADE_PATH_LEAN_SHEEN_ASIDE;
+    const bool second_pass = shade_path == SHADE_PATH_LEAN_ASIDE || shade_path == SHADE_PATH_LEAN_SHEEN_ASIDE;
     auto launch_shade = [&](dim3 grid, const WfBuffers& w, int cur, int b) {
+        if (lean) {
+            if (lean_sheen) {
+                if (shade_variant == 1) hipLaunchKernelGGL((k_wf_shade<kShadeSpecialised | kShadeDefaults, true, kLeanSheen>), grid, block, 0, stream, sc, fc, w, cur, b, counters);
+                else hipLaunchKernelGGL((k_wf_shade<kShadeSpecialised | kShadeDefaultsNoLights, true, kLeanSheen>), grid, block, 0, stream, sc, fc, w, cur, b, counters);
+            } else {
+                if (shade_variant == 1) hipLaunchKernelGGL((k_wf_shade<kShadeSpecialised | kShadeDefaults, true, kLeanNoSheen>), grid, block, 0, stream, sc, fc, w, cur, b, counters);
+                else hipLaunchKernelGGL((k_wf_shade<kShadeSpecialised | kShadeDefaultsNoLights, true, kLeanNoSheen>), grid, block, 0, stream, sc, fc, w, cur, b, counters);
+            }
+            if (!second_pass) return;
+            WfBuffers a = w;
+            a.ray_o[cur] = aside_array(w, ASIDE_O); a.ray_d[cur] = aside_array(w, ASIDE_D); a.q_beta[cur] = aside_array(w, ASIDE_BETA); a.q_thr[cur] = aside_array(w, ASIDE_THR);
+            a.hit = aside_array(w, ASIDE_HIT); a.env_a = aside_array(w, ASIDE_ENV_A); a.env_b = aside_array(w, ASIDE_ENV_B);
+            a.cnt[cur] = w.cnt[6] + kAsideCount + ((uint32_t)b & 1u);
+            a.cnt[6] = w.cnt[6] + kAsideHead;
+            a.blocks_per_shard = w.blocks_per_shard < 2u ? w.blocks_per_shard : 2u;
+            const dim3 g2(kShards * a.blocks_per_shard);
+            if (shade_variant == 1) hipLaunchKernelGGL((k_wf_shade<kShadeSpecialised | kShadeDefaults, true>), g2, block, 0, stream, sc, fc, a, cur, b, counters);
+            else hipLaunchKernelGGL((k_wf_shade<kShadeSpecialised | kShadeDefaultsNoLights, true>), g2, block, 0, stream, sc, fc, a, cur, b, counters);
+            return;
+        }
         if (small_tables && shade_variant == 1) hipLaunchKernelGGL((k_wf_shade<kShadeSpecialised | kShadeDefaults, true>), grid, block, 0, stream, sc, fc, w, cur, b, counters);
         else if (small_tables && shade_variant == 2) hipLaunchKernelGGL((k_wf_shade<kShadeSpecialised | kShadeDefaultsNoLights, true>), grid, block, 0, stream, sc, fc, w, cur, b, counters);
         else if (small_tables) hipLaunchKernelGGL((k_wf_shade<0u, true>), grid, block, 0, stream, sc, fc, w, cur, b, counters);
```

New measurement: 6100 (median of 2 runs). About the same (-0.1%).
